# monniert/differentiable-blocksworld

Hardware: AMD Instinct MI355X
Metric: rendered views/sec (fwd+bwd) per node, DTU 400x300 K=10 blocks (higher is better)
Workload: dtype f32; 1 GPU; DTU-scan24-like synthetic: 49 views/GPU/step, 400x300, 10 superquadric blocks + ground + sky dome, faces_per_pixel=10, 256^2 textures, coarse phase (sigma=1e-4, opacity noise, decimated textures), MSE+parsimony+TV+overlap, Adam; LPIPS excluded; views_per_gpu=49, n_blocks=10, faces_per_pixel=10, txt_size=256, parallelism=one GPU: all views on it, no collective, nranks=1

## Files before the change

differentiable-blocksworld_amd/build.py:

```python
import os
import subprocess
import sys

HERE = os.path.dirname(os.path.abspath(__file__))
CSRC = os.path.join(HERE, 'csrc')
SOURCES = ['util.hip', 'raster.hip', 'project_clip.hip', 'shade_blend.hip', 'render_fused.hip', 'texture.hip', 'model_ops.hip', 'train_step.hip', 'lpips_head.hip',
           'nn_search.hip', 'render_lit.hip', 'frame_export.hip', 'image_ingest.hip', 'lens_undistort.hip', 'run_monitor.hip']
OUT = os.path.join(HERE, 'dbw_amd', 'libdbw_hip.so')
FLAGS = ['--offload-arch=gfx950', '-O3', '-std=c++17', '-fPIC', '-ffp-contract=off', '-munsafe-fp-atomics',
         '-fno-gpu-flush-denormals-to-zero', '-Wall', '-Wno-unused-function']


def needs_build():
    if not os.path.exists(OUT):
        return True
    t = os.path.getmtime(OUT)
    deps = [os.path.join(CSRC, f) for f in os.listdir(CSRC)] + [os.path.join(HERE, '..', 'include', h) for h in ('dbw_hip.h', 'dbw_eval.h', 'dbw_viz.h', 'dbw_export.h', 'dbw_ingest.h', 'dbw_lens.h', 'dbw_monitor.h')] + [__file__]
    return any(os.path.getmtime(d) > t for d in deps)


def build(force=False, verbose=False, extra_flags=()):
    if not force and not needs_build():
        return OUT
    hipcc = os.environ.get('HIPCC', '/opt/rocm/bin/hipcc')
    objs = []
    os.makedirs(os.path.join(HERE, 'build'), exist_ok=True)
    procs = []
    for s in SOURCES:
        o = os.path.join(HERE, 'build', s.replace('.hip', '.o'))
        objs.append(o)
        cmd = [hipcc] + FLAGS + list(extra_flags) + ['-c', os.path.join(CSRC, s), '-o', o]
        if verbose:
            print(' '.join(cmd))
        procs.append((s, subprocess.Popen(cmd, stdout=subprocess.PIPE, stderr=subprocess.STDOUT)))
    for s, p in procs:
        out, _ = p.communicate()
        if p.returncode != 0:
            sys.stderr.write(out.decode())
            raise RuntimeError(f'hipcc failed on {s}')
        if verbose and out:
            print(out.decode())
    subprocess.check_call([hipcc, '--offload-arch=gfx950', '-shared', '-fPIC'] + objs + ['-o', OUT])
    return OUT


def build_device_checks(force=False):
    src = os.path.join(HERE, '..', 'tests', 'device_checks.hip')
    out_dir = os.path.join(HERE, '..', 'tests', '_build')
    out = os.path.join(out_dir, 'libdbw_device_checks.so')
    deps = [src] + [os.path.join(CSRC, f) for f in ('dbw_common.h', 'raster_math.h', 'model_math.h', 'rng_math.h')]
# ... 11 lines not shown
```

differentiable-blocksworld_amd/csrc/env_bwd.h:

```cpp
#pragma once
#include "shade_common.h"

namespace dbw {

#ifndef DBW_HARD_TEX_LOG2
#define DBW_HARD_TEX_LOG2 6
#endif
#ifndef DBW_HARD_FACE_LOG2
#define DBW_HARD_FACE_LOG2 5
#endif
typedef LdsAgg<3, DBW_HARD_TEX_LOG2> HardTexAgg;
typedef LdsAgg<9, DBW_HARD_FACE_LOG2> HardFaceAgg;

#ifndef DBW_HARD_P
#define DBW_HARD_P 2
#endif
template <int P>
struct HardRegion {
    static_assert(P == 1 || P == 2 || P == 4, "tiles per wave: 1, 2 or 4");
    static constexpr int PX = P == 1 ? 1 : 2, PY = P / PX;
    static constexpr int RX = 2 * PX, RY = 2 * PY;
    static long long blocks(int N, int H, int W) {
        const int tx = (W + 7) >> 3, ty = (H + 7) >> 3;
        return (long long)N * ((tx + RX - 1) / RX) * ((ty + RY - 1) / RY);
    }
};

__device__ __forceinline__ void env_bwd_pixel(const ShadeArgs &A, const float *__restrict__ fv, float *__restrict__ gmaps, float *__restrict__ gfv,
                                              int want_bary, int persp, const MapDescCache &mdc, const int *s_md, HardTexAgg &tex_agg,
                                              HardFaceAgg &face_agg, bool valid, int fc, float u, float v, int jm, const float (&gc)[3], int xi, int yi) {
    const int j = jm & 0xfffff, map = jm >> 20;
    const bool tex = valid && (gc[0] != 0.f || gc[1] != 0.f || gc[2] != 0.f);
    Sample s;
    s.a00 = s.a01 = s.a10 = s.a11 = 0;
    s.w00 = s.w01 = s.w10 = s.w11 = 0.f;
    if (__ballot(tex) != 0ull) {
        int md[6];
        mdc.get(A, s_md, valid ? map : 0, md);
        footprint_desc(u, v, md[0], md[1], md[2], md[3], md[4], md[5], s);
        float w00 = s.w00, w01 = s.w01, w10 = s.w10, w11 = s.w11;
        if (s.a01 == s.a00) { w00 += w01; w01 = 0.f; }
        if (s.a10 == s.a00) { w00 += w10; w10 = 0.f; }
        if (s.a11 == s.a00) { w00 += w11; w11 = 0.f; }
        else if (s.a11 == s.a01) { w01 += w11; w11 = 0.f; }
        else if (s.a11 == s.a10) { w10 += w11; w11 = 0.f; }
        const int ad[4] = {s.a00, s.a01, s.a10, s.a11};
        const float wt[4] = {w00, w01, w10, w11};
        const int f = wt[1] != 0.f ? 1 : (wt[2] != 0.f ? 2 : 3);
        const int a2[2] = {ad[0], f == 1 ? ad[1] : (f == 2 ? ad[2] : ad[3])};
        const float w2[2] = {wt[0], f == 1 ? wt[1] : (f == 2 ? wt[2] : wt[3])};
#pragma unroll
        for (int q = 0; q < 2; ++q) {
            float val[3] = {gc[0] * w2[q], gc[1] * w2[q], gc[2] * w2[q]};
            const bool on = tex && w2[q] != 0.f;
            tex_agg.template add_wave_merged<4>(gmaps, (int)((unsigned)a2[q] / 3u), val, on);
        }
        const bool rest = tex && ((f == 1 && (wt[2] != 0.f || wt[3] != 0.f)) || (f == 2 && wt[3] != 0.f));
        const unsigned long long rm = __ballot(rest);
        if (rm != 0ull) {
            const bool wide = __popcll(rm) > 16;
#pragma unroll
            for (int q = 2; q < 4; ++q) {
                float val[3] = {gc[0] * wt[q], gc[1] * wt[q], gc[2] * wt[q]};
                const bool on = rest && q > f && wt[q] != 0.f;
                const int key = (int)((unsigned)ad[q] / 3u);
                if (wide) tex_agg.template add_wave_merged<4>(gmaps, key, val, on);
                else if (on) tex_agg.add(gmaps, key, val);
            }
        }
    }
    const bool geom = tex && want_bary != 0 && j >= A.geom_begin;
    float g9[9] = {0.f, 0.f, 0.f, 0.f, 0.f, 0.f, 0.f, 0.f, 0.f};
    bool has_g9 = false;
    if (__ballot(geom) != 0ull) {
        if (geom) {
            float gu, gv;
            sample_grad_uv(A.maps, s, gc, gu, gv);
            const float *uv = A.face_uvs + (long long)j * 6;
            const float go[3] = {gu * uv[0] + gv * uv[1], gu * uv[2] + gv * uv[3], gu * uv[4] + gv * uv[5]};
            int cd = -1;
            float w2 = 0.f, w3 = 0.f;
            if (A.c2o) {
                cd = A.code[fc]; w2 = A.cw[(long long)fc * 2]; w3 = A.cw[(long long)fc * 2 + 1];
            }
            float gb[3] = {0.f, 0.f, 0.f};
            convert_bary_bwd(cd, w2, w3, go, gb);
            if (gb[0] != 0.f || gb[1] != 0.f || gb[2] != 0.f) {
                has_g9 = true;
                f2 pndc;
                pndc.x = pix_to_ndc_fast(A.W - 1 - xi, ndc_axis_given(A.W, A.ndc[0], A.ndc[1]));
                pndc.y = pix_to_ndc_fast(A.H - 1 - yi, ndc_axis_given(A.H, A.ndc[2], A.ndc[3]));
                const float *q = fv + (long long)fc * 9;
                const f2 a{q[0], q[1]}, b{q[3], q[4]}, c{q[6], q[7]};
                const float z0 = q[2], z1 = q[5], z2 = q[8];
                const f3 bary0 = bary_fwd<true>(pndc, a, b, c);
                const f3 bp = persp ? persp_fwd<true>(bary0, z0, z1, z2) : bary0;
                f3 gg3{gb[0], gb[1], gb[2]};
                gg3 = clip_bwd<true>(bp, gg3);
                float pz0 = 0.f, pz1 = 0.f, pz2 = 0.f;
                if (persp) gg3 = persp_bwd<true>(bary0, z0, z1, z2, gg3, pz0, pz1, pz2);
                f2 e0, e1, e2;
                bary_bwd<true>(pndc, a, b, c, gg3, e0, e1, e2);
                g9[0] = e0.x; g9[1] = e0.y; g9[2] = pz0;
                g9[3] = e1.x; g9[4] = e1.y; g9[5] = pz1;
                g9[6] = e2.x; g9[7] = e2.y; g9[8] = pz2;
            }
        }
        face_agg.add_wave(gfv, valid ? fc : 0, g9, has_g9);
    }
}


template <int P>
__device__ __forceinline__ void env_bwd_region(const ShadeArgs &A, long long total_blocks, const float *__restrict__ gimg,
                                               float *__restrict__ gmaps, const float *__restrict__ fv, float *__restrict__ gfv,
                                               int want_bary, int persp, void *lds, int *s_md) {
    typedef HardRegion<P> R;
    constexpr int NTH = 256;
    const long long logical = xcd_remap(blockIdx.x, total_blocks);
    if (logical < 0) return;
    HardTexAgg tex_agg;
    HardFaceAgg face_agg;
    tex_agg.bind(lds);
    face_agg.bind((char *)lds + HardTexAgg::BYTES);
    const int lane = threadIdx.x & 63;
    const int wv = __builtin_amdgcn_readfirstlane(threadIdx.x >> 6);
    const int tiles_x = (A.W + 7) >> 3, tiles_y = (A.H + 7) >> 3;
    const int rx = (tiles_x + R::RX - 1) / R::RX, ry = (tiles_y + R::RY - 1) / R::RY;
    const int n = (int)(logical / (rx * ry)), t = (int)(logical % (rx * ry));
    const int tx0 = (t % rx) * R::RX + (wv & 1) * R::PX, ty0 = (t / rx) * R::RY + (wv >> 1) * R::PY;
    const long long view0 = (long long)n * tiles_y * tiles_x;
    const long long plane = (long long)A.H * A.W;
    const float gs = A.gscale ? *A.gscale : 1.f;
    int rfc[P], xs[P], ys[P];
    float ru[P], rv[P], rjm[P], rg[P][3];
    bool inpx[P];
#pragma unroll
    for (int p = 0; p < P; ++p) {
        const int tx = tx0 + p % R::PX, ty = ty0 + p / R::PX;
        const bool real = tx < tiles_x && ty < tiles_y;
        const long long tile = real ? view0 + (long long)ty * tiles_x + tx : view0;
        xs[p] = tx * 8 + (lane & 7);
        ys[p] = ty * 8 + (lane >> 3);
        inpx[p] = real && xs[p] < A.W && ys[p] < A.H;
        rfc[p] = ld_stream(A.p2f + (tile << 6) + lane);
        const float *b = A.bary + ((tile * 3) << 6) + lane;
        ru[p] = ld_stream(b); rv[p] = ld_stream(b + 64); rjm[p] = ld_stream(b + 128);
        const int xc = xs[p] < A.W ? xs[p] : A.W - 1, yc = ys[p] < A.H ? ys[p] : A.H - 1;
        const long long gb = A.img_tiled ? ((tile * 4) << 6) + lane : (long long)n * 4 * plane + (long long)yc * A.W + xc;
        const long long cs = A.img_tiled ? 64 : plane;
        rg[p][0] = ld_stream(gimg + gb); rg[p][1] = ld_stream(gimg + gb + cs); rg[p][2] = ld_stream(gimg + gb + 2 * cs);
    }
    tex_agg.clear(threadIdx.x, NTH);
    face_agg.clear(threadIdx.x, NTH);
    MapDescCache mdc;
    mdc.load(A, s_md, nullptr, threadIdx.x, NTH, true);
    __syncthreads();
    bool valid[P];
    int fc[P], jm[P];
    float gc[P][3];
#pragma unroll
    for (int p = 0; p < P; ++p) {
        valid[p] = inpx[p] && rfc[p] >= 0;
        fc[p] = valid[p] ? rfc[p] : 0;
        jm[p] = valid[p] ? __float_as_int(rjm[p]) : 0;
        ru[p] = valid[p] ? ru[p] : 0.f;
        rv[p] = valid[p] ? rv[p] : 0.f;
#pragma unroll
        for (int c = 0; c < 3; ++c) gc[p][c] = valid[p] ? rg[p][c] * gs : 0.f;
    }
#pragma unroll 1
    for (int p = 0; p < P; ++p)
        env_bwd_pixel(A, fv, gmaps, gfv, want_bary, persp, mdc, s_md, tex_agg, face_agg, valid[p], fc[p], ru[p], rv[p], jm[p], gc[p], xs[p], ys[p]);
    __syncthreads();
    tex_agg.flush(gmaps, threadIdx.x, NTH);
    face_agg.flush(gfv, threadIdx.x, NTH);
}

}
```

differentiable-blocksworld_amd/csrc/render_fused.hip:

```cpp
#include "raster_common.h"
#include "shade_common.h"
#include "loss_math.h"
#include "raster_bin.h"
#include "step_kernels.h"
#include "../../include/dbw_hip.h"

#include <math.h>
#include <stdlib.h>
#include <string.h>

using namespace dbw;

int dbw_prepare_raster(const float *face_verts, const int *first_idx, const int *num_faces, const int *neighbor, int N, long long F_total,
                       long long max_faces_per_view, int H, int W, float margin, int cull, void *workspace, size_t workspace_bytes,
                       dbw::CoarseBins &cb, hipStream_t s, bool launch, bool want_cells);
const dbw::FaceRec *dbw_workspace_recs(const void *workspace, long long F_total);
void *dbw_workspace_shade_recs(void *workspace, long long F_total);
int dbw_fill_shade_args(ShadeArgs &A, const int32_t *pix_to_face, const float *bary, const float *dists, const int32_t *c2o,
                        const int32_t *clip_code, const float *clip_w, int Fc_stride, const float *face_uvs,
                        const int32_t *face_map, const int32_t *map_desc, const float *maps, const float *faces_alpha,
                        int alpha_len, int N, int H, int W, int K, int F, float sigma, const float *background3);

#ifdef DBW_TILE_CLOCK
namespace dbw { __device__ unsigned g_tile_clock[1 << 18][4]; }
extern "C" void dbw_debug_read_tile_clock(unsigned *out, int nblocks) {
    (void)hipDeviceSynchronize();
    (void)hipMemcpyFromSymbol(out, HIP_SYMBOL(dbw::g_tile_clock), (size_t)(nblocks < (1 << 18) ? nblocks : (1 << 18)) * 16);
}
#endif
#ifdef DBW_PROFILE_FWD
extern "C" void dbw_debug_read_fwd_profile(unsigned long long *out16, int reset) {
    static unsigned long long *host = nullptr;
    const size_t bytes = (size_t)dbw::FPROF_BLOCKS * 16 * sizeof(unsigned long long);
    if (!host) host = (unsigned long long *)malloc(bytes);
    (void)hipDeviceSynchronize();
    (void)hipMemcpyFromSymbol(host, HIP_SYMBOL(dbw::g_fprof), bytes);
    for (int i = 0; i < 16; ++i) out16[i] = 0;
    for (size_t b = 0; b < (size_t)dbw::FPROF_BLOCKS; ++b)
// ... 115 lines not shown
                    bary[o.b + 3 * o.bstride] = a;
                    bary[o.b + 4 * o.bstride] = c[0]; bary[o.b + 5 * o.bstride] = c[1]; bary[o.b + 6 * o.bstride] = c[2];
                }
            }
        }
    }
    const ImgAddr ia = img_addr(A, n, yi, xi, 4);
    float *out = image + ia.base;
    float px[4];
    blend_front_finish(bl, A.bg, px);
    out[0] = px[0]; out[ia.cstride] = px[1]; out[2 * ia.cstride] = px[2]; out[3 * ia.cstride] = px[3];
}

struct UvSlot { bool valid; int fik; pay4 v; ShadeRec sr; };

template <int KMAX>
__device__ __forceinline__ UvSlot uv_slot(const TopK<KMAX, true> &q, const pay4 *home, const ShadeRec *__restrict__ srec, int k, bool in_img) {
    UvSlot s;
    float pz = 0.f;
    s.fik = 0;
    s.v = pay4{0.f, 0.f, 0.f, 0.f};
    s.valid = q.get(k, home, 64, threadIdx.x, pz, s.fik, s.v) && in_img;
    if (!s.valid) s.fik = 0;
    s.sr = srec[s.fik];
    return s;
}

__device__ __forceinline__ ShadeRec load_srec_uniform(const ShadeRec *__restrict__ sp) {
    union { v16f v; ShadeRec r; } u;
    u.v = *(const v16f *)sp;
    return u.r;
}

struct EnvFold {
    const FaceRec *recs;
    const int *first_idx;
    const int2 *cell; const int *pool;
    const int *dom;
    const int *clist, *ccount; int nx, ny;
    const int *num_faces;
    const ShadeRec *srec;
    const float *maps;
    float bg[3];
    int *p2f; float *uvj;
    int persp, dbg;
    float ndc[4];
};

__device__ __forceinline__ void env_fold_pixel(const EnvFold &E, int H, int W, int n_, int xi, int yi, bool in_img, float (&rgb)[3]) {
    const int lane = threadIdx.x;
    const int n = __builtin_amdgcn_readfirstlane(n_);
    const int tiles_x = (W + 7) >> 3, tiles_y = (H + 7) >> 3;
    const int L = __builtin_amdgcn_readfirstlane((n * tiles_y + (yi >> 3)) * tiles_x + (xi >> 3));
    const NdcAxis ax = ndc_axis_given(W, E.ndc[0], E.ndc[1]), ay = ndc_axis_given(H, E.ndc[2], E.ndc[3]);
    f2 p;
    p.x = pix_to_ndc_fast(W - 1 - xi, ax);
    p.y = pix_to_ndc_fast(H - 1 - yi, ay);
    const bool fastdiv = DBW_RASTER_FASTDIV && !(E.dbg & 1);
    const int fb = __builtin_amdgcn_readfirstlane(E.first_idx[n]);
    const int jb = __builtin_amdgcn_readfirstlane(E.dom[L]);
    if (jb >= 0 && fastdiv && !(E.dbg & 4096)) {
        const FaceRec r = load_rec_nowait(E.recs + fb + jb);
        float pz1 = 0.f, sd1 = 0.f;
        f3 bc1{0.f, 0.f, 0.f};
        bool unsafe = false;
        const bool inbox = in_img && !(p.x < r.xlo || p.x > r.xhi || p.y < r.ylo || p.y > r.yhi);
        const bool keep = inbox && eval_pair<true>(r, p, 0.f, E.persp, 1, pz1, sd1, bc1, unsafe, true);
        if (__ballot(in_img && (!keep || unsafe)) == 0ull) {
            const ShadeRec sr = load_srec_uniform(E.srec + fb + jb);
            const float bc[3] = {bc1.x, bc1.y, bc1.z};
            float bo[3], u, vv;
            convert_bary(sr.cd, sr.w2, sr.w3, bc, bo);
            interp_uv(bo, sr.uv, u, vv);
            SampleFwd s;
            footprint_fwd(u, vv, sr.off, sr.hw >> 16, sr.hw & 0xffff, sr.pads >> 16, sr.pads & 0xffff, sr.sh, s);
            fetch_fwd(E.maps, s, rgb);
            if (in_img) {
                const long long o = ((long long)L << 6) + lane;
                float *bp = E.uvj + ((long long)L * 3 << 6) + lane;
#if DBW_NT_STORES
                __builtin_nontemporal_store(fb + jb, E.p2f + o);
                __builtin_nontemporal_store(u, bp); __builtin_nontemporal_store(vv, bp + 64);
                __builtin_nontemporal_store(__int_as_float(sr.j | (sr.map << 20)), bp + 128);
#else
                E.p2f[o] = fb + jb;
                bp[0] = u; bp[64] = vv; bp[128] = __int_as_float(sr.j | (sr.map << 20));
#endif
            }
            return;
        }
    }
    TopK<1, false> q;
    q.init();
    const int2 c_ = E.cell[L];
    const int2 c = make_int2(__builtin_amdgcn_readfirstlane(c_.x), __builtin_amdgcn_readfirstlane(c_.y));
    const bool walk = c.y < 0;
    int total = c.y > 0 ? c.y : 0, cx = 0, cy = 0;
    const int *__restrict__ lst = E.pool + c.x;
    if (walk) {
        const int x0 = __builtin_amdgcn_readfirstlane(xi & ~7), y0 = __builtin_amdgcn_readfirstlane(yi & ~7);
        const int nb = E.nx * E.ny, bin = (y0 / COARSE) * E.nx + (x0 / COARSE);
        total = __builtin_amdgcn_readfirstlane(E.ccount[n * nb + bin]);
        lst = E.clist + (long long)fb * nb + (long long)bin * __builtin_amdgcn_readfirstlane(E.num_faces[n]);
        cx = (x0 & (COARSE - 1)) >> 3; cy = (y0 & (COARSE - 1)) >> 3;
    }
#pragma unroll 1
    for (int cb0 = 0; cb0 < total; cb0 += DBW_WAVE) {
        const bool have = cb0 + lane < total;
        const int e = have ? lst[cb0 + lane] : 0;
        const bool hit = have && (!walk || !(cx < ((e >> 20) & 7) || cx > ((e >> 23) & 7) || cy < ((e >> 26) & 7) || cy > ((e >> 29) & 7)));
        const unsigned long long m = __ballot(hit);
        eval_staged_chunk<1, false>(E.recs, fb, e & 0xfffff, min(DBW_WAVE, total - cb0), in_img, p, 1, 0.f, E.persp, 1, fastdiv, true, q, nullptr, DBW_WAVE,
                                    lane, false, false, m);
    }
    float pz = 0.f;
    int fi = 0;
    pay4 v{0.f, 0.f, 0.f, 0.f};
    const bool valid = q.get(0, nullptr, DBW_WAVE, lane, pz, fi, v) && in_img;
    if (!valid) fi = 0;
    const ShadeRec sr = E.srec[fi];
    const float bc[3] = {v.y, v.z, v.w};
    float bo[3], u, vv;
    convert_bary(sr.cd, sr.w2, sr.w3, bc, bo);
    interp_uv(bo, sr.uv, u, vv);
    SampleFwd s;
    footprint_fwd(u, vv, sr.off, sr.hw >> 16, sr.hw & 0xffff, sr.pads >> 16, sr.pads & 0xffff, sr.sh, s);
    float col[3];
    fetch_fwd(E.maps, s, col);
#pragma unroll
    for (int k = 0; k < 3; ++k) rgb[k] = valid ? col[k] : E.bg[k];
    if (in_img) {
        const long long o = ((long long)L << 6) + lane;
#if DBW_NT_STORES
        __builtin_nontemporal_store(valid ? fi : -1, E.p2f + o);
#else
        E.p2f[o] = valid ? fi : -1;
#endif
        if (valid) {
            float *bp = E.uvj + ((long long)L * 3 << 6) + lane;
#if DBW_NT_STORES
            __builtin_nontemporal_store(u, bp); __builtin_nontemporal_store(vv, bp + 64);
            __builtin_nontemporal_store(__int_as_float(sr.j | (sr.map << 20)), bp + 128);
#else
            bp[0] = u; bp[64] = vv; bp[128] = __int_as_float(sr.j | (sr.map << 20));
#endif
        }
    }
}

template <bool TILED>
__device__ __forceinline__ void uv8_epilogue_t(const ShadeArgs &A, int n, int xi, int yi, bool in_img, int tile, int lane, const float (&px)[4],
                                               float *__restrict__ image, const float (&env_rgb)[3], bool fold, bool no_fragments) {
    const long long plane = (long long)A.H * A.W, pix = (long long)yi * A.W + xi;
    const long long cs = TILED ? 64 : plane;
    const long long o4 = TILED ? (long long)tile * 256 : (long long)n * 4 * plane, o3 = TILED ? (long long)tile * 192 : (long long)n * 3 * plane;
    const unsigned ul = (unsigned)lane;
    const long long ol = TILED ? (long long)ul : pix;
    const float f0 = px[0], f1 = px[1], f2 = px[2], m = px[3];
    if (A.target) {
// ... 23 lines not shown
#endif
        }
        const float tot = wave_sum_dpp(sq);
        if (lane == 0) A.loss_part[tile] = tot;
    } else if (in_img) {
        float *out = image + o4 + ol;
        out[0] = f0;
        out[cs] = f1;
        out[2 * cs] = f2;
        out[3 * cs] = m;
    }
}
__device__ __forceinline__ void uv8_epilogue(const ShadeArgs &A, int n, int xi, int yi, bool in_img, int tile, int lane, const float (&px)[4],
                                             float *__restrict__ image, const float (&env_rgb)[3], bool fold, bool no_fragments = false) {
    if (A.img_tiled) uv8_epilogue_t<true>(A, n, xi, yi, in_img, tile, lane, px, image, env_rgb, fold, no_fragments);
    else uv8_epilogue_t<false>(A, n, xi, yi, in_img, tile, lane, px, image, env_rgb, fold, no_fragments);
}

template <int KMAX>
__device__ __forceinline__ void shade_uv8_empty(const ShadeArgs &A, int K, int n, int xi, int yi, int *__restrict__ p2f, float *__restrict__ image,
                                                const float (&env_rgb)[3], bool fold) {
    const int lane = threadIdx.x;
    const bool in_img = xi < A.W && yi < A.H;
    const int tiles_x = (A.W + 7) >> 3, tiles_y = (A.H + 7) >> 3;
    const int tile = __builtin_amdgcn_readfirstlane((n * tiles_y + (yi >> 3)) * tiles_x + (xi >> 3));
    if (in_img) p2f[(((long long)tile * K) << 6) + lane] = -1;
    BlendFront bl;
    blend_front_init(bl);
    float px[4];
    blend_front_finish(bl, A.bg, px);
    uv8_epilogue(A, n, xi, yi, in_img, tile, lane, px, image, env_rgb, fold, true);
}

template <int KMAX>
__device__ __forceinline__ void shade_uv8(const ShadeArgs &A, int K, const ShadeRec *__restrict__ srec, const TopK<KMAX, true> &q, const pay4 *home, int n,
                                          int xi, int yi, int *__restrict__ p2f, float *__restrict__ bary, float *__restrict__ dists,
                                          float *__restrict__ image, int dbg, const float (&env_rgb)[3], bool fold) {
    const int lane = threadIdx.x;
    const bool in_img = xi < A.W && yi < A.H;
    const int tiles_x = (A.W + 7) >> 3, tiles_y = (A.H + 7) >> 3;
    const int tile = __builtin_amdgcn_readfirstlane((n * tiles_y + (yi >> 3)) * tiles_x + (xi >> 3));
    const long long tb = ((long long)tile * K) << 6;
    int *__restrict__ p2f_t = p2f + tb;
    float *__restrict__ dists_t = dists + tb;
    float *__restrict__ bary_t = bary + tb * 8;
#if DBW_TOPK_ORDERED
    const int cnt = in_img ? q.cnt : 0;
#else
    int cnt = 0;
#pragma unroll
    for (int k = 0; k < KMAX; ++k) cnt += (in_img && k < K && q.valid(k)) ? 1 : 0;
#endif
    if (in_img && cnt == 0) p2f_t[lane] = -1;
    BlendFront bl;
    blend_front_init(bl);
    bool more = __ballot(cnt > 0) != 0ull && !(dbg & 64);
    UvSlot cur;
    cur.valid = false; cur.fik = 0; cur.v = pay4{0.f, 0.f, 0.f, 0.f};
    if (more) cur = uv_slot(q, home, srec, 0, in_img);
    UvSlot nxt = cur;
#pragma unroll
    for (int k = 0; k < KMAX; ++k) {
        more = more && k < K && __ballot(cnt > k) != 0ull;
        if (!more) break;
        if (k + 1 < KMAX) nxt = uv_slot(q, home, srec, k + 1, in_img);
        const ShadeRec &sr = cur.sr;
        const float bc[3] = {cur.v.y, cur.v.z, cur.v.w};
        float bo[3];
        convert_bary(sr.cd, sr.w2, sr.w3, bc, bo);
        float u, v;
        interp_uv(bo, sr.uv, u, v);
        const float d = cur.v.x;
        float e;
        if (A.sigma == 0.f) e = d <= 0.f ? 1.f : 0.f;
#if DBW_FWD_FAST_EXP
        else e = __expf(-(d > 0.f ? d : 0.f) * A.inv_sigma);
#else
        else e = expf(-(d > 0.f ? d : 0.f) / A.sigma);
#endif
        const float a = cur.valid ? e * sr.fa : 0.f;
        SampleFwd s;
        footprint_fwd(u, v, sr.off, sr.hw >> 16, sr.hw & 0xffff, sr.pads >> 16, sr.pads & 0xffff, sr.sh, s);
        float c[3];
        fetch_fwd(A.maps, s, c);
        if (!(a != 0.f)) c[0] = c[1] = c[2] = 0.f;
        const float T = bl.T;
        blend_front_step(bl, a, c);
        if (cur.valid && !(dbg & 32)) {
            const int o = (k << 6) + lane;
#if DBW_NT_STORES
            __builtin_nontemporal_store(k == 0 ? (cur.fik | (cnt << FRAG_COUNT_SHIFT)) : cur.fik, p2f_t + o);
            __builtin_nontemporal_store(d, dists_t + o);
            float *bp = bary_t + (k << 9) + lane;
            __builtin_nontemporal_store(u, bp);
            __builtin_nontemporal_store(v, bp + 64);
            __builtin_nontemporal_store(__int_as_float(sr.j | (sr.map << 20)), bp + 128);
            __builtin_nontemporal_store(a, bp + 192);
            __builtin_nontemporal_store(c[0], bp + 256); __builtin_nontemporal_store(c[1], bp + 320); __builtin_nontemporal_store(c[2], bp + 384);
            __builtin_nontemporal_store(T, bp + 448);
#else
            p2f_t[o] = k == 0 ? (cur.fik | (cnt << FRAG_COUNT_SHIFT)) : cur.fik;
            dists_t[o] = d;
            float *bp = bary_t + (k << 9) + lane;
            bp[0] = u;
            bp[64] = v;
            bp[128] = __int_as_float(sr.j | (sr.map << 20));
            bp[192] = a;
            bp[256] = c[0]; bp[320] = c[1]; bp[384] = c[2];
            bp[448] = T;
#endif
        }
        cur = nxt;
    }
    float px[4];
    blend_front_finish(bl, A.bg, px);
    uv8_epilogue(A, n, xi, yi, in_img, tile, lane, px, image, env_rgb, fold);
}

#define DBW_RENDER_WAVES(KMAX, UV) ((UV) ? ((KMAX) <= 4 ? 6 : (KMAX) <= 10 ? 5 : (KMAX) <= 16 ? 3 : 2) : DBW_RASTER_WAVES(KMAX))
template <int KMAX, int TW, int TH, int GROUP, bool UV, bool KEX = false>
__global__ __launch_bounds__(TW * TH, DBW_RENDER_WAVES(KMAX, UV)) void render_fwd_kernel(const FaceRec *__restrict__ recs, const float4 *__restrict__ bbox,
                                                             const int *__restrict__ first_idx, const int *__restrict__ num_faces,
                                                             float blur, int persp, int dbg,
                                                             long long total_blocks, ShadeArgs A, CoarseBins cb, const ShadeRec *__restrict__ srec,
                                                             int *__restrict__ p2f, float *__restrict__ bary, float *__restrict__ dists,
                                                             float *__restrict__ image, const EnvFold E) {
    static_assert(!UV || (TW == 8 && TH == 8), "shade_uv8 needs one wave per 8x8 tile");
    int n, xi, yi;
    TopK<KMAX, UV> q;
    pay4 *home;
    FPROF_T(t_k0);
    FPROF_ADD(13, wall_clock64());
#ifdef DBW_TILE_CLOCK
    if (KMAX > 1 && blockIdx.x < (1u << 18)) g_tile_clock[blockIdx.x][3] = (unsigned)wall_clock64();
#endif
    bool empty = false;
    float env_rgb[3] = {0.f, 0.f, 0.f};
#if defined(DBW_PROFILE_FWD) || defined(DBW_TILE_CLOCK)
    constexpr bool fold = false;
    (void)E;
#else
    const bool fold = UV && E.recs != nullptr;
#endif
    auto env_layer = [&](int n_, int xi_, int yi_, bool in_img_) {
        if constexpr (UV) { if (fold) env_fold_pixel(E, A.H, A.W, n_, xi_, yi_, in_img_, env_rgb); }
    };
    const int K = KEX ? KMAX : A.K;
    if (!raster_tile<KMAX, TW, TH, GROUP, UV>(recs, bbox, first_idx, num_faces, A.H, A.W, K, blur, persp, 1, total_blocks, cb,
                                              (dbg & (3 | 128)) | ((KMAX == 1 && A.tiled != 0 && !(dbg & 8)) ? 8 : 0), n, xi, yi, q, home,
                                              UV ? &empty : nullptr, env_layer)) return;
    FPROF_T(t_k1);
    if constexpr (UV) {
        if (empty) shade_uv8_empty<KMAX>(A, K, n, xi, yi, p2f, image, env_rgb, fold);
        else shade_uv8<KMAX>(A, K, srec, q, home, n, xi, yi, p2f, bary, dists, image, dbg, env_rgb, fold);
    }
    else {
        if (xi >= A.W || yi >= A.H) return;
        shade_generic<KMAX, TW * TH>(A, q, home, n, xi, yi, p2f, bary, dists, image);
    }
    FPROF_T(t_k2);
    FPROF_ADD(2, t_k2 - t_k1);
    FPROF_ADD(3, t_k2 - t_k0);
    FPROF_ADD(14, wall_clock64());
#ifdef DBW_TILE_CLOCK
    if (KMAX > 1 && threadIdx.x == 0 && blockIdx.x < (1u << 18)) {
        unsigned *o = g_tile_clock[blockIdx.x];
        o[0] = (unsigned)n | ((__builtin_amdgcn_s_getreg((16 - 1) << 11 | 4) & 0xffffu) << 16); o[1] = ((unsigned)(yi >> 3) << 16) | (unsigned)(xi >> 3); o[2] = (unsigned)wall_clock64();
    }
#endif
}

template <int KMAX, int TW, int TH, int GROUP, bool UV, bool KEX = false>
int launch_v(const FaceRec *recs, const float4 *bbox, const int *first_idx, const int *num_faces, float blur,
             int persp, ShadeArgs &A, const CoarseBins &cb, const ShadeRec *srec, int *p2f, float *bary, float *dists, float *image, const EnvFold &E,
             hipStream_t s) {
    const long long total = (long long)A.N * ((A.W + TW - 1) / TW) * ((A.H + TH - 1) / TH);
    DBW_REQUIRE(total < (1LL << 31) - 8, "more than 2^31 tiles in one pass");
    hipLaunchKernelGGL((render_fwd_kernel<KMAX, TW, TH, GROUP, UV, KEX>), dim3(dbw_xcd_grid(total)), dim3(TW * TH), 0, s, recs, bbox, first_idx,
                       num_faces, blur, persp, g_render_dbg, total, A, cb, srec, p2f, bary, dists, image, E);
    return dbw_check_launch("render_fwd_kernel");
}

template <int KMAX>
int launch(const FaceRec *recs, const float4 *bbox, const int *first_idx, const int *num_faces, float blur,
           int persp, ShadeArgs &A, const CoarseBins &cb, const ShadeRec *srec, int *p2f, float *bary, float *dists, float *image, const EnvFold &E,
           hipStream_t s) {
#define DBW_V(TW, TH, G, UV) launch_v<KMAX, TW, TH, G, UV>(recs, bbox, first_idx, num_faces, blur, persp, A, cb, srec, p2f, bary, dists, image, E, s)
    if constexpr (KMAX == 1) {
        if (g_render_variant == 1) return DBW_V(8, 8, 2, false);
        if (g_render_variant == 2) return DBW_V(16, 8, 2, false);
        return DBW_V(16, 16, 1, false);
    }
    else {
#ifndef DBW_FWD_GROUP
#define DBW_FWD_GROUP 2
#endif
        if (A.tiled == 2 && (A.target || !(g_render_dbg & 4)) && A.sigma >= 0.f) {
#if DBW_FWD_KEXACT
            if (A.K == KMAX) return launch_v<KMAX, 8, 8, DBW_FWD_GROUP, true, true>(recs, bbox, first_idx, num_faces, blur, persp, A, cb, srec, p2f, bary, dists, image, E, s);
#endif
            return DBW_V(8, 8, DBW_FWD_GROUP, true);
        }
        return DBW_V(8, 8, DBW_FWD_GROUP, false);
    }
#undef DBW_V
}

}

struct MseArgs { const float *env_img, *target; float scale; float *loss_part, *g_fg, *g_env; float *rec_out = nullptr; const float *grad_rec = nullptr; };

static int render_fwd_impl(const float *face_verts_c, const int32_t *first_idx, const int32_t *num_faces,
                                    const int32_t *neighbor, const int32_t *c2o, const int32_t *clip_code,
                                    const float *clip_w, int Fc_stride, const float *face_uvs, const int32_t *face_map,
                                    const int32_t *map_desc, const float *maps, const float *faces_alpha, int alpha_len,
                                    int N, int64_t F_total, int H, int W, int K, int F, float sigma, float blur_radius,
                                    int perspective_correct, const float *background3, int32_t *pix_to_face, float *bary,
                                    float *dists, float *image, void *workspace, size_t workspace_bytes,
                                    int frag_layout, const MseArgs *mse, int stage, int image_layout, dbw_stream_t stream,
                                    const dbw::EnvFoldHost *fold = nullptr) {
    DBW_REQUIRE(stage >= 0 && stage <= 2, "stage must be 0 (whole pass), 1 (workspace only) or 2 (workspace already prepared)");
    DBW_REQUIRE(face_verts_c && first_idx && num_faces && pix_to_face && bary && dists && (image || mse) && workspace, "null pointer");
    DBW_REQUIRE(workspace_bytes >= dbw_rasterize_workspace_bytes(F_total), "workspace too small");
    DBW_REQUIRE(blur_radius >= 0.f && F_total >= 0, "bad blur_radius / F_total");
    ShadeArgs A;
    int rc = dbw_fill_shade_args(A, pix_to_face, bary, dists, c2o, clip_code, clip_w, Fc_stride, face_uvs, face_map, map_desc, maps,
                                 faces_alpha, alpha_len, N, H, W, K, F, sigma, background3);
    if (rc) return rc;
    DBW_REQUIRE(frag_layout >= 0 && frag_layout <= 3, "frag_layout must be 0 (N,H,W,K), 1 (8x8-tile planar), 2 (planar, uv) or 3 (planar, hard uv)");
    DBW_REQUIRE(frag_layout < 2 || F < (1 << 20), "frag_layouts 2 and 3 pack the face id in 20 bits");
    DBW_REQUIRE(frag_layout != 3 || (K == 1 && sigma == 0.f && blur_radius == 0.f && !faces_alpha),
                "frag_layout 3 is the hard single-layer pass: K == 1, sigma == 0, no faces_alpha");
    DBW_REQUIRE(frag_layout != 2 || F_total < (1LL << FRAG_COUNT_SHIFT), "frag_layout 2 packs the clipped face id in 26 bits");
    DBW_REQUIRE(image_layout == 0 || image_layout == 1, "image_layout must be 0 (N,C,H,W) or 1 (8x8-tile planar)");
    A.tiled = frag_layout;
    A.img_tiled = image_layout;
    if (mse) {
        DBW_REQUIRE(frag_layout == 2 && K > 1 && sigma >= 0.f, "the composite + MSE epilogue belongs to the uv-fragment soft pass (frag_layout 2, K > 1, sigma >= 0)");
        DBW_REQUIRE(stage == 1 || ((mse->env_img || fold) && mse->target && mse->loss_part && mse->g_fg && mse->g_env), "null pointer");
        A.env_img = mse->env_img; A.target = mse->target; A.mse_scale = mse->scale; A.loss_part = mse->loss_part; A.g_fg = mse->g_fg; A.g_env = mse->g_env;
        A.rec_out = mse->rec_out; A.grad_rec = mse->grad_rec;
    }
    if (K > DBW_MAX_FACES_PER_PIXEL) {
        dbw_set_error("dbw_render_fwd_fused: faces_per_pixel=%d > %d", K, DBW_MAX_FACES_PER_PIXEL);
        return DBW_ERR_UNSUPPORTED;
    }
    if (N == 0) return DBW_OK;
    hipStream_t s = (hipStream_t)stream;
    const float margin = (float)sqrt((double)blur_radius);
    CoarseBins cb;
    rc = dbw_prepare_raster(face_verts_c, first_idx, num_faces, neighbor, N, F_total, c2o ? (long long)Fc_stride : F_total, H, W, margin, 0, workspace, workspace_bytes, cb, s,
                            stage != 2,  K > 1 || g_render_variant == 1);
    if (rc) return rc;
    const float4 *bbox = (const float4 *)workspace;
    const FaceRec *recs = dbw_workspace_recs(workspace, F_total);
    ShadeRec *srec = nullptr;
    if (frag_layout == 2 && K > 1 && F_total > 0) {
        srec = (ShadeRec *)dbw_workspace_shade_recs(workspace, F_total);
        if (stage != 2) {
            hipLaunchKernelGGL(shade_setup_kernel, dim3((unsigned)((F_total + 255) / 256)), dim3(256), 0, s, A, first_idx, num_faces, (long long)F_total, srec);
            rc = dbw_check_launch("shade_setup_kernel");
            if (rc) return rc;
        }
    }
    if (stage == 1) return DBW_OK;
    EnvFold E;
    memset(&E, 0, sizeof(E));
    if (fold) {
        DBW_REQUIRE(mse && frag_layout == 2 && K > 1, "the env layer folds into the soft pass with the loss epilogue");
        DBW_REQUIRE(fold->ws && fold->ws->cells && fold->ws->dom && fold->ws->shade_recs && fold->first_idx && fold->num_faces && fold->maps && fold->p2f && fold->uvj, "null pointer (env fold)");
        const dbw::RasterWorkspace &w = *fold->ws;
        E.recs = w.recs; E.first_idx = fold->first_idx; E.cell = w.cell; E.pool = w.pool; E.dom = w.dom; E.clist = w.list; E.ccount = w.count; E.nx = w.nx; E.ny = w.ny;
        E.num_faces = fold->num_faces; E.srec = (const ShadeRec *)w.shade_recs; E.maps = fold->maps;
        for (int i = 0; i < 3; ++i) E.bg[i] = fold->bg[i];
        E.p2f = fold->p2f; E.uvj = fold->uvj; E.persp = perspective_correct; E.dbg = g_render_dbg;
        for (int i = 0; i < 4; ++i) E.ndc[i] = cb.ndc[i];
        A.lean_grads = 1;
    }
#define DBW_RF(KM) launch<KM>(recs, bbox, first_idx, num_faces, blur_radius, perspective_correct, A, cb, srec, pix_to_face, bary, dists, image, E, s)
    if (K == 1) return DBW_RF(1);
    if (K <= 4) return DBW_RF(4);
    if (K <= 10) return DBW_RF(10);
    if (K <= 16) return DBW_RF(16);
    return DBW_RF(25);
#undef DBW_RF
}

extern "C" int dbw_render_fwd_fused(const float *face_verts_c, const int32_t *first_idx, const int32_t *num_faces,
                                    const int32_t *neighbor, const int32_t *c2o, const int32_t *clip_code,
                                    const float *clip_w, int Fc_stride, const float *face_uvs, const int32_t *face_map,
                                    const int32_t *map_desc, const float *maps, const float *faces_alpha, int alpha_len,
                                    int N, int64_t F_total, int H, int W, int K, int F, float sigma, float blur_radius,
                                    int perspective_correct, const float *background3, int32_t *pix_to_face, float *bary,
                                    float *dists, float *image, void *workspace, size_t workspace_bytes,
                                    int frag_layout, int stage, int image_layout, dbw_stream_t stream) {
    return render_fwd_impl(face_verts_c, first_idx, num_faces, neighbor, c2o, clip_code, clip_w, Fc_stride, face_uvs, face_map, map_desc, maps,
                           faces_alpha, alpha_len, N, F_total, H, W, K, F, sigma, blur_radius, perspective_correct, background3, pix_to_face,
                           bary, dists, image, workspace, workspace_bytes, frag_layout, nullptr, stage, image_layout, stream);
}

extern "C" int dbw_render_fwd_fused_mse(const float *face_verts_c, const int32_t *first_idx, const int32_t *num_faces,
                                        const int32_t *neighbor, const int32_t *c2o, const int32_t *clip_code,
                                        const float *clip_w, int Fc_stride, const float *face_uvs, const int32_t *face_map,
                                        const int32_t *map_desc, const float *maps, const float *faces_alpha, int alpha_len,
                                        int N, int64_t F_total, int H, int W, int K, int F, float sigma, float blur_radius,
                                        int perspective_correct, const float *background3, int32_t *pix_to_face, float *bary,
                                        float *dists, void *workspace, size_t workspace_bytes, const float *env_image,
                                        const float *target, float mse_scale, float *loss_partial, float *grad_fg,
                                        float *grad_env, int stage, int image_layout, dbw_stream_t stream) {
    const MseArgs mse{env_image, target, mse_scale, loss_partial, grad_fg, grad_env, nullptr, nullptr};
    return render_fwd_impl(face_verts_c, first_idx, num_faces, neighbor, c2o, clip_code, clip_w, Fc_stride, face_uvs, face_map, map_desc, maps,
                           faces_alpha, alpha_len, N, F_total, H, W, K, F, sigma, blur_radius, perspective_correct, background3, pix_to_face,
                           bary, dists, nullptr, workspace, workspace_bytes, 2, &mse, stage, image_layout, stream);
}

int dbw::render_fwd_fused_mse_fold(const float *face_verts_c, const int32_t *first_idx, const int32_t *num_faces, const int32_t *neighbor,
                                   const int32_t *c2o, const int32_t *clip_code, const float *clip_w, int Fc_stride, const float *face_uvs,
                                   const int32_t *face_map, const int32_t *map_desc, const float *maps, const float *faces_alpha, int alpha_len, int N,
                                   int64_t F_total, int H, int W, int K, int F, float sigma, float blur_radius, int perspective_correct,
                                   const float *background3, int32_t *pix_to_face, float *bary, float *dists, void *workspace, size_t workspace_bytes,
                                   const float *target, float mse_scale, float *loss_partial, float *grad_fg, float *grad_env, const EnvFoldHost &fold,
                                   float *rec_out, const float *grad_rec, hipStream_t stream) {
    const MseArgs mse{nullptr, target, mse_scale, loss_partial, grad_fg, grad_env, rec_out, grad_rec};
    return render_fwd_impl(face_verts_c, first_idx, num_faces, neighbor, c2o, clip_code, clip_w, Fc_stride, face_uvs, face_map, map_desc, maps,
                           faces_alpha, alpha_len, N, F_total, H, W, K, F, sigma, blur_radius, perspective_correct, background3, pix_to_face,
                           bary, dists, nullptr, workspace, workspace_bytes, 2, &mse, 2, 1, (dbw_stream_t)stream, &fold);
}
```

differentiable-blocksworld_amd/csrc/shade_blend.hip:

```cpp
#include "shade_common.h"
#include "env_bwd.h"
#include "../../include/dbw_hip.h"
#include "step_kernels.h"

#include <stdlib.h>
#include <string.h>

using namespace dbw;

__device__ __forceinline__ void st_stream4(int4 *p, int4 v) {
#if DBW_NT_LOADS
    int *q = (int *)p;
    typedef int v4i __attribute__((ext_vector_type(4)));
    v4i w; w.x = v.x; w.y = v.y; w.z = v.z; w.w = v.w;
    __builtin_nontemporal_store(w, (v4i *)q);
#else
    *p = v;
#endif
}

__device__ __forceinline__ void st_record(int4 *records, unsigned long long idx, int packed, float wx1, float wy1, float g0, float g1, float g2) {
    typedef int v2i __attribute__((ext_vector_type(2)));
    v2i *q = (v2i *)records + idx * 3ull;
    v2i a, b, c;
    a.x = packed; a.y = __float_as_int(wx1); b.x = __float_as_int(wy1); b.y = __float_as_int(g0); c.x = __float_as_int(g1); c.y = __float_as_int(g2);
#if DBW_NT_LOADS
    __builtin_nontemporal_store(a, q); __builtin_nontemporal_store(b, q + 1); __builtin_nontemporal_store(c, q + 2);
#else
    q[0] = a; q[1] = b; q[2] = c;
#endif
}

namespace {

#ifndef DBW_BWD_UNROLL
// ... 487 lines not shown
    const float t = (dx * (p.x - a.x) + dy * (p.y - a.y)) * __builtin_amdgcn_rcpf(l2);
    tt = t < 0.f ? 0.f : (t > 1.f ? 1.f : t);
    const float qx = a.x + tt * dx, qy = a.y + tt * dy;
    return (p.x - qx) * (p.x - qx) + (p.y - qy) * (p.y - qy);
}

struct BinRes {
    int bin, rank, leader, base, packed;
    float wx1, wy1;
    uint2 lay;
};

constexpr int ALPHA_DIRECT_MAPS = 64, ALPHA_DIRECT_SPREAD = 8;
constexpr size_t ALPHA_DIRECT_BYTES = (size_t)ALPHA_DIRECT_MAPS * ALPHA_DIRECT_SPREAD * sizeof(double);
#ifndef DBW_TEX_MERGE
#define DBW_TEX_MERGE 1
#endif
#ifndef DBW_FACE_MERGE
#define DBW_FACE_MERGE 1
#endif
#ifndef DBW_FACE_MERGE_BINNED
#define DBW_FACE_MERGE_BINNED 1
#endif
constexpr int TEX_MERGE = DBW_TEX_MERGE, FACE_MERGE = DBW_FACE_MERGE;
#ifndef DBW_UVB_WAVES
#define DBW_UVB_WAVES 4
#endif
#ifdef DBW_TILE_CLOCK
__device__ unsigned g_bwd_clock[1 << 16][4];
#define BWD_CLOCK_END(n_, layers_) { if (threadIdx.x == 0 && blockIdx.x < (1u << 16)) { unsigned *o_ = g_bwd_clock[blockIdx.x]; o_[0] = (unsigned)(n_); o_[1] = (unsigned)(layers_); o_[2] = (unsigned)wall_clock64(); } }
#else
#define BWD_CLOCK_END(n_, layers_)
#endif
template <bool BINNED>
__global__ __launch_bounds__(NT, (BINNED ? DBW_UVB_WAVES : 5)) void render_bwd_uv_kernel(ShadeArgs A, long long total_blocks, const float *__restrict__ gimg,
                                                              float *__restrict__ gmaps, float *__restrict__ galpha,
                                                              const float *__restrict__ fv, float *__restrict__ gfv) {
    extern __shared__ __attribute__((aligned(16))) float s_uvbwd[];
    constexpr bool SINGLE = false;
    (void)SINGLE;
    TexAgg tex_agg;
    FaceAlphaAgg fa_agg;
    if (A.sync_flag && blockIdx.x == 0 && threadIdx.x == 0) __hip_atomic_store(A.sync_flag, A.sync_val, __ATOMIC_RELEASE, __HIP_MEMORY_SCOPE_AGENT);
#ifdef DBW_TILE_CLOCK
    if (blockIdx.x < (1u << 16)) { g_bwd_clock[blockIdx.x][3] = (unsigned)wall_clock64(); g_bwd_clock[blockIdx.x][2] = 0u; }
#endif
    int n, xi, yi;
    if (!pixel_of_block<true>(A, total_blocks, n, xi, yi)) return;
    const bool in_img = xi < A.W && yi < A.H;
    const int lane = threadIdx.x & 63;
    const int tiles_x = (A.W + 7) >> 3, tiles_y = (A.H + 7) >> 3;
    const bool phantom = (yi >> 3) >= tiles_y || (xi >> 3) >= tiles_x;
    const int tile = __builtin_amdgcn_readfirstlane(phantom ? n * tiles_y * tiles_x : (n * tiles_y + (yi >> 3)) * tiles_x + (xi >> 3));
    const long long tb = ((long long)tile * A.K) << 6;
    const int *__restrict__ p2f_t = A.p2f + tb + lane;
    const float *__restrict__ dists_t = A.dists + tb + lane;
    const float *__restrict__ bary_t = A.bary + tb * 8 + lane;
    int cnt = 0;
    if (in_img && (yi >> 3) < tiles_y && (xi >> 3) < tiles_x) {
        const int raw0 = ld_stream(p2f_t);
        cnt = raw0 < 0 ? 0 : (raw0 >> FRAG_COUNT_SHIFT);
    }
    if (!BINNED) {
        tex_agg.bind(s_uvbwd);
        tex_agg.clear(threadIdx.x, NT);
    }
    fa_agg.bind((char *)s_uvbwd + (BINNED ? 0 : TexAgg::BYTES));
    fa_agg.clear(threadIdx.x, NT);
#ifndef DBW_MD_LDS_UNBINNED
#define DBW_MD_LDS_UNBINNED 0
#endif
    constexpr bool MD_LDS = BINNED || DBW_MD_LDS_UNBINNED;
    __shared__ __attribute__((aligned(16))) int s_md[MD_LDS ? MD_CACHE_MAPS * 8 : 8];
#ifndef DBW_LAST_WAVE_FLUSH
#define DBW_LAST_WAVE_FLUSH 1
#endif
    constexpr bool LAST_WAVE_FLUSH = BINNED && DBW_LAST_WAVE_FLUSH;
    __shared__ int s_done;
    if (threadIdx.x == 0) s_done = 0;
    MapDescCache mdc;
    mdc.load(A, s_md, BINNED ? A.bin_base : nullptr, threadIdx.x, NT, MD_LDS);
    double *alpha_dir = (double *)((char *)s_uvbwd + (BINNED ? 0 : TexAgg::BYTES) + FaceAlphaAgg::BYTES);
    const int n_maps = -A.alpha_len;
    const bool alpha_direct = galpha && A.faces_alpha && A.alpha_len < 0 && n_maps <= ALPHA_DIRECT_MAPS;
    if (alpha_direct)
        for (int i = threadIdx.x; i < n_maps * ALPHA_DIRECT_SPREAD; i += NT) alpha_dir[i] = 0.0;
    if (!__syncthreads_or(cnt > 0)) { BWD_CLOCK_END(n, -1); return; }
    f2 pndc;
    pndc.x = pix_to_ndc(A.W - 1 - xi, A.W, A.H);
    pndc.y = pix_to_ndc(A.H - 1 - yi, A.H, A.W);
    const long long plane = (long long)A.H * A.W;
    float gr = 0.f, gg = 0.f, gbl = 0.f, gA = 0.f;
    if (in_img && cnt > 0) {
        const ImgAddr ia = img_addr(A, n, yi, xi, 4);
        const float *gi = gimg + ia.base;
        const float gs = A.gscale ? *A.gscale : 1.f;
        gr = ld_stream(gi) * gs; gg = ld_stream(gi + ia.cstride) * gs; gbl = ld_stream(gi + 2 * ia.cstride) * gs; gA = ld_stream(gi + 3 * ia.cstride) * gs;
    }
    PROF_T(t_begin);
    int kmax = 0;
    for (int k = 0; k < A.K; ++k) {
        if (__ballot(cnt > k) == 0ull) break;
        kmax = k + 1;
    }
    PROF_T(t_p0);
    PROF_ADD(0, t_begin, t_p0);
    BlendBack bk;
    blend_back_init(bk, A.bg);
    struct Raw { int fc; float u, v, jm, a, c0, c1, c2, T, d; };
    auto load = [&](int k, bool ok) {
        Raw r;
        r.fc = 0; r.u = r.v = r.jm = r.a = r.c0 = r.c1 = r.c2 = r.d = 0.f; r.T = 1.f;
        if (ok) {
            r.fc = ld_stream(p2f_t + (k << 6)) & FRAG_FACE_MASK;
            const float *b = bary_t + (k << 9);
            r.u = ld_stream(b); r.v = ld_stream(b + 64); r.jm = ld_stream(b + 128); r.a = ld_stream(b + 192);
            r.c0 = ld_stream(b + 256); r.c1 = ld_stream(b + 320); r.c2 = ld_stream(b + 384); r.T = ld_stream(b + 448);
            r.d = ld_stream(dists_t + (k << 6));
        }
        return r;
    };
    auto load_u = [&](int k) {
        Raw r;
        r.fc = ld_stream(p2f_t + (k << 6));
        const float *b = bary_t + (k << 9);
        r.u = ld_stream(b); r.v = ld_stream(b + 64); r.jm = ld_stream(b + 128); r.a = ld_stream(b + 192);
        r.c0 = ld_stream(b + 256); r.c1 = ld_stream(b + 320); r.c2 = ld_stream(b + 384); r.T = ld_stream(b + 448);
        r.d = ld_stream(dists_t + (k << 6));
        return r;
    };
    auto masked = [&](const Raw &x, bool ok) {
        Raw r;
        r.fc = ok ? (x.fc & FRAG_FACE_MASK) : 0;
        r.u = ok ? x.u : 0.f; r.v = ok ? x.v : 0.f; r.jm = ok ? x.jm : 0.f; r.a = ok ? x.a : 0.f;
        r.c0 = ok ? x.c0 : 0.f; r.c1 = ok ? x.c1 : 0.f; r.c2 = ok ? x.c2 : 0.f; r.T = ok ? x.T : 1.f; r.d = ok ? x.d : 0.f;
        return r;
    };
    struct FaceXY { float2 v0, v1, v2; };
    auto load_xy = [&](int fc) {
        FaceXY q;
        const float *p = fv + (long long)fc * 9;
        q.v0 = make_float2(p[0], p[1]); q.v1 = make_float2(p[3], p[4]); q.v2 = make_float2(p[6], p[7]);
        return q;
    };
    const int sub = tile & (BIN_SUB - 1);
    auto reserve = [&](const Raw &r, bool ok) {
        BinRes R;
        R.bin = -1; R.rank = 0; R.leader = 0; R.base = 0; R.packed = 0; R.wx1 = R.wy1 = 0.f; R.lay = make_uint2(0u, 0u);
        const float wgt = r.T * r.a;
        const bool tex = ok && (wgt * gr != 0.f || wgt * gg != 0.f || wgt * gbl != 0.f) && !(A.dbg & (1 << 19));
        if (__ballot(tex) == 0ull) return R;
        const int map = __float_as_int(r.jm) >> 20;
        int md[6];
        mdc.get(A, s_md, tex ? map : 0, md);
        Sample s;
        footprint_desc(r.u, r.v, md[0], md[1], md[2], md[3], md[4], md[5], s);
        const bool on = tex && bin_regular(s);
        if (on) {
            R.bin = mdc.get_extra(s_md, A.bin_base, map) + (s.r0 >> 5) * ((s.ws + 31) >> 5) + (s.c0 >> 5);
            R.packed = (int)((unsigned)(s.r0 & 31) | ((unsigned)(s.c0 & 31) << 5) | ((unsigned)(s.r0 - s.r1) << 10) | ((unsigned)(s.c1 - s.c0) << 11));
            R.wx1 = s.wx1; R.wy1 = s.wy1;
        }
        unsigned long long rem = __ballot(on);
        const unsigned long long below = (1ull << lane) - 1ull;
        while (rem) {
// ... 48 lines not shown
            if (g7[6] != 0.f) atomicAdd(&alpha_dir[map * ALPHA_DIRECT_SPREAD + (lane & (ALPHA_DIRECT_SPREAD - 1))], (double)g7[6]);
            g7[6] = 0.f;
        }
        const bool f_pre = valid && (gd != 0.f || g7[6] != 0.f) && !(A.dbg & 2);
        PROF_T(t_a);
        PROF_ADD(2, t_it, t_a);
        if (BINNED) {
            if (__ballot(tex) != 0ull) {
                const unsigned start = (unsigned)__shfl((int)(cres.lay.x + (unsigned)cres.base), cres.leader, 64);
                const int room = __shfl((int)cres.lay.y - cres.base, cres.leader, 64);
                bool pending = tex;
                if (tex && cres.bin >= 0) {
                    if (cres.rank < room) {
                        if (!(A.dbg & (1 << 17)))
                            st_record(A.bin_records, (unsigned long long)(start + (unsigned)cres.rank), cres.packed, cres.wx1, cres.wy1, gc[0], gc[1], gc[2]);
                        pending = false;
                    }
                }
                if (pending) {
                    int md[6];
                    mdc.get(A, s_md, map, md);
                    Sample s;
                    footprint_desc(cur.u, cur.v, md[0], md[1], md[2], md[3], md[4], md[5], s);
#pragma unroll
                    for (int ch = 0; ch < 3; ++ch) {
                        unsafeAtomicAdd(gmaps + s.a00 + ch, gc[ch] * s.w00);
                        unsafeAtomicAdd(gmaps + s.a01 + ch, gc[ch] * s.w01);
                        unsafeAtomicAdd(gmaps + s.a10 + ch, gc[ch] * s.w10);
                        unsafeAtomicAdd(gmaps + s.a11 + ch, gc[ch] * s.w11);
                    }
                }
            }
        } else if (__ballot(tex) != 0ull) {
            int md[6];
            mdc.get(A, s_md, valid ? map : 0, md);
            Sample s;
            footprint_desc(cur.u, cur.v, md[0], md[1], md[2], md[3], md[4], md[5], s);
            float w00 = s.w00, w01 = s.w01, w10 = s.w10, w11 = s.w11;
            if (s.a01 == s.a00) { w00 += w01; w01 = 0.f; }
            if (s.a10 == s.a00) { w00 += w10; w10 = 0.f; }
            if (s.a11 == s.a00) { w00 += w11; w11 = 0.f; }
            else if (s.a11 == s.a01) { w01 += w11; w11 = 0.f; }
            else if (s.a11 == s.a10) { w10 += w11; w11 = 0.f; }
            const int ad[4] = {s.a00, s.a01, s.a10, s.a11};
            const float wt[4] = {w00, w01, w10, w11};
#ifdef DBW_STATS_BWD
            {
                int dk, rp, taps = 0, tap_lanes = 0, tap_replays = 0;
                for (int q = 0; q < 4; ++q) {
                    const bool onq = tex && wt[q] != 0.f;
                    key_stats((int)((unsigned)ad[q] / 3u), onq, dk, rp);
                    taps += __ballot(onq) != 0ull ? 1 : 0;
                    tap_lanes += __popcll(__ballot(onq));
                    tap_replays += rp;
                    if (q == 0) STAT_ADD(2, dk);
                }
                STAT_ADD(1, tap_lanes); STAT_ADD(3, taps); STAT_ADD(7, tap_replays);
            }
#endif
            const int f = wt[1] != 0.f ? 1 : (wt[2] != 0.f ? 2 : 3);
            const int a2[2] = {ad[0], f == 1 ? ad[1] : (f == 2 ? ad[2] : ad[3])};
            const float w2[2] = {wt[0], f == 1 ? wt[1] : (f == 2 ? wt[2] : wt[3])};
#pragma unroll
            for (int q = 0; q < 2; ++q) {
                float v3[3] = {gc[0] * w2[q], gc[1] * w2[q], gc[2] * w2[q]};
                bool on = tex && w2[q] != 0.f && !(A.dbg & 1);
                if (TEX_MERGE > 0 && __ballot(on) != 0ull) lane_merge<3, TEX_MERGE>((int)((unsigned)a2[q] / 3u), on, v3);
                if (on) tex_agg.add(gmaps, (int)((unsigned)a2[q] / 3u), v3);
            }
            const bool rest = tex && !(A.dbg & 1) && ((f == 1 && (wt[2] != 0.f || wt[3] != 0.f)) || (f == 2 && wt[3] != 0.f));
            if (__ballot(rest) != 0ull) {
#pragma unroll
                for (int q = 2; q < 4; ++q)
                    if (rest && q > f && wt[q] != 0.f) {
                        const float v3[3] = {gc[0] * wt[q], gc[1] * wt[q], gc[2] * wt[q]};
                        tex_agg.add(gmaps, (int)((unsigned)ad[q] / 3u), v3);
                    }
            }
        }
        PROF_T(t_b);
        PROF_ADD(4, t_a, t_b);
        if (__ballot(gd != 0.f) != 0ull && !(A.dbg & 16)) {
            f2 v0, v1, v2;
            if (PIPE) { v0 = f2{curq.v0.x, curq.v0.y}; v1 = f2{curq.v1.x, curq.v1.y}; v2 = f2{curq.v2.x, curq.v2.y}; }
            else {
                const float *q = fv + (long long)(valid ? cur.fc : 0) * 9;
                v0 = f2{q[0], q[1]}; v1 = f2{q[3], q[4]}; v2 = f2{q[6], q[7]};
            }
            float t01, t02, t12;
            const float e01 = seg_dist_t(pndc, v0, v1, t01), e02 = seg_dist_t(pndc, v0, v2, t02), e12 = seg_dist_t(pndc, v1, v2, t12);
            const int sel = (e01 <= e02 && e01 <= e12) ? 0 : ((e02 <= e01 && e02 <= e12) ? 1 : ((e12 <= e01 && e12 <= e02) ? 2 : 3));
            const f2 ea = sel == 2 ? v1 : v0, eb = sel == 0 ? v1 : v2;
            const float tt = sel == 0 ? t01 : (sel == 1 ? t02 : t12);
            const float qx = (1.f - tt) * ea.x + tt * eb.x, qy = (1.f - tt) * ea.y + tt * eb.y;
            const float g = sel == 3 ? 0.f : gd;
            const float gax = g * (1.f - tt) * 2.f * (qx - pndc.x), gay = g * (1.f - tt) * 2.f * (qy - pndc.y);
            const float gbx = g * tt * 2.f * (qx - pndc.x), gby = g * tt * 2.f * (qy - pndc.y);
            g7[0] = sel <= 1 ? gax : 0.f; g7[1] = sel <= 1 ? gay : 0.f;
            g7[2] = sel == 0 ? gbx : (sel == 2 ? gax : 0.f); g7[3] = sel == 0 ? gby : (sel == 2 ? gay : 0.f);
            g7[4] = sel >= 1 ? gbx : 0.f; g7[5] = sel >= 1 ? gby : 0.f;
        }
        PROF_T(t_c);
        PROF_ADD(5, t_b, t_c);
#ifdef DBW_STATS_BWD
        {
            int dk, rp;
            const bool f_on = valid && (gd != 0.f || g7[6] != 0.f);
            key_stats(cur.fc, f_on, dk, rp);
            STAT_ADD(0, 1); STAT_ADD(4, __popcll(__ballot(f_on))); STAT_ADD(5, dk); STAT_ADD(6, rp);
        }
#endif
        bool f_on = f_pre;
        constexpr int FM = BINNED ? DBW_FACE_MERGE_BINNED : FACE_MERGE;
        if (FM > 0 && __ballot(f_on) != 0ull) lane_merge<7, FM>(cur.fc, f_on, g7);
        if (f_on) {
            const int aidx = A.faces_alpha ? (int)alpha_grad_index(A, n, j, map) : 0;
            fa_agg.add(gfv, galpha, cur.fc, aidx, g7);
        }
        PROF_T(t_d);
        PROF_ADD(6, t_c, t_d);
    }
    PROF_T(t_end);
    int last = 0;
    if (LAST_WAVE_FLUSH) {
        if (lane == 0) last = atomicAdd(&s_done, 1) == NT / 64 - 1 ? 1 : 0;
        last = __builtin_amdgcn_readfirstlane(last);
    } else __syncthreads();
    PROF_T(t_sync);
    PROF_ADD(3, t_end, t_sync);
    if ((LAST_WAVE_FLUSH && !last) || (A.dbg & 128)) return;
    const int f_tid = LAST_WAVE_FLUSH ? lane : (int)threadIdx.x, f_n = LAST_WAVE_FLUSH ? 64 : NT;
    if (!BINNED) tex_agg.flush(gmaps, f_tid, f_n);
    fa_agg.flush(gfv, galpha, f_tid, f_n);
    if (alpha_direct)
        for (int i = f_tid; i < n_maps * ALPHA_DIRECT_SPREAD; i += f_n) {
            const float x = (float)alpha_dir[i];
            if (x != 0.f) unsafeAtomicAdd(galpha + (long long)(i / ALPHA_DIRECT_SPREAD) * DBW_ALPHA_SPREAD + ((blockIdx.x * ALPHA_DIRECT_SPREAD + i) & (DBW_ALPHA_SPREAD - 1)), x);
        }
    PROF_T(t_fl);
    PROF_ADD(1, t_sync, t_fl);
    PROF_ADD(7, t_begin, t_fl);
    BWD_CLOCK_END(n, kmax);
}

#ifndef DBW_BIN_STAGE
#define DBW_BIN_STAGE 512
#endif
constexpr int BIN_STAGE = DBW_BIN_STAGE, BIN_PER_THREAD = BIN_STAGE / 256, BIN_LANE_STRIDE = BIN_STAGE / 64;
typedef int bin_fix_t;
constexpr int BIN_FIX_SH = 20, BIN_FIX_EMIN = -100;
__global__ __launch_bounds__(256) void texbin_reduce_kernel(const int *__restrict__ bin_info, const int *__restrict__ cursor,
                                                            const int4 *__restrict__ records, int cap, const unsigned *__restrict__ layout,
                                                            float *__restrict__ gmaps) {
    __shared__ bin_fix_t tile[33 * 33 * 3];
    __shared__ int2 stage[BIN_STAGE * 3 + BIN_STAGE / BIN_LANE_STRIDE];
    __shared__ float s_wmax[4];
#ifdef DBW_REDUCE_SCRAMBLE
    const unsigned bx = blockIdx.x, nb_ = gridDim.x;
    const int bin = bx < (nb_ & ~63u) ? (int)((bx & ~63u) | ((__brev(bx & 63u) >> 26) ^ (((bx >> 6) * 2654435761u) >> 26))) : (int)bx;
    const int sub0 = blockIdx.y * BIN_SUB_PER_WG;
#else
    const int bin = (int)window_scramble(blockIdx.x, gridDim.x), sub0 = blockIdx.y * BIN_SUB_PER_WG;
#endif
    int n_sub[BIN_SUB_PER_WG], total = 0;
    unsigned first[BIN_SUB_PER_WG];
#pragma unroll
    for (int g = 0; g < BIN_SUB_PER_WG; ++g) {
        const int ci = bin * BIN_SUB + sub0 + g;
        first[g] = layout[ci * 2];
        n_sub[g] = min(cursor[ci], (int)layout[ci * 2 + 1]);
        total += n_sub[g];
    }
    if (total == 0) return;
    for (int i = threadIdx.x; i < 33 * 33 * 3; i += 256) tile[i] = 0;
    const int lane = threadIdx.x & 63, wv = threadIdx.x >> 6;
// ... 124 lines not shown
        for (int i = 0; i < 8; ++i) out8[i] += host[b * 8 + i];
    if (reset) { memset(host, 0, bytes); (void)hipMemcpyToSymbol(HIP_SYMBOL(g_prof), host, bytes); }
}
#endif

int fill_args(ShadeArgs &A, const int32_t *pix_to_face, const float *bary, const float *dists, const int32_t *c2o,
              const int32_t *clip_code, const float *clip_w, int Fc_stride, const float *face_uvs,
              const int32_t *face_map, const int32_t *map_desc, const float *maps, const float *faces_alpha,
              int alpha_len, int N, int H, int W, int K, int F, float sigma, const float *background3) {
    DBW_REQUIRE(pix_to_face && bary && dists && face_uvs && face_map && map_desc && maps, "null pointer");
    DBW_REQUIRE((c2o && clip_code && clip_w) || (!c2o && !clip_code && !clip_w), "c2o/clip_code/clip_w: all or none");
    DBW_REQUIRE(N >= 0 && H > 0 && W > 0 && K > 0 && F > 0, "bad size");
    DBW_REQUIRE(!faces_alpha || alpha_len == F || (long long)alpha_len == (long long)N * F || alpha_len < 0,
                "faces_alpha length must be F, N*F, or -(number of maps) for one opacity per texture map");
    A.p2f = pix_to_face; A.bary = bary; A.dists = dists; A.c2o = c2o; A.code = clip_code; A.cw = clip_w;
    A.Fc_stride = Fc_stride; A.face_uvs = face_uvs; A.face_map = face_map; A.map_desc = map_desc; A.maps = maps;
    A.faces_alpha = faces_alpha; A.alpha_len = alpha_len; A.N = N; A.H = H; A.W = W; A.K = K; A.F = F; A.sigma = sigma; A.inv_sigma = sigma != 0.f ? 1.f / fabsf(sigma) : 0.f;
    for (int i = 0; i < 3; ++i) A.bg[i] = background3 ? background3[i] : 0.f;
    {
        float rx = 2.0f, ry = 2.0f;
        if (W > H) rx = ((float)W * rx) / (float)H;
        if (H > W) ry = ((float)H * ry) / (float)W;
        A.ndc[0] = rx; A.ndc[1] = rx / 2.0f; A.ndc[2] = ry; A.ndc[3] = ry / 2.0f;
    }
    A.dbg = g_dbg_flags;
    A.agg = 0;
    A.tiled = 0;
    A.bin_base = nullptr; A.bin_cursor = nullptr; A.bin_records = nullptr; A.bin_cap = 0; A.bin_layout = nullptr;
    A.gscale = nullptr; A.geom_begin = 0; A.env_img = nullptr; A.target = nullptr; A.mse_scale = 0.f; A.loss_part = nullptr; A.g_fg = nullptr; A.g_env = nullptr;
    A.img_tiled = 0;
    A.lean_grads = 0;
    A.rec_out = nullptr; A.grad_rec = nullptr;
    A.sync_flag = nullptr; A.sync_val = 0;
    return DBW_OK;
}

}

extern "C" int dbw_shade_blend_fwd(const int32_t *pix_to_face, const float *bary, const float *dists,
                                   const int32_t *c2o, const int32_t *clip_code, const float *clip_w, int Fc_stride,
                                   const float *face_uvs, const int32_t *face_map, const int32_t *map_desc,
                                   const float *maps, const float *faces_alpha, int alpha_len, int N, int H, int W,
                                   int K, int F, float sigma, const float *background3, float *image,
                                   dbw_stream_t stream) {
    ShadeArgs A;
    int rc = fill_args(A, pix_to_face, bary, dists, c2o, clip_code, clip_w, Fc_stride, face_uvs, face_map, map_desc,
                       maps, faces_alpha, alpha_len, N, H, W, K, F, sigma, background3);
    if (rc) return rc;
    DBW_REQUIRE(image, "null pointer");
    if (N == 0) return DBW_OK;
    const long long total = (long long)N * ((W + TILE - 1) / TILE) * ((H + TILE - 1) / TILE);
    hipLaunchKernelGGL(shade_blend_fwd_kernel, dim3(dbw_xcd_grid(total)), dim3(NT), 0, (hipStream_t)stream, A, total, image);
    return dbw_check_launch("shade_blend_fwd_kernel");
}

int dbw_fill_shade_args(ShadeArgs &A, const int32_t *pix_to_face, const float *bary, const float *dists, const int32_t *c2o,
                        const int32_t *clip_code, const float *clip_w, int Fc_stride, const float *face_uvs,
                        const int32_t *face_map, const int32_t *map_desc, const float *maps, const float *faces_alpha,
                        int alpha_len, int N, int H, int W, int K, int F, float sigma, const float *background3) {
    return fill_args(A, pix_to_face, bary, dists, c2o, clip_code, clip_w, Fc_stride, face_uvs, face_map, map_desc, maps, faces_alpha,
                     alpha_len, N, H, W, K, F, sigma, background3);
}


constexpr int HARD_P = DBW_HARD_P;
__global__ __launch_bounds__(NT) void render_bwd_hard_kernel(ShadeArgs A, long long total_blocks, const float *__restrict__ gimg,
                                                            float *__restrict__ gmaps, const float *__restrict__ fv,
                                                            float *__restrict__ gfv, int want_bary, int persp) {
    extern __shared__ __attribute__((aligned(16))) float s_hard[];
    __shared__ __attribute__((aligned(16))) int s_md[MD_CACHE_MAPS * 8];
    env_bwd_region<HARD_P>(A, total_blocks, gimg, gmaps, fv, gfv, want_bary, persp, s_hard, s_md);
}

__global__ void flag_store_kernel(unsigned *flag, unsigned v) { __hip_atomic_store(flag, v, __ATOMIC_RELEASE, __HIP_MEMORY_SCOPE_AGENT); }

static int launch_bwd(ShadeArgs &A, int N, int H, int W, int K, const float *grad_image, float *grad_maps,
                      float *grad_faces_alpha, float *grad_dists, float *grad_bary, int lds_aggregate, const float *fv,
                      float *gfv, int want_bary, int persp, hipStream_t s) {
    if (K > DBW_MAX_FACES_PER_PIXEL) {
        dbw_set_error("shade/blend backward: faces_per_pixel=%d > %d", K, DBW_MAX_FACES_PER_PIXEL);
        return DBW_ERR_UNSUPPORTED;
    }
    if (N == 0) return DBW_OK;
    const long long total = (long long)N * ((W + TILE - 1) / TILE) * ((H + TILE - 1) / TILE);
    size_t lds = (size_t)K * NT * sizeof(float);
    const bool fused = gfv != nullptr;
    A.agg = (lds_aggregate && !(g_dbg_flags & 8)) ? 3 : ((fused && grad_faces_alpha && !(g_dbg_flags & 8)) ? 2 : 0);
    if (A.agg & 1) lds += TexAgg::BYTES;
    if (A.agg & 2) lds += AlphaAgg::BYTES;
    if (fused) lds += FaceAgg::BYTES;
    if (fused && A.bin_records) lds += (size_t)(4 * BIN_SLOTS + K * NT) * sizeof(int);
    static bool raised = false;
    if (!raised) {
        if (hipFuncSetAttribute((const void *)shade_blend_bwd_kernel<false, false, false>, hipFuncAttributeMaxDynamicSharedMemorySize, 160 * 1024) != hipSuccess ||
            hipFuncSetAttribute((const void *)shade_blend_bwd_kernel<true, false, false>, hipFuncAttributeMaxDynamicSharedMemorySize, 160 * 1024) != hipSuccess ||
            hipFuncSetAttribute((const void *)shade_blend_bwd_kernel<true, false, true>, hipFuncAttributeMaxDynamicSharedMemorySize, 160 * 1024) != hipSuccess ||
            hipFuncSetAttribute((const void *)shade_blend_bwd_kernel<true, true, false>, hipFuncAttributeMaxDynamicSharedMemorySize, 160 * 1024) != hipSuccess) {
            dbw_set_error("shade/blend backward: cannot raise the dynamic LDS limit");
            return DBW_ERR_LAUNCH;
        }
        raised = true;
    }
    const bool uv_kernel = fused && K > 1 && A.tiled == 2 && !want_bary && ((A.agg & 1) || A.bin_records) && !(g_dbg_flags & (1 << 16)) && A.sigma >= 0.f;
    if (A.sync_flag && !uv_kernel) {
        hipLaunchKernelGGL(flag_store_kernel, dim3(1), dim3(1), 0, s, A.sync_flag, A.sync_val);
        A.sync_flag = nullptr;
    }
    if (uv_kernel) {
        static bool raised_uv = false;
        if (!raised_uv) {
            if (hipFuncSetAttribute((const void *)render_bwd_uv_kernel<false>, hipFuncAttributeMaxDynamicSharedMemorySize, 64 * 1024) != hipSuccess ||
                hipFuncSetAttribute((const void *)render_bwd_uv_kernel<true>, hipFuncAttributeMaxDynamicSharedMemorySize, 64 * 1024) != hipSuccess) {
                dbw_set_error("shade/blend backward: cannot raise the dynamic LDS limit");
                return DBW_ERR_LAUNCH;
            }
            raised_uv = true;
        }
        if (A.bin_records)
            hipLaunchKernelGGL(render_bwd_uv_kernel<true>, dim3(bwd_interleave_grid(total)), dim3(NT), FaceAlphaAgg::BYTES + ALPHA_DIRECT_BYTES, s, A, total, grad_image, grad_maps,
                               grad_faces_alpha, fv, gfv);
        else
            hipLaunchKernelGGL(render_bwd_uv_kernel<false>, dim3(bwd_interleave_grid(total)), dim3(NT), TexAgg::BYTES + FaceAlphaAgg::BYTES + ALPHA_DIRECT_BYTES, s, A, total,
                               grad_image, grad_maps, grad_faces_alpha, fv, gfv);
        return dbw_check_launch("render_bwd_uv_kernel");
    }
    if (A.tiled == 3) {
        const long long regions = HardRegion<HARD_P>::blocks(N, H, W);
        hipLaunchKernelGGL(render_bwd_hard_kernel, dim3(dbw_xcd_grid(regions)), dim3(NT), HardTexAgg::BYTES + HardFaceAgg::BYTES, s, A, regions, grad_image,
                           grad_maps, fv, gfv, want_bary, persp);
        return dbw_check_launch("render_bwd_hard_kernel");
    }
    if (fused && A.bin_records)
        hipLaunchKernelGGL((shade_blend_bwd_kernel<true, true, false>), dim3(dbw_xcd_grid(total)), dim3(NT), lds, s, A, total, grad_image, grad_maps,
                           grad_faces_alpha, nullptr, nullptr, fv, gfv, want_bary, persp);
    else if (fused && K == 1)
        hipLaunchKernelGGL((shade_blend_bwd_kernel<true, false, true>), dim3(dbw_xcd_grid(total)), dim3(NT), lds, s, A, total, grad_image, grad_maps,
                           grad_faces_alpha, nullptr, nullptr, fv, gfv, want_bary, persp);
    else if (fused)
        hipLaunchKernelGGL((shade_blend_bwd_kernel<true, false, false>), dim3(dbw_xcd_grid(total)), dim3(NT), lds, s, A, total, grad_image, grad_maps,
                           grad_faces_alpha, nullptr, nullptr, fv, gfv, want_bary, persp);
    else
        hipLaunchKernelGGL((shade_blend_bwd_kernel<false, false, false>), dim3(dbw_xcd_grid(total)), dim3(NT), lds, s, A, total, grad_image, grad_maps,
                           grad_faces_alpha, grad_dists, grad_bary, nullptr, nullptr, 0, 1);
    return dbw_check_launch("shade_blend_bwd_kernel");
}

extern "C" int dbw_shade_blend_bwd(const int32_t *pix_to_face, const float *bary, const float *dists,
                                   const int32_t *c2o, const int32_t *clip_code, const float *clip_w, int Fc_stride,
                                   const float *face_uvs, const int32_t *face_map, const int32_t *map_desc,
                                   const float *maps, const float *faces_alpha, int alpha_len, int N, int H, int W,
                                   int K, int F, float sigma, const float *background3, const float *grad_image,
                                   float *grad_maps, float *grad_faces_alpha, float *grad_dists, float *grad_bary,
                                   int lds_aggregate, dbw_stream_t stream) {
    ShadeArgs A;
    int rc = fill_args(A, pix_to_face, bary, dists, c2o, clip_code, clip_w, Fc_stride, face_uvs, face_map, map_desc,
                       maps, faces_alpha, alpha_len, N, H, W, K, F, sigma, background3);
    if (rc) return rc;
    DBW_REQUIRE(grad_image && grad_maps, "null pointer");
    DBW_REQUIRE(!grad_faces_alpha || faces_alpha, "grad_faces_alpha without faces_alpha");
    return launch_bwd(A, N, H, W, K, grad_image, grad_maps, grad_faces_alpha, grad_dists, grad_bary, lds_aggregate, nullptr,
                      nullptr, 0, 1, (hipStream_t)stream);
}

int dbw::render_bwd_fused_signal(const int32_t *pix_to_face, const float *bary, const float *dists,
                                    const int32_t *c2o, const int32_t *clip_code, const float *clip_w, int Fc_stride,
                                    const float *face_uvs, const int32_t *face_map, const int32_t *map_desc,
                                    const float *maps, const float *faces_alpha, int alpha_len, int N, int H, int W,
                                    int K, int F, float sigma, const float *background3, const float *grad_image,
                                    const float *face_verts_c, int perspective_correct, int detach_bary,
                                    float *grad_maps, float *grad_faces_alpha, float *grad_face_verts_c,
                                    int lds_aggregate, int frag_layout, const int32_t *bin_base, int32_t *bin_cursor,
                                    void *bin_records, int bin_cap, const uint32_t *bin_layout, int const_geometry_faces,
                                    const float *grad_scale, int image_layout, dbw_stream_t stream, unsigned *sync_flag, unsigned sync_val) {
    ShadeArgs A;
    int rc = fill_args(A, pix_to_face, bary, dists, c2o, clip_code, clip_w, Fc_stride, face_uvs, face_map, map_desc,
                       maps, faces_alpha, alpha_len, N, H, W, K, F, sigma, background3);
    if (rc) return rc;
    DBW_REQUIRE(grad_image && grad_maps && face_verts_c && grad_face_verts_c, "null pointer");
    DBW_REQUIRE(!grad_faces_alpha || faces_alpha, "grad_faces_alpha without faces_alpha");
    DBW_REQUIRE(frag_layout >= 0 && frag_layout <= 3, "frag_layout must be 0 (N,H,W,K), 1 (8x8-tile planar), 2 (planar, uv) or 3 (planar, hard uv)");
    DBW_REQUIRE(frag_layout != 2 || detach_bary, "frag_layout 2 carries no barycentrics: only valid with detach_bary");
    DBW_REQUIRE(frag_layout != 3 || (K == 1 && sigma == 0.f && !faces_alpha && lds_aggregate && F < (1 << 20)),
                "frag_layout 3 is the hard single-layer pass: K == 1, sigma == 0, no faces_alpha, lds_aggregate, F < 2^20");
    DBW_REQUIRE(const_geometry_faces >= 0 && const_geometry_faces <= F, "const_geometry_faces must lie in [0, F]");
    DBW_REQUIRE(image_layout == 0 || image_layout == 1, "image_layout must be 0 (N,4,H,W) or 1 (8x8-tile planar)");
    A.tiled = frag_layout;
    A.img_tiled = image_layout;
    A.gscale = grad_scale;
    A.geom_begin = const_geometry_faces;
    A.sync_flag = sync_flag; A.sync_val = sync_val;
    DBW_REQUIRE((bin_base && bin_cursor && bin_records && bin_cap >= DBW_BIN_SUBCURSORS) || (!bin_base && !bin_cursor && !bin_records), "texture bins: all or none (bin_cap >= DBW_BIN_SUBCURSORS)");
    if (bin_records && !lds_aggregate) {
        A.bin_base = bin_base; A.bin_cursor = bin_cursor; A.bin_records = (int4 *)bin_records; A.bin_cap = bin_cap; A.bin_layout = bin_layout;
    }
    DBW_REQUIRE(!bin_records || bin_layout, "texture bins need their layout table (bin_layout: dbw_bin_layout; equal shares: all counts 0)");
    return launch_bwd(A, N, H, W, K, grad_image, grad_maps, grad_faces_alpha, nullptr, nullptr, lds_aggregate, face_verts_c,
                      grad_face_verts_c, detach_bary ? 0 : 1, perspective_correct, (hipStream_t)stream);
}

extern "C" int dbw_render_bwd_fused(const int32_t *pix_to_face, const float *bary, const float *dists,
                                    const int32_t *c2o, const int32_t *clip_code, const float *clip_w, int Fc_stride,
                                    const float *face_uvs, const int32_t *face_map, const int32_t *map_desc,
                                    const float *maps, const float *faces_alpha, int alpha_len, int N, int H, int W,
                                    int K, int F, float sigma, const float *background3, const float *grad_image,
                                    const float *face_verts_c, int perspective_correct, int detach_bary,
                                    float *grad_maps, float *grad_faces_alpha, float *grad_face_verts_c,
                                    int lds_aggregate, int frag_layout, const int32_t *bin_base, int32_t *bin_cursor,
                                    void *bin_records, int bin_cap, const uint32_t *bin_layout, int const_geometry_faces,
                                    const float *grad_scale, int image_layout, dbw_stream_t stream) {
    return dbw::render_bwd_fused_signal(pix_to_face, bary, dists, c2o, clip_code, clip_w, Fc_stride, face_uvs, face_map, map_desc, maps, faces_alpha, alpha_len,
                                        N, H, W, K, F, sigma, background3, grad_image, face_verts_c, perspective_correct, detach_bary, grad_maps, grad_faces_alpha,
                                        grad_face_verts_c, lds_aggregate, frag_layout, bin_base, bin_cursor, bin_records, bin_cap, bin_layout, const_geometry_faces,
                                        grad_scale, image_layout, stream, nullptr, 0);
}

#ifdef DBW_TILE_CLOCK
extern "C" void dbw_debug_read_bwd_clock(unsigned *out, int nblocks) {
    (void)hipDeviceSynchronize();
    (void)hipMemcpyFromSymbol(out, HIP_SYMBOL(g_bwd_clock), (size_t)(nblocks < (1 << 16) ? nblocks : (1 << 16)) * 16);
}
#endif

extern "C" int dbw_texbin_reduce(const int32_t *bin_info, const int32_t *bin_cursor, const void *bin_records, int bin_cap,
                                 const uint32_t *bin_layout, int nbins, float *grad_maps, dbw_stream_t stream) {
    DBW_REQUIRE(bin_info && bin_cursor && bin_records && bin_layout && grad_maps, "null pointer");
    DBW_REQUIRE(bin_cap >= DBW_BIN_SUBCURSORS && nbins >= 0, "bad size");
    DBW_REQUIRE((long long)nbins * bin_cap < (1LL << 32), "the record array is indexed with 32 bits: nbins * bin_cap must stay below 2^32 (128 GB of records)");
    if (nbins == 0) return DBW_OK;
    hipLaunchKernelGGL(texbin_reduce_kernel, dim3(nbins, BIN_SUB / BIN_SUB_PER_WG), dim3(256), 0, (hipStream_t)stream, bin_info, bin_cursor,
                       (const int4 *)bin_records, bin_cap, bin_layout, grad_maps);
    return dbw_check_launch("texbin_reduce_kernel");
}

__global__ __launch_bounds__(1024) void bin_layout_kernel(const int *__restrict__ asked, long long n, double total, int min_records,
                                                          unsigned *__restrict__ layout) {
    __shared__ double s_sum[1024];
    const int t = threadIdx.x;
    const long long per = (n + 1023) / 1024, i0 = min(n, t * per), i1 = min(n, i0 + per);
    double mine = 0.0;
    for (long long i = i0; i < i1; ++i) mine += (double)max(asked[i], min_records) * 1.25;
    s_sum[t] = mine;
    __syncthreads();
    for (int o = 512; o > 0; o >>= 1) { if (t < o) s_sum[t] += s_sum[t + o]; __syncthreads(); }
    const double scale = (total - (double)n) / s_sum[0];
    __syncthreads();
    double caps = 0.0;
// ... 31 lines not shown
```

differentiable-blocksworld_amd/csrc/shade_common.h:

```cpp
#pragma once
#include "dbw_common.h"
#include "shade_math.h"

namespace dbw {

#ifndef DBW_NT_LOADS
#define DBW_NT_LOADS 1
#endif
template <class T>
__device__ __forceinline__ T ld_stream(const T *p) {
#if DBW_NT_LOADS
    return __builtin_nontemporal_load(p);
#else
    return *p;
#endif
}

#ifndef DBW_TEX_LOG2
#define DBW_TEX_LOG2 8
#endif
typedef LdsAgg<3, DBW_TEX_LOG2> TexAgg;
typedef LdsAgg<1, 8> AlphaAgg;
typedef LdsAgg<9, 7> FaceAgg;

struct ShadeArgs {
    const int *p2f; const float *bary; const float *dists;
    const int *c2o; const int *code; const float *cw; int Fc_stride;
    const float *face_uvs; const int *face_map; const int *map_desc; const float *maps;
    const float *faces_alpha; int alpha_len;
    int N, H, W, K, F; float sigma, inv_sigma; float bg[3];
    int tiled;
    int agg;
    const int *bin_base;
    float ndc[4];
    int *bin_cursor;
    int4 *bin_records;
    int bin_cap;
    const unsigned *bin_layout;
    int dbg;
    const float *gscale;
    int geom_begin;
    const float *env_img, *target;
    float mse_scale;
    float *loss_part, *g_fg, *g_env;
    int img_tiled;
    int lean_grads;
    float *rec_out;
    const float *grad_rec;
    unsigned *sync_flag; unsigned sync_val;
};

#ifndef DBW_MD_LDS
#define DBW_MD_LDS 1
#endif
constexpr int MD_CACHE_MAPS = 64;
struct MapDescCache {
    bool in_lds;
    __device__ __forceinline__ void load(const ShadeArgs &A, int *s_md, const int *extra, int tid, int nthreads, bool enable) {
        const int rows = (DBW_MD_LDS && enable) ? __builtin_amdgcn_readfirstlane(A.map_desc[6]) : 0;
        in_lds = rows > 0 && rows <= MD_CACHE_MAPS;
        if (in_lds)
            for (int i = tid; i < rows * 8; i += nthreads) s_md[i] = ((i & 7) == 7 && extra) ? extra[i >> 3] : A.map_desc[i];
    }
    __device__ __forceinline__ void get(const ShadeArgs &A, const int *s_md, int map, int (&d)[6]) const {
        if (in_lds) {
            const int4 a = *(const int4 *)(s_md + map * 8);
            const int2 b = *(const int2 *)(s_md + map * 8 + 4);
            d[0] = a.x; d[1] = a.y; d[2] = a.z; d[3] = a.w; d[4] = b.x; d[5] = b.y;
        } else {
            const int *md = A.map_desc + map * 8;
#pragma unroll
            for (int i = 0; i < 6; ++i) d[i] = md[i];
            asm volatile("" : "+v"(d[0]), "+v"(d[1]), "+v"(d[2]), "+v"(d[3]), "+v"(d[4]), "+v"(d[5]));
        }
    }
    __device__ __forceinline__ int get_extra(const int *s_md, const int *extra, int map) const {
        int v;
        if (in_lds) v = s_md[map * 8 + 7];
        else {
            v = extra[map];
            asm volatile("" : "+v"(v));
        }
// ... 188 lines not shown
```

differentiable-blocksworld_amd/csrc/shade_math.h:

```cpp
#pragma once
#include "raster_math.h"

namespace dbw {

struct Sample {
    int a00, a01, a10, a11;
    float w00, w01, w10, w11;
    float dudx, dvdy;
    float wx0, wx1, wy0, wy1;
    int r0, c0, r1, c1, ws;
};

DBW_HD float sel3(int i, float a, float b, float c) { return i == 0 ? a : (i == 1 ? b : c); }

#ifndef DBW_SHADE_FMA
#define DBW_SHADE_FMA 0
#endif
#if DBW_SHADE_FMA && defined(__clang__)
#define DBW_FMA_SCOPE _Pragma("clang fp contract(fast)")
#else
#define DBW_FMA_SCOPE
#endif

DBW_HD void convert_bary(int cd, float w2, float w3, const float b[3], float bo[3]) {
// ... 28 lines not shown
    if ((unsigned)c >= (unsigned)w) { c %= w; if (c < 0) c += w; }
    return c;
}

DBW_HD void footprint_desc(float u, float v, int off, int h, int w, int pl, int pr, int sh, Sample &s) {
    const int wp = w + pl + pr;
    float ix = ((u * 2.f - 1.f) + 1.f) / 2.f * (float)(wp - 1);
    float iy = ((v * 2.f - 1.f) + 1.f) / 2.f * (float)(h - 1);
    s.dudx = (float)(wp - 1); s.dvdy = (float)(h - 1);
    if (!(ix > 0.f)) { ix = 0.f; s.dudx = 0.f; } else if (ix >= (float)(wp - 1)) { ix = (float)(wp - 1); s.dudx = 0.f; }
    if (!(iy > 0.f)) { iy = 0.f; s.dvdy = 0.f; } else if (iy >= (float)(h - 1)) { iy = (float)(h - 1); s.dvdy = 0.f; }
    const float fx = floorf(ix), fy = floorf(iy);
    const int x0 = (int)fx, y0 = (int)fy;
    const int x1 = x0 + 1 < wp - 1 ? x0 + 1 : wp - 1, y1 = y0 + 1 < h - 1 ? y0 + 1 : h - 1;
    s.wx1 = ix - fx; s.wx0 = 1.f - s.wx1;
    s.wy1 = iy - fy; s.wy0 = 1.f - s.wy1;
    int c0 = wrap_col(x0 - pl, w), c1 = wrap_col(x1 - pl, w);
    const int r0 = (h - 1 - y0) >> sh, r1 = (h - 1 - y1) >> sh, ws = w >> sh;
    c0 >>= sh; c1 >>= sh;
    s.a00 = off + (r0 * ws + c0) * 3; s.a01 = off + (r0 * ws + c1) * 3;
    s.a10 = off + (r1 * ws + c0) * 3; s.a11 = off + (r1 * ws + c1) * 3;
    s.w00 = s.wx0 * s.wy0; s.w01 = s.wx1 * s.wy0; s.w10 = s.wx0 * s.wy1; s.w11 = s.wx1 * s.wy1;
    s.r0 = r0; s.c0 = c0; s.r1 = r1; s.c1 = c1; s.ws = ws;
}

DBW_HD void fetch(const float *maps, const Sample &s, float c[3]) {
    DBW_FMA_SCOPE
#pragma unroll
    for (int ch = 0; ch < 3; ++ch)
        c[ch] = maps[s.a00 + ch] * s.w00 + maps[s.a01 + ch] * s.w01 + maps[s.a10 + ch] * s.w10 + maps[s.a11 + ch] * s.w11;
}

struct SampleFwd { unsigned b00, b01, b10, b11; float w00, w01, w10, w11; };
DBW_HD void footprint_fwd(float u, float v, int off, int h, int w, int pl, int pr, int sh, SampleFwd &s) {
    const int wp = w + pl + pr;
    float ix = ((u * 2.f - 1.f) + 1.f) / 2.f * (float)(wp - 1);
    float iy = ((v * 2.f - 1.f) + 1.f) / 2.f * (float)(h - 1);
    ix = __builtin_fminf(__builtin_fmaxf(ix, 0.f), (float)(wp - 1));
    iy = __builtin_fminf(__builtin_fmaxf(iy, 0.f), (float)(h - 1));
    const float fx = floorf(ix), fy = floorf(iy);
    const int x0 = (int)fx, y0 = (int)fy;
    const int x1 = x0 + 1 < wp - 1 ? x0 + 1 : wp - 1, y1 = y0 + 1 < h - 1 ? y0 + 1 : h - 1;
    const float wx1 = ix - fx, wx0 = 1.f - wx1, wy1 = iy - fy, wy0 = 1.f - wy1;
    int c0 = wrap_col(x0 - pl, w), c1 = wrap_col(x1 - pl, w);
    const int r0 = (h - 1 - y0) >> sh, r1 = (h - 1 - y1) >> sh, ws = w >> sh;
    c0 >>= sh; c1 >>= sh;
    s.b00 = ((unsigned)off + (unsigned)(r0 * ws + c0) * 3u) * 4u; s.b01 = ((unsigned)off + (unsigned)(r0 * ws + c1) * 3u) * 4u;
    s.b10 = ((unsigned)off + (unsigned)(r1 * ws + c0) * 3u) * 4u; s.b11 = ((unsigned)off + (unsigned)(r1 * ws + c1) * 3u) * 4u;
    s.w00 = wx0 * wy0; s.w01 = wx1 * wy0; s.w10 = wx0 * wy1; s.w11 = wx1 * wy1;
}
DBW_HD void fetch_fwd(const float *maps, const SampleFwd &s, float c[3]) {
    DBW_FMA_SCOPE
    const char *m = (const char *)maps;
    const float *t00 = (const float *)(m + s.b00), *t01 = (const float *)(m + s.b01), *t10 = (const float *)(m + s.b10), *t11 = (const float *)(m + s.b11);
#pragma unroll
    for (int ch = 0; ch < 3; ++ch) c[ch] = t00[ch] * s.w00 + t01[ch] * s.w01 + t10[ch] * s.w10 + t11[ch] * s.w11;
}


DBW_HD void sample_grad_uv(const float *maps, const Sample &s, const float gc[3], float &gu, float &gv) {
    float gix = 0.f, giy = 0.f;
#pragma unroll
    for (int ch = 0; ch < 3; ++ch) {
        const float t00 = maps[s.a00 + ch], t01 = maps[s.a01 + ch], t10 = maps[s.a10 + ch], t11 = maps[s.a11 + ch];
        gix += gc[ch] * ((t01 - t00) * s.wy0 + (t11 - t10) * s.wy1);
        giy += gc[ch] * ((t10 - t00) * s.wx0 + (t11 - t01) * s.wx1);
    }
    gu = gix * s.dudx;
    gv = giy * s.dvdy;
}

DBW_HD float geometric_alpha(float d, float sigma) {
    if (sigma == 0.f) return d <= 0.f ? 1.f : 0.f;
    if (sigma < 0.f) return 1.f / (1.f + expf(d / -sigma));
    return expf(-(d > 0.f ? d : 0.f) / sigma);
}

struct BlendFront { float T, r, g, b; };
DBW_HD void blend_front_init(BlendFront &s) { s.T = 1.f; s.r = s.g = s.b = 0.f; }
DBW_HD void blend_front_step(BlendFront &s, float a, const float c[3]) {
    DBW_FMA_SCOPE
    const float wgt = s.T * a;
// ... 21 lines not shown
```

differentiable-blocksworld_amd/csrc/step_kernels.h:

```cpp
#pragma once
#include <hip/hip_runtime.h>
#include <stdint.h>

#include "../../include/dbw_hip.h"

namespace dbw {
struct RasterWorkspace;

constexpr int STEP_MAX_SETS = 4;
struct StepTextureSets { dbw_texture_set s[STEP_MAX_SETS]; };

struct PrologueArgs {
    StepTextureSets tex; int nsets;
    const float *alpha_logit, *noise;
    float noise_scale, thresh;
    int nb;
    float *alpha, *alpha_full;
    int *keep;
    unsigned long long seed, rng_step;
    const float *sq_eps, *S, *R6, *T, *trig;
    int nv;
    float ratio, scale_min, S_world;
    const float *Rw, *Tw;
    float *blk_verts;
// ... 44 lines not shown
    float *ws;
    unsigned *ticket;
};
int launch_regularisers(const RegulariserArgs &A, hipStream_t s);

struct BlocksTailArgs {
    const float *sq_eps, *S, *R6, *T, *sq_local; const int *keep; int nb, nv; float scale_min, S_world; const float *Rw;
    const float *g_verts;
    float *g_sq_eps, *g_S, *g_R6, *g_T;
    const float *alpha, *g_alpha_parts, *g_alpha_full; int alpha_parts; float *g_logit;
    const float *void_raised; float *void_flag;
};
int launch_blocks_tail(const BlocksTailArgs &A, hipStream_t s);

struct ClipBwdArgs {
    const float *verts; const int *faces; const float *R, *T, *Kmat; int B, V, F; float eps, zc; int persp;
    const int *num_faces, *c2o, *code; const float *cw, *gfvc; float *gverts;
};
int launch_clip_bwd_tex(const ClipBwdArgs &C, const dbw_texture_set &tex, hipStream_t s);

struct AdamTailArgs {
    float *param, *grad, *exp_avg, *exp_avg_sq; const int64_t *group_end; const float *lr; int ngroups;
    float beta1, beta2, eps; int step;
    void *zero_buf; int64_t zero_bytes, hole_begin, hole_end;
    dbw_texture_set tex[2]; int ntex;
    const float *void_raised; float *void_flag;
};
bool adam_tail_fits(const AdamTailArgs &A);
int launch_adam_tail(const AdamTailArgs &A, hipStream_t s);

struct EnvFoldHost {
    const RasterWorkspace *ws; const int *first_idx, *num_faces; const float *maps; float bg[3];
    int *p2f; float *uvj;
};
int render_fwd_fused_mse_fold(const float *face_verts_c, const int32_t *first_idx, const int32_t *num_faces, const int32_t *neighbor,
                              const int32_t *c2o, const int32_t *clip_code, const float *clip_w, int Fc_stride, const float *face_uvs,
                              const int32_t *face_map, const int32_t *map_desc, const float *maps, const float *faces_alpha, int alpha_len, int N,
                              int64_t F_total, int H, int W, int K, int F, float sigma, float blur_radius, int perspective_correct,
                              const float *background3, int32_t *pix_to_face, float *bary, float *dists, void *workspace, size_t workspace_bytes,
                              const float *target, float mse_scale, float *loss_partial, float *grad_fg, float *grad_env, const EnvFoldHost &fold,
                              float *rec_out, const float *grad_rec, hipStream_t stream);

int render_bwd_fused_signal(const int32_t *pix_to_face, const float *bary, const float *dists, const int32_t *c2o, const int32_t *clip_code,
                            const float *clip_w, int Fc_stride, const float *face_uvs, const int32_t *face_map, const int32_t *map_desc, const float *maps,
                            const float *faces_alpha, int alpha_len, int N, int H, int W, int K, int F, float sigma, const float *background3,
                            const float *grad_image, const float *face_verts_c, int perspective_correct, int detach_bary, float *grad_maps,
                            float *grad_faces_alpha, float *grad_face_verts_c, int lds_aggregate, int frag_layout, const int32_t *bin_base,
                            int32_t *bin_cursor, void *bin_records, int bin_cap, const uint32_t *bin_layout, int const_geometry_faces,
                            const float *grad_scale, int image_layout, dbw_stream_t stream, unsigned *sync_flag, unsigned sync_val);

}
```

differentiable-blocksworld_amd/csrc/train_step.hip:

```cpp
#include "dbw_common.h"
#include "raster_bin.h"
#include "step_kernels.h"
#include "../../include/dbw_hip.h"

#include <math.h>
#include <mutex>
#include <new>
#include <stdlib.h>
#include <string.h>

using namespace dbw;

namespace {

__global__ __launch_bounds__(256) void tile_target_kernel(const float *__restrict__ img, int B, int C, int H, int W, float *__restrict__ out) {
    const int tx = (W + 7) >> 3, ty = (H + 7) >> 3;
    const long long total = (long long)B * ty * tx * C * 64;
    for (long long i = (long long)blockIdx.x * blockDim.x + threadIdx.x; i < total; i += (long long)gridDim.x * blockDim.x) {
        const int lane = (int)(i & 63);
        long long r = i >> 6;
        const int c = (int)(r % C); r /= C;
        const int tix = (int)(r % tx); r /= tx;
        const int tiy = (int)(r % ty);
        const int n = (int)(r / ty);
        const int y = tiy * 8 + (lane >> 3), x = tix * 8 + (lane & 7);
        out[i] = (y < H && x < W) ? img[(((long long)n * C + c) * H + y) * W + x] : 0.f;
    }
}

constexpr int LOSS_BLOCKS = 32;
__global__ __launch_bounds__(256) void loss_finish_kernel(const float *__restrict__ part, long long nparts, float scale, float tv_value_scale, float *vals,
                                                          float *__restrict__ out5) {
    __shared__ float s_red[4];
    __shared__ int s_last;
    float acc = 0.f;
    for (long long i = (long long)blockIdx.x * 256 + threadIdx.x; i < nparts; i += (long long)gridDim.x * 256) acc += part[i];
    acc = wave_sum(acc);
    if ((threadIdx.x & 63) == 0) s_red[threadIdx.x >> 6] = acc;
    __syncthreads();
    if (threadIdx.x == 0) {
        const float t = (s_red[0] + s_red[1]) + (s_red[2] + s_red[3]);
        if (t != 0.f) unsafeAtomicAdd(vals, t);
        __threadfence();
        s_last = atomicAdd((unsigned *)(vals + 5), 1u) == gridDim.x - 1 ? 1 : 0;
    }
    __syncthreads();
    if (s_last && threadIdx.x == 0) {
        __threadfence();
        const float rgb = atomicAdd(vals, 0.f) * scale;
        const float tvv = vals[2] * tv_value_scale;
        out5[0] = rgb; out5[1] = vals[1]; out5[2] = tvv; out5[3] = vals[3];
        out5[4] = ((rgb + vals[1]) + tvv) + vals[3];
    }
}

size_t al(size_t x) { return (x + 255) & ~(size_t)255; }

struct SceneBuf { size_t fvc, first, num, c2o, nbr, code, cw, rws, rws_bytes; };

struct Layout {
    SceneBuf e, f;
    size_t p2f_e, bary_e, dists_e, img_e, p2f, bary, dists, part, g_fg, g_env;
    size_t env_maps, blk_maps, sig[3], g_sig[3];
    size_t alpha, alpha_full, keep, blk_verts, sq_local, losses, target;
    size_t records, cursor[2], layout[2], layout_uniform;
    size_t arena_begin, g_alpha_full, ovl_ws, vals, tickets, g_blk_maps, g_env_maps, g_maps_end, g_fa, g_fvc_f, g_blk_verts, g_fvc_e, g_env_verts, arena_end;
    size_t total;
    int Fe, Ff, Ve, Vf, tiles, bin_cap;
    size_t ce, cb_, n_env_maps, n_blk_maps;
};

bool tv_on(const dbw_step_desc &d) { return d.w_tv_bkg != 0.f || d.w_tv_blocks != 0.f || d.w_tv_ground != 0.f; }
bool bins_on(const dbw_step_desc &d) { return d.decim_blocks == 1 && d.n_bins > 0 && d.block_bin_base && d.block_bin_info; }

int texbin_capacity(int B, int H, int W, int K, int nbins) {
    long long cap = (long long)B * H * W * (K > 4 ? K : 4) / (2LL * nbins);
    if (cap < 256) cap = 256;
    const long long hi = (16LL << 30) / (32LL * nbins);
    if (cap > hi) cap = hi;
    return (int)((cap + DBW_BIN_SUBCURSORS - 1) / DBW_BIN_SUBCURSORS * DBW_BIN_SUBCURSORS);
}

void scene_layout(SceneBuf &s, size_t &o, int B, int F, int H, int W) {
    const size_t n = (size_t)B * 2 * F;
    s.fvc = o; o += al(n * 9 * 4);
    s.first = o; o += al((size_t)B * 4);
    s.num = o; o += al((size_t)B * 4);
    s.c2o = o; o += al(n * 4);
    s.nbr = o; o += al(n * 4);
    s.code = o; o += al(n * 4);
    s.cw = o; o += al(n * 8);
    s.rws_bytes = dbw_rasterize_workspace_bytes_binned((int64_t)n, B, H, W);
    s.rws = o; o += al(s.rws_bytes);
}

void make_layout(const dbw_step_desc &d, Layout &L) {
    memset(&L, 0, sizeof(L));
    const int B = d.max_views, K = d.faces_per_pixel;
    L.Fe = d.n_sky_faces + d.n_ground_faces; L.Ff = d.n_blocks * d.block_nf;
    L.Ve = d.n_sky_verts + d.n_ground_verts; L.Vf = d.n_blocks * d.block_nv;
    L.tiles = ((d.H + 7) / 8) * ((d.W + 7) / 8);
    const size_t bt = (size_t)B * L.tiles;
    L.ce = (size_t)(d.env_txt_size / d.decim_env) * (d.env_txt_size / d.decim_env) * 3;
    L.cb_ = (size_t)(d.txt_size / d.decim_blocks) * (d.txt_size / d.decim_blocks) * 3;
    L.n_env_maps = 2 * L.ce; L.n_blk_maps = (size_t)d.n_blocks * L.cb_;
    size_t o = 0;
// ... 3 lines not shown
    L.bary_e = o; o += al(bt * 64 * 3 * 4);
    L.dists_e = o; o += al(bt * 64 * 4);
    L.img_e = o; o += al(bt * 256 * 4);
    L.p2f = o; o += al(bt * K * 64 * 4);
    L.bary = o; o += al(bt * K * 64 * 8 * 4);
    L.dists = o; o += al(bt * K * 64 * 4);
    L.part = o; o += al(bt * 4);
    L.g_fg = o; o += al(bt * 256 * 4);
    L.g_env = o; o += al(bt * 256 * 4);
    L.env_maps = o; o += al(L.n_env_maps * 4);
    L.blk_maps = o; o += al(L.n_blk_maps * 4);
    const size_t full[3] = {(size_t)d.env_txt_size * d.env_txt_size * 3, (size_t)d.n_blocks * d.txt_size * d.txt_size * 3, (size_t)d.env_txt_size * d.env_txt_size * 3};
    const int dec[3] = {d.decim_env, d.decim_blocks, d.decim_env};
    for (int i = 0; i < 3; ++i) {
        if (dec[i] > 1) { L.sig[i] = o; o += al(full[i] * 4); }
        else L.sig[i] = i == 0 ? L.env_maps : (i == 1 ? L.blk_maps : L.env_maps + L.ce * 4);
        if (tv_on(d)) { L.g_sig[i] = o; o += al(full[i] * 4); }
    }
    L.alpha = o; o += al((size_t)d.n_blocks * 4);
    L.alpha_full = o; o += al((size_t)d.n_blocks * 4);
    L.keep = o; o += al((size_t)d.n_blocks * 4);
    L.blk_verts = o; o += al((size_t)L.Vf * 12);
    L.sq_local = o; o += al((size_t)L.Vf * 36);
    L.losses = o; o += al(8 * 4);
    L.target = o; o += al(bt * 192 * 4);
    if (bins_on(d)) {
        L.bin_cap = texbin_capacity(B, d.H, d.W, K, d.n_bins);
        const size_t nsub = (size_t)d.n_bins * DBW_BIN_SUBCURSORS;
        L.records = o; o += al((size_t)d.n_bins * L.bin_cap * 32);
        for (int i = 0; i < 2; ++i) { L.cursor[i] = o; o += al(nsub * 4); }
        for (int i = 0; i < 2; ++i) { L.layout[i] = o; o += al(nsub * 8); }
        L.layout_uniform = o; o += al(nsub * 8);
    }
    L.arena_begin = o;
    L.g_alpha_full = o; o += al((size_t)d.n_blocks * 4);
    L.ovl_ws = o; o += al((size_t)d.n_blocks * 18 * 4);
    L.vals = o; o += al(8 * 4);
    L.tickets = o; o += al(4 * 4);
    L.g_blk_maps = o; o += al(L.n_blk_maps * 4);
    L.g_env_maps = o; o += al(L.n_env_maps * 4);
    L.g_maps_end = o;
    L.g_fa = o; o += al((size_t)d.n_blocks * 64 * 4);
    L.g_fvc_f = o; o += al((size_t)B * 2 * L.Ff * 9 * 4);
    L.g_blk_verts = o; o += al((size_t)L.Vf * 12);
    L.g_fvc_e = o; o += al((size_t)B * 2 * L.Fe * 9 * 4);
    L.g_env_verts = o; o += al((size_t)L.Ve * 12);
    L.arena_end = o;
    L.total = o;
}


void fill_texture_sets(const dbw_step_desc &d, const Layout &L, char *ws, dbw_texture_set (&sets)[3]) {
#define FPW(off) ((float *)(ws + (off)))
    memset(sets, 0, sizeof(sets));
    const float *tex[3] = {d.texture_bkg, d.textures, d.texture_ground};
    float *gtex[3] = {d.g_texture_bkg, d.g_textures, d.g_texture_ground};
    const int tn[3] = {1, d.n_blocks, 1}, th[3] = {d.env_txt_size, d.txt_size, d.env_txt_size}, td[3] = {d.decim_env, d.decim_blocks, d.decim_env};
    float *maps_out[3] = {FPW(L.env_maps), FPW(L.blk_maps), FPW(L.env_maps) + L.ce};
    float *gmaps[3] = {FPW(L.g_env_maps), FPW(L.g_blk_maps), FPW(L.g_env_maps) + L.ce};
    const float tvw[3] = {d.w_tv_bkg, d.w_tv_blocks, d.w_tv_ground};
    for (int i = 0; i < 3; ++i) {
        dbw_texture_set &t = sets[i];
        t.texture = tex[i]; t.n = tn[i]; t.h = th[i]; t.w = th[i]; t.decim = td[i];
        t.maps = maps_out[i];
        t.sig = td[i] > 1 ? FPW(L.sig[i]) : nullptr;
        t.wrap_x = i == 1 ? 1 : 0;
// ... 78 lines not shown
            __hip_atomic_store(host_timeouts, 1u, __ATOMIC_RELEASE, __HIP_MEMORY_SCOPE_SYSTEM);
            break;
        }
    }
}
constexpr unsigned long long SYNC_LIMIT_TICKS = 100000000ull;

}

struct dbw_step_plan {
    dbw_step_desc d;
    Layout L;
    char *ws;
    RasterWorkspace rw_e, rw_f;
    hipEvent_t ev_prologue, ev_scatter, ev_fg_fwd, ev_reg, ev_layout, ev_kernel_done, ev_blocks_ready, ev_env_done, ev_losses;
    hipStream_t stream_r, stream_env;
    unsigned long long runs;
    int bin_turn, bin_ready, uniform_ready;
    bool arena_clean;
    float *host_losses;
    bool losses_pending;
    bool phase1_done;
    bool cur_flags;
    bool profile, profiled;
    hipEvent_t ev_t[8];
    unsigned *sync_words;
    unsigned *host_timeouts, *host_timeouts_dev;
    unsigned sync_val[SYNC_FLAGS];
    int voided_runs;
    int force_timeout;
    bool last_tail;
};

extern "C" size_t dbw_train_step_workspace_bytes(const dbw_step_desc *desc) {
    if (check_desc(desc)) return 0;
    Layout L;
    make_layout(*desc, L);
    return L.total;
}

extern "C" dbw_step_plan *dbw_train_step_create(const dbw_step_desc *desc, void *workspace, size_t workspace_bytes) {
    if (check_desc(desc)) return nullptr;
    if (!workspace || ((uintptr_t)workspace & 255)) { dbw_set_error("dbw_train_step_create: the workspace must be 256-byte aligned"); return nullptr; }
    dbw_step_plan *p = new (std::nothrow) dbw_step_plan();
    if (!p) { dbw_set_error("dbw_train_step_create: out of host memory"); return nullptr; }
    p->d = *desc;
    make_layout(p->d, p->L);
    if (workspace_bytes < p->L.total) {
        dbw_set_error("dbw_train_step_create: workspace of %zu bytes, %zu needed", workspace_bytes, p->L.total);
        dbw_train_step_destroy(p);
        return nullptr;
    }
    p->ws = (char *)workspace;
    hipEvent_t *evs[] = {&p->ev_prologue, &p->ev_scatter, &p->ev_fg_fwd, &p->ev_reg, &p->ev_layout, &p->ev_kernel_done, &p->ev_blocks_ready, &p->ev_env_done, &p->ev_losses};
    for (hipEvent_t *e : evs)
        if (hipEventCreateWithFlags(e, hipEventDisableTiming) != hipSuccess) { dbw_set_error("dbw_train_step_create: hipEventCreate failed"); dbw_train_step_destroy(p); return nullptr; }
    if (step_streams(p->stream_r, p->stream_env)) { dbw_train_step_destroy(p); return nullptr; }
    if (hipHostMalloc((void **)&p->host_losses, 8 * sizeof(float), hipHostMallocDefault) != hipSuccess) {
        dbw_set_error("dbw_train_step_create: hipHostMalloc failed");
        dbw_train_step_destroy(p);
        return nullptr;
    }
    for (int i = 0; i < 8; ++i) p->host_losses[i] = 0.f;
    p->sync_words = nullptr;
    if (hipMalloc((void **)&p->sync_words, SYNC_WORDS * sizeof(unsigned)) != hipSuccess || hipMemset(p->sync_words, 0, SYNC_WORDS * sizeof(unsigned)) != hipSuccess) {
        dbw_set_error("dbw_train_step_create: hipMalloc failed");
// ... 18 lines not shown
    return p;
}

extern "C" void dbw_train_step_destroy(dbw_step_plan *p) {
    if (!p) return;
    hipEvent_t evs[] = {p->ev_prologue, p->ev_scatter, p->ev_fg_fwd, p->ev_reg, p->ev_layout, p->ev_kernel_done, p->ev_blocks_ready, p->ev_env_done, p->ev_losses};
    for (hipEvent_t e : evs) if (e) (void)hipEventDestroy(e);
    for (hipEvent_t e : p->ev_t) if (e) (void)hipEventDestroy(e);
    if (p->host_losses) (void)hipHostFree(p->host_losses);
    if (p->sync_words) (void)hipFree(p->sync_words);
    if (p->host_timeouts) (void)hipHostFree(p->host_timeouts);
    delete p;
}

extern "C" int64_t dbw_train_step_offset(const dbw_step_plan *p, int which) {
    if (!p) return -1;
    const Layout &L = p->L;
    switch (which) {
        case 0: return (int64_t)L.alpha;
        case 1: return (int64_t)L.alpha_full;
        case 2: return (int64_t)L.keep;
        case 3: return (int64_t)L.losses;
        case 4: return (int64_t)L.arena_begin;
        case 5: return (int64_t)L.arena_end;
        case 6: return (int64_t)L.g_fg;
        case 7: return (int64_t)L.g_env;
        case 8: return (int64_t)L.img_e;
        case 9: return (int64_t)L.blk_verts;
        case 10: return (int64_t)L.part;
        case 11: return (int64_t)L.p2f_e;
        case 12: return (int64_t)L.bary_e;
        case 13: return (int64_t)L.g_blk_maps;
        case 14: return (int64_t)L.g_maps_end;
        default: return -1;
    }
}


extern "C" int dbw_train_step_losses(dbw_step_plan *p, float *out5) {
    DBW_REQUIRE(p && out5, "null pointer");
    DBW_REQUIRE(p->losses_pending, "no run with read_losses != 0 to read from");
    if (hipEventSynchronize(p->ev_losses) != hipSuccess) { dbw_set_error("dbw_train_step_losses: hipEventSynchronize failed"); return DBW_ERR_LAUNCH; }
    for (int i = 0; i < 5; ++i) out5[i] = p->host_losses[i];
    return DBW_OK;
}

#define HIP_OK(call)                                                              \
    do {                                                                          \
        const hipError_t e_ = (call);                                             \
        if (e_ != hipSuccess) {                                                   \
            dbw_set_error("dbw_train_step_run: %s: %s", #call, hipGetErrorString(e_)); \
            return DBW_ERR_LAUNCH;                                                \
        }                                                                         \
    } while (0)
#define RC(call)                  \
    do {                          \
        const int rc_ = (call);   \
        if (rc_) return rc_;      \
    } while (0)

extern "C" int dbw_train_step_run(dbw_step_plan *p, const dbw_step_inputs *in, dbw_stream_t stream_main, dbw_stream_t stream_side) {
    DBW_REQUIRE(p && in, "null pointer");
    const dbw_step_desc &d = p->d;
    const Layout &L = p->L;
    DBW_REQUIRE(in->imgs && in->R && in->T, "null input");
    if (*(volatile unsigned *)p->host_timeouts != 0u) {
// ... 233 lines not shown
            RC(launch_scene_bins(Bn, M));
            RC(dbw_launch_work_scatter(wf, B, H, W, M, tex_flag, tex_val));
        }
    } else {
        RC(dbw_project_clip_fwd(d.env_verts, d.env_faces, in->R, in->T, d.Kmat, B, Ve, Fe, d.cam_eps, zc_on, d.z_clip, d.perspective_correct, FP(L.e.fvc),
                                IP(L.e.first), IP(L.e.num), IP(L.e.c2o), IP(L.e.nbr), IP(L.e.code), FP(L.e.cw), M));
        RC(dbw_project_clip_fwd(FP(L.blk_verts), d.block_faces, in->R, in->T, d.Kmat, B, Vf, Ff, d.cam_eps, zc_on, d.z_clip, d.perspective_correct,
                                FP(L.f.fvc), IP(L.f.first), IP(L.f.num), IP(L.f.c2o), IP(L.f.nbr), IP(L.f.code), FP(L.f.cw), M));
        RC(dbw_render_fwd_fused(FP(L.e.fvc), IP(L.e.first), IP(L.e.num), IP(L.e.nbr), IP(L.e.c2o), IP(L.e.code), FP(L.e.cw), 2 * Fe, d.env_face_uvs,
                                d.env_face_map, d.env_map_desc, FP(L.env_maps), nullptr, 0, B, Fte, H, W, 1, Fe, 0.f, 0.f, d.perspective_correct, d.bg_env,
                                IP(L.p2f_e), FP(L.bary_e), FP(L.dists_e), FP(L.img_e), ws + L.e.rws, L.e.rws_bytes, 3, 1, 1, M));
        RC(dbw_render_fwd_fused_mse(FP(L.f.fvc), IP(L.f.first), IP(L.f.num), IP(L.f.nbr), IP(L.f.c2o), IP(L.f.code), FP(L.f.cw), 2 * Ff, d.block_face_uvs,
                                    d.block_face_map, d.block_map_desc, FP(L.blk_maps), fa, alpha_len, B, Ftf, H, W, K, Ff, d.sigma, d.blur_radius,
                                    d.perspective_correct, d.bg_fg, IP(L.p2f), FP(L.bary), FP(L.dists), ws + L.f.rws, L.f.rws_bytes, nullptr, nullptr, 0.f,
                                    nullptr, nullptr, nullptr, 1, 1, M));
    }

    if (prologue_signal_folded) RC(side_head());

#define PROF(i, st) do { if (p->profile) HIP_OK(hipEventRecord(p->ev_t[i], st)); } while (0)
    PROF(0, M);
    if (!fold)
        RC(dbw_render_fwd_fused(FP(L.e.fvc), IP(L.e.first), IP(L.e.num), IP(L.e.nbr), IP(L.e.c2o), IP(L.e.code), FP(L.e.cw), 2 * Fe, d.env_face_uvs,
                                d.env_face_map, d.env_map_desc, FP(L.env_maps), nullptr, 0, B, Fte, H, W, 1, Fe, 0.f, 0.f, d.perspective_correct, d.bg_env,
                                IP(L.p2f_e), FP(L.bary_e), FP(L.dists_e), FP(L.img_e), ws + L.e.rws, L.e.rws_bytes, 3, 2, 1, M));
    PROF(1, M);
    if (setup_aside) RC(await(M, F_SCATTER, p->ev_scatter));
    PROF(2, M);
    if (fold) {
        EnvFoldHost fh;
        fh.ws = &we; fh.first_idx = IP(L.e.first); fh.num_faces = IP(L.e.num); fh.maps = FP(L.env_maps);
        for (int i = 0; i < 3; ++i) fh.bg[i] = d.bg_env[i];
        fh.p2f = IP(L.p2f_e); fh.uvj = FP(L.bary_e);
        RC(render_fwd_fused_mse_fold(FP(L.f.fvc), IP(L.f.first), IP(L.f.num), IP(L.f.nbr), IP(L.f.c2o), IP(L.f.code), FP(L.f.cw), 2 * Ff, d.block_face_uvs,
                                     d.block_face_map, d.block_map_desc, FP(L.blk_maps), fa, alpha_len, B, Ftf, H, W, K, Ff, d.sigma, d.blur_radius,
                                     d.perspective_correct, d.bg_fg, IP(L.p2f), FP(L.bary), FP(L.dists), ws + L.f.rws, L.f.rws_bytes, target, mse_scale,
                                     FP(L.part), FP(L.g_fg), FP(L.g_env), fh, phase == 1 ? in->rec_out : nullptr, phase == 2 ? in->grad_rec : nullptr, M));
        if (phase == 1) { p->phase1_done = true; return DBW_OK; }
        p->phase1_done = false;
    } else
    RC(dbw_render_fwd_fused_mse(FP(L.f.fvc), IP(L.f.first), IP(L.f.num), IP(L.f.nbr), IP(L.f.c2o), IP(L.f.code), FP(L.f.cw), 2 * Ff, d.block_face_uvs,
                                d.block_face_map, d.block_map_desc, FP(L.blk_maps), fa, alpha_len, B, Ftf, H, W, K, Ff, d.sigma, d.blur_radius,
                                d.perspective_correct, d.bg_fg, IP(L.p2f), FP(L.bary), FP(L.dists), ws + L.f.rws, L.f.rws_bytes, FP(L.img_e), target, mse_scale,
                                FP(L.part), FP(L.g_fg), FP(L.g_env), 2, 1, M));
    PROF(3, M);
    const bool seq = d.backward_order != 0 || (bins && !d.binned_concurrent);
    const bool fwd_signal_folded = flags && two;
    if (two && !fwd_signal_folded) RC(signal(M, F_FG_FWD, p->ev_fg_fwd));

    auto loss_values = [&](hipStream_t st) -> int {
        hipLaunchKernelGGL(loss_finish_kernel, dim3(LOSS_BLOCKS), dim3(256), 0, st, FP(L.part), (long long)B * L.tiles, mse_scale,
                           d.tv_value_scale != 0.f ? d.tv_value_scale : 1.f, vals, FP(L.losses));
        RC(dbw_check_launch("loss_finish_kernel"));
        if (two) RC(signal(st, F_REG, p->ev_reg));
        if (in->read_losses) {
            HIP_OK(hipMemcpyAsync(p->host_losses, FP(L.losses), 5 * sizeof(float), hipMemcpyDeviceToHost, st));
            HIP_OK(hipEventRecord(p->ev_losses, st));
            p->losses_pending = true;
        }
        return DBW_OK;
    };

    auto env_backward = [&](hipStream_t st) -> int {
        PROF(6, st);
        RC(dbw_render_bwd_fused(IP(L.p2f_e), FP(L.bary_e), FP(L.dists_e), IP(L.e.c2o), IP(L.e.code), FP(L.e.cw), 2 * Fe, d.env_face_uvs, d.env_face_map,
                                d.env_map_desc, FP(L.env_maps), nullptr, 0, B, H, W, 1, Fe, 0.f, d.bg_env, FP(L.g_env), FP(L.e.fvc), d.perspective_correct, 0,
                                FP(L.g_env_maps), nullptr, FP(L.g_fvc_e), 1, 3, nullptr, nullptr, nullptr, 0, nullptr, d.n_sky_faces, nullptr, 1, st));
        PROF(7, st);
        RC(dbw_project_clip_bwd(d.env_verts, d.env_faces, in->R, in->T, d.Kmat, B, Ve, Fe, d.cam_eps, d.z_clip, d.perspective_correct, IP(L.e.num),
                                IP(L.e.c2o), IP(L.e.code), FP(L.e.cw), FP(L.g_fvc_e), FP(L.g_env_verts), st));
        RC(dbw_posed_mesh_bwd(d.ground_base, d.n_ground_verts, d.R6_ground, d.T_ground, d.S_world, d.R_world, FP(L.g_env_verts) + (size_t)d.n_sky_verts * 3,
                              d.g_R6_ground, d.g_T_ground, st));
        if (defer || adam_tail) return DBW_OK;
        if (two) RC(await(st, F_REG, p->ev_reg));
        dbw_texture_set env_sets[2] = {sets[0], sets[2]};
        if (!tv) { env_sets[0].grad_sig = nullptr; env_sets[1].grad_sig = nullptr; }
        RC(dbw_texture_prep_bwd_sets(env_sets, 2, st));
        return DBW_OK;
    };
    auto side_after_fwd = [&]() -> int {
        if (two) {
            RC(await(Rg, F_FG_FWD, p->ev_fg_fwd));
            RC(loss_values(Rg));
        }
        if (two && !seq) {
            RC(await(E, F_FG_FWD, p->ev_fg_fwd));
            RC(env_backward(E));
            RC(signal(E, F_ENV_DONE, p->ev_env_done));
        }
        return DBW_OK;
    };
    if (!fwd_signal_folded) RC(side_after_fwd());

    if (bins && two) RC(await(M, F_LAYOUT, p->ev_layout));
    PROF(4, M);
    unsigned *bwd_flag = nullptr, bwd_val = 0;
    if (fwd_signal_folded) { bwd_flag = p->sync_words + F_FG_FWD; bwd_val = ++p->sync_val[F_FG_FWD]; }
    RC(render_bwd_fused_signal(IP(L.p2f), FP(L.bary), FP(L.dists), IP(L.f.c2o), IP(L.f.code), FP(L.f.cw), 2 * Ff, d.block_face_uvs, d.block_face_map,
                               d.block_map_desc, FP(L.blk_maps), fa, alpha_len, B, H, W, K, Ff, d.sigma, d.bg_fg, FP(L.g_fg), FP(L.f.fvc), d.perspective_correct, 1,
                               FP(L.g_blk_maps), coarse ? FP(L.g_fa) : nullptr, FP(L.g_fvc_f), d.decim_blocks > 1 ? 1 : 0, 2, bins ? d.block_bin_base : nullptr, cursor,
                               bins ? (void *)(ws + L.records) : nullptr, bins ? L.bin_cap : 0, blayout, 0, nullptr, 1, M, bwd_flag, bwd_val));
    PROF(5, M);
    if (fwd_signal_folded) RC(side_after_fwd());
    if (two && seq) {
        RC(signal(M, F_KERNEL_DONE, p->ev_kernel_done));
        RC(await(E, F_KERNEL_DONE, p->ev_kernel_done));
        RC(env_backward(E));
        RC(signal(E, F_ENV_DONE, p->ev_env_done));
    }
    if (bins) RC(dbw_texbin_reduce(d.block_bin_info, cursor, ws + L.records, L.bin_cap, blayout, d.n_bins, FP(L.g_blk_maps), M));
    if (adam_tail) RC(await(M, F_REG, p->ev_reg));
    const bool early_textures = two && !in->with_adam && !defer;
    auto blocks_textures = [&]() -> int {
        if (defer) return DBW_OK;
        dbw_texture_set blk = sets[1];
        if (!tv) blk.grad_sig = nullptr;
        RC(dbw_texture_prep_bwd_sets(&blk, 1, M));
        if (early_textures) RC(signal(M, F_BLOCKS_READY, p->ev_blocks_ready));
        return DBW_OK;
    };
    if (early_textures) {
        RC(await(M, F_REG, p->ev_reg));
        RC(blocks_textures());
    }
    const bool tail_merged = (d.fuse & 32) && !early_textures && !defer;
    if (!tail_merged)
        RC(dbw_project_clip_bwd(FP(L.blk_verts), d.block_faces, in->R, in->T, d.Kmat, B, Vf, Ff, d.cam_eps, d.z_clip, d.perspective_correct, IP(L.f.num),
                                IP(L.f.c2o), IP(L.f.code), FP(L.f.cw), FP(L.g_fvc_f), FP(L.g_blk_verts), M));
    if (!two) { RC(env_backward(M)); RC(loss_values(M)); }
    auto blocks_chain = [&]() -> int {
        if (tail_merged) {
            ClipBwdArgs C;
            C.verts = FP(L.blk_verts); C.faces = d.block_faces; C.R = in->R; C.T = in->T; C.Kmat = d.Kmat; C.B = B; C.V = Vf; C.F = Ff;
            C.eps = d.cam_eps; C.zc = d.z_clip; C.persp = d.perspective_correct;
// ... 137 lines not shown
```

differentiable-blocksworld_amd/dbw_amd/_lib.py:

```python
import ctypes
import os

_HERE = os.path.dirname(os.path.abspath(__file__))
LIB_PATH = os.path.join(_HERE, 'libdbw_hip.so')
_lib = None


def _header_abi_version():
    import re
    with open(os.path.join(_HERE, '..', '..', 'include', 'dbw_hip.h')) as f:
        return int(re.search(r'#define DBW_ABI_VERSION (\d+)', f.read()).group(1))


ABI_VERSION = _header_abi_version()

c_p = ctypes.c_void_p
c_i = ctypes.c_int
c_f = ctypes.c_float
c_i64 = ctypes.c_int64
c_d = ctypes.c_double
c_sz = ctypes.c_size_t



# ... 165 lines not shown
    'dbw_images_undistort_u8': [c_p, c_i, c_i, c_i, c_p, c_p, c_p],
}
LENS_N_PARAMS = 12


def _header_lens_abi_version():
    import re
    with open(os.path.join(_HERE, '..', '..', 'include', 'dbw_lens.h')) as f:
        return int(re.search(r'#define DBW_LENS_ABI_VERSION (\d+)', f.read()).group(1))


LENS_ABI_VERSION = _header_lens_abi_version()

MONITOR_SIGNATURES = {
    'dbw_image_scores': [c_p, c_p, c_i, c_i, c_i, c_i, c_p, c_p, c_p, c_p],
    'dbw_meter_add': [c_p, c_p, c_i, c_d, c_i64, c_p],
    'dbw_meter_reset': [c_p, c_i, c_p],
}
MONITOR_OTHER_SIGNATURES = {
    'dbw_image_scores_workspace_bytes': (c_sz, [c_i, c_i, c_i, c_i]),
}
METER_MAX_VALUES = 16


def _header_monitor_abi_version():
    import re
    with open(os.path.join(_HERE, '..', '..', 'include', 'dbw_monitor.h')) as f:
        return int(re.search(r'#define DBW_MONITOR_ABI_VERSION (\d+)', f.read()).group(1))


MONITOR_ABI_VERSION = _header_monitor_abi_version()


def load():
    global _lib
    if _lib is not None:
        return _lib
    try:
        import importlib.util
        spec = importlib.util.spec_from_file_location('_dbw_build', os.path.join(_HERE, '..', 'build.py'))
        b = importlib.util.module_from_spec(spec)
        spec.loader.exec_module(b)
        if b.needs_build() and os.path.exists(os.environ.get('HIPCC', '/opt/rocm/bin/hipcc')):
            b.build()
    except Exception as e:
        if not os.path.exists(LIB_PATH):
            raise RuntimeError(f'libdbw_hip.so is missing and could not be built: {e}') from e
    if not os.path.exists(LIB_PATH):
        raise RuntimeError(f'{LIB_PATH} not found: run `python differentiable-blocksworld_amd/build.py` '
                           '(there is no CPU fallback for the render path)')
    lib = ctypes.CDLL(os.environ.get('DBW_HIP_LIB') or LIB_PATH)
    lib.dbw_last_error.restype = ctypes.c_char_p
    lib.dbw_abi_version.restype = c_i
    if not os.environ.get('DBW_HIP_LIB') and lib.dbw_abi_version() != ABI_VERSION:
        raise RuntimeError(f'{LIB_PATH} was built for ABI {lib.dbw_abi_version()}, include/dbw_hip.h declares {ABI_VERSION}: rebuild '
                           '(python differentiable-blocksworld_amd/build.py --force)')
    if hasattr(lib, 'dbw_bin_subcursors'):
        lib.dbw_bin_subcursors.restype = c_i
    lib.dbw_rasterize_workspace_bytes.restype = c_sz
    lib.dbw_rasterize_workspace_bytes.argtypes = [c_i64]
    lib.dbw_rasterize_workspace_bytes_binned.restype = c_sz
    lib.dbw_rasterize_workspace_bytes_binned.argtypes = [c_i64, c_i, c_i, c_i]
    for name, argtypes in SIGNATURES.items():
        if name.startswith('dbw_train_step') and not hasattr(lib, name):
            continue
        fn = getattr(lib, name)
# ... 18 lines not shown
        for name, (restype, argtypes) in VIZ_OTHER_SIGNATURES.items():
            fn = getattr(lib, name)
            fn.argtypes, fn.restype = argtypes, restype
    if hasattr(lib, 'dbw_export_abi_version'):
        lib.dbw_export_abi_version.restype = c_i
        for name, argtypes in EXPORT_SIGNATURES.items():
            fn = getattr(lib, name)
            fn.argtypes = argtypes
            fn.restype = c_i
    if hasattr(lib, 'dbw_ingest_abi_version'):
        lib.dbw_ingest_abi_version.restype = c_i
        for name, argtypes in INGEST_SIGNATURES.items():
            fn = getattr(lib, name)
            fn.argtypes = argtypes
            fn.restype = c_i
        for name, (restype, argtypes) in INGEST_OTHER_SIGNATURES.items():
            fn = getattr(lib, name)
            fn.argtypes, fn.restype = argtypes, restype
    if hasattr(lib, 'dbw_lens_abi_version'):
        lib.dbw_lens_abi_version.restype = c_i
        for name, argtypes in LENS_SIGNATURES.items():
            fn = getattr(lib, name)
            fn.argtypes = argtypes
            fn.restype = c_i
    if hasattr(lib, 'dbw_monitor_abi_version'):
        lib.dbw_monitor_abi_version.restype = c_i
        for name, argtypes in MONITOR_SIGNATURES.items():
            fn = getattr(lib, name)
            fn.argtypes = argtypes
            fn.restype = c_i
        for name, (restype, argtypes) in MONITOR_OTHER_SIGNATURES.items():
            fn = getattr(lib, name)
            fn.argtypes, fn.restype = argtypes, restype
    _lib = lib
    return lib


def call(name, *args):
    lib = load()
    rc = getattr(lib, name)(*args)
    if rc != 0:
        raise RuntimeError(f'{name} failed (rc={rc}): {lib.dbw_last_error().decode()}')
```

differentiable-blocksworld_amd/dbw_amd/c_step.py:

```python
import ctypes
import os
import warnings
import weakref

import torch

from . import _lib, ops
from .dbw import OVERLAP_N_BLOCKS, OVERLAP_N_POINTS, OVERLAP_TEMPERATURE

_p = ops._ptr
FUSE_ALL = 127
_SIDE_STREAMS = {}
_OFF = {'alpha': 0, 'alpha_full': 1, 'keep': 2, 'losses': 3, 'arena_begin': 4, 'arena_end': 5, 'g_fg': 6, 'g_env': 7, 'env_img': 8, 'blk_verts': 9,
        'loss_part': 10, 'p2f_env': 11, 'uvj_env': 12}


def side_stream(dev, priority=True):
    key = (dev.index, bool(priority))
    if key not in _SIDE_STREAMS:
        _SIDE_STREAMS[key] = torch.cuda.Stream(device=dev, priority=-1 if priority else 0)
    return _SIDE_STREAMS[key]


class StepLosses(dict):
    NAMES = ('rgb', 'parsimony', 'tv', 'overlap', 'total')

    def __init__(self, step, dev_vals, names, pending_host, perceptual=None):
        super().__init__()
        self._step, self._pending, self._perceptual = step, pending_host, perceptual
        for k in names:
            if k == 'perceptual':
                dict.__setitem__(self, k, perceptual)
            elif k in self.NAMES:
                dict.__setitem__(self, k, dev_vals[self.NAMES.index(k)])
        dict.__setitem__(self, 'total', dev_vals[4] if perceptual is None else dev_vals[4] + perceptual)

    def host(self):
        if self._pending:
            out = (ctypes.c_float * 5)()
            _lib.call('dbw_train_step_losses', self._step._plan_handle(), ctypes.cast(out, ctypes.c_void_p))
            res = {k: float(out[self.NAMES.index(k)]) for k in self if k in self.NAMES}
            if self._perceptual is not None:
                res['perceptual'] = float(self._perceptual)
                res['total'] += res['perceptual']
            return {k: res[k] for k in self}
        v = torch.stack([dict.__getitem__(self, k) for k in self]).tolist()
        return dict(zip(self.keys(), v))


class CStep:
    def __init__(self, model, params, opt_state, fuse=FUSE_ALL, max_views=None):
        self.m, self.params, self.opt = model, params, opt_state
        self.fuse = int(fuse)
        self.max_views = max_views
        self.side_priority = True
        self.backward_order = None
        self.binned_concurrent = None
        self.use_side_stream = True
        self.own_side_stream = False
        self.serial_setup_max_views = 12
        self.sync_events = os.environ.get('DBW_STEP_EVENTS', '0') not in ('', '0')
        self.read_losses = False
        self._plans = {}
        self._pid = os.getpid()
        self._cur = None
        self._target, self._target_key = None, None
        self._env_key = None
        self._inp = _lib.StepInputs()
        self._clean_plan = None
        self._calls = 0
        self._voided_seen = {}

    def supported(self):
        m, w = self.m, self.m.loss_weights
        r = m.renderer
        perceptual_ok = 'perceptual' not in w or (m.perceptual_fn is not None and (self.fuse & 18) == 18)
        ok = (m.decouple_rendering and m.sync_free and 'rgb' in w and perceptual_ok and r.detach_bary and r.faces_per_pixel > 1
              and r.clip_inside and getattr(m.renderer_fine, 'clip_inside', True) and getattr(m, 'default_criteria', True)
              and r.cam_name == 'perspective' and m.blocks_n_faces < (1 << 20) and m.n_blocks + 2 < (1 << 11) and m.n_blocks <= 64
              and ops.FUSED_FORWARD and ops.FUSED_BACKWARD and ops.TILED_FRAGMENTS and ops.UV_FRAGMENTS and ops.HARD_UV_FRAGMENTS
              and ops.COARSE_BINS and ops.TEXTURE_BINS)
        lib = _lib.load()
        return bool(ok and hasattr(lib, 'dbw_train_step_run'))

    def _plan_handle(self):
        return self._cur[0]

    def close(self):
        if os.getpid() == self._pid:
            for handle, *_ in self._plans.values():
                _lib.load().dbw_train_step_destroy(handle)
        self._plans, self._cur = {}, None

    def __del__(self):
        try:
            self.close()
        except Exception:
            pass

    def _plan_for(self, inp, B, defer=False):
        m = self.m
        coarse = m.is_live('coarse_learning')
        decim = int(m.decim_factor) if m.is_live('decimate_txt') else 1
        decim_blocks = decim if coarse else 1
        renderer = m.renderer if coarse else m.renderer_fine
        dev = inp['imgs'].device
        Kt = renderer.cameras.K
        seq = self.backward_order
        if seq is None:
            seq = 1 if (m.world_size > 1 and not defer) else 0
        both = self.binned_concurrent
        if both is None:
            both = m.world_size == 1
        key = (coarse, decim, decim_blocks, m.world_size, self.fuse, int(seq), int(bool(both)), Kt.data_ptr(), m.R_world.data_ptr(),
               m.R_world._version, m.T_world._version, float(m.S_world),
               self.params.flat.data_ptr(), tuple(sorted(m.loss_weights.items())), float(m.opacity_noise or 0.0), bool(m.kill_blocks),
               int(self.serial_setup_max_views), bool(self.sync_events), bool(defer))
        have = self._plans.get(key)
        if have is not None and have[3] >= B:
            self._cur = have
            return self._cur
        max_views = max(int(self.max_views or 0), B)
        if have is not None:
            if os.getpid() == self._pid:
                with torch.cuda.device(dev):
                    torch.cuda.synchronize(dev)
                    _lib.load().dbw_train_step_destroy(have[0])
            if self._clean_plan == have[0]:
                self._clean_plan = None
            del self._plans[key]
        w = m.loss_weights
        rs = 1.0 / m.world_size
        fine = not coarse
        S_w, R_w, T_w = m._world_consts()
        TS, u_, nb = m.txt_size, m.txt_bkg_upscale, m.n_blocks
        keep = []
        d = _lib.StepDesc()
        H, W = m.img_size
        d.H, d.W, d.faces_per_pixel, d.max_views = H, W, int(renderer.faces_per_pixel), max_views
        d.n_blocks, d.block_nv, d.block_nf = nb, m._block_nv, m.BNF
        d.n_sky_verts, d.n_ground_verts = m._bkg_verts.shape[0], m._ground_base.shape[0]
        d.n_sky_faces, d.n_ground_faces = m._n_bkg_faces, m._n_ground_faces
        d.txt_size, d.env_txt_size, d.decim_env, d.decim_blocks, d.coarse = TS, TS * u_, decim, decim_blocks, int(coarse)
        cfg = renderer._cfg(nb * m.BNF)
        d.sigma, d.blur_radius = float(cfg.sigma), float(cfg.blur)
        d.z_clip, d.cam_eps, d.perspective_correct = float(cfg.z_clip or 0.0), float(cfg.eps), int(cfg.persp)
        for i in range(3):
            d.bg_fg[i], d.bg_env[i] = float(renderer.background_color[i]), float(m.renderer_env.background_color[i])
        d.S_world, d.ratio_block_scene, d.scale_min = float(S_w), float(m.ratio_block_scene), float(m.scale_min)
        d.opacity_noise = float(m.opacity_noise) if (m.opacity_noise and coarse) else 0.0
# ... 5 lines not shown
        d.w_rgb = float(w['rgb'])
        d.w_parsimony = float(w['parsimony']) * rs if ('parsimony' in w and coarse) else 0.0
        d.w_tv_bkg, d.w_tv_blocks, d.w_tv_ground = tv, tv, tv * tv_f
        d.w_overlap = float(w['overlap']) * rs if ('overlap' in w and coarse) else 0.0
        d.overlap_points, d.overlap_temperature, d.overlap_n_blocks = OVERLAP_N_POINTS, OVERLAP_TEMPERATURE, OVERLAP_N_BLOCKS
        Kmat = Kt[0].to(dev).contiguous()
        nbv = m._bkg_verts.shape[0]
        env_verts = torch.empty(nbv + m._ground_base.shape[0], 3, device=dev)
        env_verts[:nbv] = ((m._bkg_verts * S_w) @ R_w + T_w)
        desc_e = m._env_map_desc if decim == 1 else m._env_map_desc_dec
        desc_f = m._block_map_desc_all if decim_blocks == 1 else m._block_map_desc_dec
        keep += [R_w, T_w, Kmat, env_verts]
        d.R_world, d.T_world, d.Kmat = _p(R_w), _p(T_w), _p(Kmat)
        d.ground_base, d.env_verts = _p(m._ground_base), _p(env_verts)
        d.env_faces, d.env_face_uvs, d.env_face_map, d.env_map_desc = _p(m._env_faces), _p(m._env_face_uvs), _p(m._env_face_map), _p(desc_e)
        d.trig, d.block_faces, d.block_face_uvs = _p(m._trig), _p(m._block_faces_all), _p(m._block_face_uvs_all)
        d.block_face_map, d.block_map_desc = _p(m._block_face_map_all), _p(desc_f)
        if decim_blocks == 1:
            d.block_bin_base, d.block_bin_info, d.n_bins = _p(m._block_bin_base), _p(m._block_bin_info), nb * m._bins_per_block
        g = {n: m.get_parameter(n).grad for n, _, _ in self.params.names}
        for f, n in (('sq_eps', 'sq_eps'), ('S', 'S'), ('R6', 'R_6d'), ('T', 'T'), ('alpha_logit', 'alpha_logit'), ('R6_ground', 'R_6d_ground'),
                     ('T_ground', 'T_ground'), ('texture_bkg', 'texture_bkg'), ('texture_ground', 'texture_ground'), ('textures', 'textures')):
            setattr(d, f, _p(m.get_parameter(n)))
            setattr(d, 'g_' + f, _p(g[n]))
        P = self.params
        d.flat_param, d.flat_grad, d.exp_avg, d.exp_avg_sq = _p(P.flat), _p(P.grad), _p(self.opt[0]), _p(self.opt[1])
        d.group_end[0], d.group_end[1] = P.bounds[0][1], P.bounds[1][1]
        d.small_grads, d.n_small_grads = _p(P.grad), P.bounds[0][1]
        d.fuse, d.backward_order, d.binned_concurrent = self.fuse, int(seq), int(bool(both))
        d.serial_setup_max_views = int(self.serial_setup_max_views)
        d.seed = int(getattr(m, '_rng_seed', 227391)) & 0xffffffffffffffff
        d.sync_events = int(bool(self.sync_events))
        lib = _lib.load()
        nbytes = lib.dbw_train_step_workspace_bytes(ctypes.byref(d))
        if nbytes == 0:
            raise RuntimeError(f'dbw_train_step_workspace_bytes: {lib.dbw_last_error().decode()}')
        wsb = torch.empty(nbytes + 256, dtype=torch.uint8, device=dev)
        off = (-wsb.data_ptr()) % 256
        wsb = wsb[off:off + nbytes]
        with torch.cuda.device(dev):
            handle = lib.dbw_train_step_create(ctypes.byref(d), wsb.data_ptr(), nbytes)
        if not handle:
            raise RuntimeError(f'dbw_train_step_create: {lib.dbw_last_error().decode()}')
        self._plans[key] = self._cur = (handle, wsb, keep + [d], max_views)
        return self._cur

    def view(self, name, dtype=torch.float32, numel=None):
        handle, wsb = self._cur[:2]
        off = _lib.load().dbw_train_step_offset(handle, _OFF[name])
        t = wsb[off:].view(dtype)
        return t if numel is None else t[:numel]

    def arena(self):
        handle, wsb = self._cur[:2]
        lib = _lib.load()
        return wsb[lib.dbw_train_step_offset(handle, 4):lib.dbw_train_step_offset(handle, 5)]

    def arena_cleaned_by_caller(self):
        self._clean_plan = self._cur[0]

    def void_flag(self):
        handle, wsb = self._cur[:2]
        off = _lib.load().dbw_train_step_void_flag_offset(handle)
        return wsb[off:off + 4].view(torch.float32)

    def voided_runs(self):
        return int(_lib.load().dbw_train_step_voided_runs(self._cur[0]))

    _WAITS = ('prologue', 'tile order', 'fg forward', 'regularisers', 'bin layout', 'fg backward kernel', "blocks' textures", 'env chain', 'texture preparation')

    def last_timeout(self):
        out = (ctypes.c_int * 3)()
        _lib.call('dbw_debug_train_step_last_timeout', self._cur[0], out)
        if out[0] < 0:
            return None
        seen, asked = (ctypes.c_uint * 12)(), (ctypes.c_uint * 12)()
        _lib.call('dbw_debug_train_step_counters', self._cur[0], seen, asked)
        return (self._WAITS[out[0]] if out[0] < len(self._WAITS) else str(out[0]), out[1], out[2],
                {n: (int(seen[i]), int(asked[i])) for i, n in enumerate(self._WAITS)})

    def _report_voided(self):
        h = self._cur[0]
        n = self.voided_runs()
        if n > self._voided_seen.get(h, 0):
# ... 108 lines not shown
```

differentiable-blocksworld_amd/dbw_amd/ops.py:

```python
import ctypes
import math

import torch

from . import _lib

MAX_FACES_PER_PIXEL = 25
ALPHA_SPREAD = 64

def bin_subcursors():
    lib = _lib.load()
    return int(lib.dbw_bin_subcursors()) if hasattr(lib, 'dbw_bin_subcursors') else 16


def __getattr__(name):
    if name == 'BIN_SUBCURSORS':
        return bin_subcursors()
    raise AttributeError(name)

COARSE_BINS = True
TEXTURE_BINS = True
UV_FRAGMENTS = True
TILED_FRAGMENTS = True
FUSED_FORWARD = True
# ... 216 lines not shown
        self.texbins = texbins
        self.bin_demand = None
        self.H, self.W, self.K, self.sigma, self.z_clip, self.persp = H, W, K, float(sigma) if clip_inside else -float(sigma), z_clip, persp
        self.blur = math.log(1. / 1e-4 - 1.) * float(sigma)
        self.detach_bary, self.eps, self.F = detach_bary, eps, F_


HARD_UV_FRAGMENTS = True


def hard_layout(cfg, fa, map_desc):
    ok = (HARD_UV_FRAGMENTS and cfg.K == 1 and cfg.sigma == 0.0 and fa is None and cfg.lds_aggregate and cfg.F < (1 << 20)
          and map_desc.shape[0] < (1 << 11))
    return 3 if ok else 1


def tiled_image_empty(B, C, H, W, device):
    return torch.empty(B, (H + 7) // 8, (W + 7) // 8, C, 64, dtype=torch.float32, device=device)


def tile_image(img):
    B, C, H, W = img.shape
    ty, tx = (H + 7) // 8, (W + 7) // 8
    if (H, W) != (ty * 8, tx * 8):
        img = torch.nn.functional.pad(img, (0, tx * 8 - W, 0, ty * 8 - H))
    return img.reshape(B, C, ty, 8, tx, 8).permute(0, 2, 4, 1, 3, 5).reshape(B, ty, tx, C, 64).contiguous()


def untile_image(t, H, W):
    B, ty, tx, C, _ = t.shape
    return t.view(B, ty, tx, C, 8, 8).permute(0, 3, 1, 4, 2, 5).reshape(B, C, ty * 8, tx * 8)[:, :, :H, :W].contiguous()


def _render_fwd_fused(fvc, cl, B, cfg, face_uvs, face_map, map_desc, maps, fa, bg, tiled=None, stage=0, state=None, img_tiled=False):
    TILED_FRAGMENTS = globals()['TILED_FRAGMENTS'] if tiled is None else tiled
    dev = fvc.device
    Ft = fvc.shape[0]
    if stage == 2:
        ws, ws_bytes, out = state
    else:
        ws_bytes = _workspace_bytes(Ft, B, cfg.H, cfg.W)
        ws = torch.empty((ws_bytes + 3) // 4, dtype=torch.float32, device=dev)
        if TILED_FRAGMENTS:
            ty, tx = (cfg.H + 7) // 8, (cfg.W + 7) // 8
            p2f = torch.empty(B, ty, tx, cfg.K, 64, dtype=torch.int32, device=dev)
            bary = torch.empty(B, ty, tx, cfg.K, 8 if int(TILED_FRAGMENTS) == 2 else 3, 64, dtype=torch.float32, device=dev)
            dists = torch.empty(B, ty, tx, cfg.K, 64, dtype=torch.float32, device=dev)
        else:
            p2f = torch.empty(B, cfg.H, cfg.W, cfg.K, dtype=torch.int32, device=dev)
            bary = torch.empty(B, cfg.H, cfg.W, cfg.K, 3, dtype=torch.float32, device=dev)
            dists = torch.empty(B, cfg.H, cfg.W, cfg.K, dtype=torch.float32, device=dev)
        img = tiled_image_empty(B, 4, cfg.H, cfg.W, dev) if img_tiled else torch.empty(B, 4, cfg.H, cfg.W, dtype=torch.float32, device=dev)
        out = (p2f, bary, dists, img)
    p2f, bary, dists, img = out
    if int(TILED_FRAGMENTS) == 2 and maps.numel() >= (1 << 30):
        raise RuntimeError(f'uv-fragment passes address their texels with 32-bit byte offsets: the maps buffer ({maps.numel()} floats) must hold fewer than 2^30')
    _lib.call('dbw_render_fwd_fused', _ptr(fvc), _ptr(cl['first_idx']), _ptr(cl['num_faces']), _ptr(cl['neighbor']), _ptr(cl['c2o']),
              _ptr(cl['clip_code']), _ptr(cl['clip_w']), 2 * cfg.F, _ptr(face_uvs), _ptr(face_map), _ptr(map_desc), _ptr(maps), _ptr(fa),
              _alpha_len(fa, map_desc, cfg.F), B, Ft, cfg.H, cfg.W, cfg.K, cfg.F, float(cfg.sigma), float(cfg.blur), int(cfg.persp),
              _bg_ptr(bg), _ptr(p2f), _ptr(bary), _ptr(dists), _ptr(img), _ptr(ws), ws_bytes, int(TILED_FRAGMENTS), int(stage),
              int(img_tiled), _stream(fvc))
    return (ws, ws_bytes, out) if stage == 1 else out


class _RenderScene(torch.autograd.Function):
    @staticmethod
    def forward(ctx, verts, maps, faces_alpha, faces_i32, R, T, Kmat, face_uvs, face_map, map_desc, bg, cfg):
        verts_c = _chk(verts.detach(), torch.float32, 'verts')
        maps_c = _chk(maps.detach(), torch.float32, 'maps')
        fa = None if faces_alpha is None else _chk(faces_alpha.detach(), torch.float32, 'faces_alpha')
        B = R.shape[0]
        cl = project_clip(verts_c, faces_i32, R, T, Kmat, cfg.eps, cfg.z_clip, cfg.persp)
        fvc = cl['face_verts'].view(-1, 3, 3)
        ctx.tiled = int(FUSED_FORWARD and FUSED_BACKWARD and TILED_FRAGMENTS)
        if ctx.tiled and UV_FRAGMENTS and cfg.detach_bary and cfg.F < (1 << 20) and map_desc.shape[0] < (1 << 11):
            ctx.tiled = 2
        elif ctx.tiled:
            ctx.tiled = hard_layout(cfg, fa, map_desc)
        if FUSED_FORWARD:
            p2f, bary, dists, img = _render_fwd_fused(fvc, cl, B, cfg, face_uvs, face_map, map_desc, maps_c, fa, bg, ctx.tiled)
        else:
            p2f, _, bary, dists = _raster_fwd(fvc, cl['first_idx'], cl['num_faces'], cl['neighbor'].view(-1), B, cfg.H, cfg.W, cfg.K,
                                              cfg.blur, cfg.persp, True, False, need_zbuf=False)
            img = shade_blend_fwd(p2f, bary, dists, cl, face_uvs, face_map, map_desc, maps_c, fa, cfg.F, cfg.sigma, bg)
        ctx.cfg, ctx.cl = cfg, cl
        ctx.has_alpha = fa is not None
        ctx.bg = bg
        ctx.save_for_backward(verts_c, maps_c, fa if fa is not None else verts_c.new_empty(0), faces_i32, R, T, Kmat, face_uvs,
                              face_map, map_desc, p2f, bary, dists)
        return img

    @staticmethod
    def backward(ctx, g_img):
        verts, maps, fa, faces_i32, R, T, Kmat, face_uvs, face_map, map_desc, p2f, bary, dists = ctx.saved_tensors
# ... 50 lines not shown
    def _fit(self, nbins, device):
        n = nbins * bin_subcursors()
        if self.key != (n, device):
            self.key = (n, device)
            self.cursors = [torch.zeros(n, dtype=torch.int32, device=device) for _ in range(2)]
            self.layouts = [torch.zeros(n, 2, dtype=torch.int32, device=device) for _ in range(2)]
            self.turn, self.ready = 0, False
        return n

    def prepare(self, nbins, cap, device):
        n = self._fit(nbins, device)
        if not self.ready:
            return None
        lay = self.layouts[self.turn]
        _lib.call('dbw_bin_layout', _ptr(self.cursors[1 - self.turn]), n, float(nbins) * float(cap), self.MIN, _ptr(lay),
                  torch.cuda.current_stream(device).cuda_stream)
        self.prepared = (nbins, cap, lay)
        return lay

    def begin(self, nbins, cap, device):
        self._fit(nbins, device)
        lay = None
        if self.ready:
            pre = getattr(self, 'prepared', None)
            lay = pre[2] if (pre is not None and pre[:2] == (nbins, cap) and pre[2] is self.layouts[self.turn]) else self.prepare(nbins, cap, device)
        self.prepared = None
        cur = self.cursors[self.turn]
        cur.zero_()
        self.turn, self.ready = 1 - self.turn, True
        return cur, lay


def _fused_bwd(p2f, bary, dists, cl, face_uvs, face_map, map_desc, maps, fa, cfg, bg, tiled, g_img, B, gscale, after_kernel=None, img_tiled=False,
               bin_demand=None):
    fvc = cl['face_verts'].view(-1, 3, 3)
    per_map = fa is not None and _alpha_len(fa, map_desc, cfg.F) < 0
    g_maps = ARENA.zeros_like(maps)
    g_alpha = None if fa is None else (ARENA.zeros(fa.numel() * ALPHA_SPREAD, torch.float32, fa.device) if per_map else ARENA.zeros_like(fa))
    g_fvc = ARENA.zeros_like(fvc)
    bins = cfg.texbins if (TEXTURE_BINS and not cfg.lds_aggregate) else None
    bin_base = cursor = records = layout = None
    cap = 0
    if bins is not None and bins[2] > 0:
        bin_base, bin_info, nbins = bins
        cap = texbin_capacity(B, cfg.H, cfg.W, cfg.K, nbins)
        if bin_demand is None:
            bin_demand = cfg.bin_demand
        if bin_demand is not None:
            cursor, layout = bin_demand.begin(nbins, cap, fvc.device)
        else:
            cursor = ARENA.zeros(nbins * bin_subcursors(), torch.int32, fvc.device)
        if layout is None:
            layout = uniform_bin_layout(nbins, cap, fvc.device)
        records = torch.empty(nbins * cap * 8, dtype=torch.int32, device=fvc.device)
    _lib.call('dbw_render_bwd_fused', *_shade_args(p2f, bary, dists, cl, face_uvs, face_map, map_desc, maps, fa, cfg.F, cfg.sigma, bg,
                                                   (B, cfg.H, cfg.W, cfg.K)),
              _ptr(g_img), _ptr(fvc), int(cfg.persp), int(cfg.detach_bary), _ptr(g_maps), _ptr(g_alpha), _ptr(g_fvc),
              int(cfg.lds_aggregate), int(tiled), _ptr(bin_base), _ptr(cursor), _ptr(records), cap, _ptr(layout), int(cfg.const_faces),
              _ptr(gscale), int(img_tiled), _stream(fvc))
    if after_kernel is not None:
        after_kernel()
    if records is not None:
        _lib.call('dbw_texbin_reduce', _ptr(bin_info), _ptr(cursor), _ptr(records), cap, _ptr(layout), nbins, _ptr(g_maps), _stream(fvc))
    return g_maps, g_alpha, g_fvc


def render_fwd_fused_mse(cl, B, cfg, face_uvs, face_map, map_desc, maps, fa, bg, env_img, imgs, scale, stage=0, state=None, img_tiled=False):
    fvc = cl['face_verts'].view(-1, 3, 3)
    dev, Ft = fvc.device, fvc.shape[0]
    if stage == 2:
        ws, ws_bytes, out = state
    else:
        ws_bytes = _workspace_bytes(Ft, B, cfg.H, cfg.W)
        ws = torch.empty((ws_bytes + 3) // 4, dtype=torch.float32, device=dev)
        ty, tx = (cfg.H + 7) // 8, (cfg.W + 7) // 8
        p2f = torch.empty(B, ty, tx, cfg.K, 64, dtype=torch.int32, device=dev)
        bary = torch.empty(B, ty, tx, cfg.K, 8, 64, dtype=torch.float32, device=dev)
        dists = torch.empty(B, ty, tx, cfg.K, 64, dtype=torch.float32, device=dev)
        part = torch.empty(B * ty * tx, dtype=torch.float32, device=dev)
        g_fg = tiled_image_empty(B, 4, cfg.H, cfg.W, dev) if img_tiled else torch.empty(B, 4, cfg.H, cfg.W, dtype=torch.float32, device=dev)
        g_env = torch.empty_like(g_fg)
        out = (p2f, bary, dists, part, g_fg, g_env)
    p2f, bary, dists, part, g_fg, g_env = out
    if maps.numel() >= (1 << 30):
        raise RuntimeError(f'uv-fragment passes address their texels with 32-bit byte offsets: the maps buffer ({maps.numel()} floats) must hold fewer than 2^30')
    _lib.call('dbw_render_fwd_fused_mse', _ptr(fvc), _ptr(cl['first_idx']), _ptr(cl['num_faces']), _ptr(cl['neighbor']), _ptr(cl['c2o']),
              _ptr(cl['clip_code']), _ptr(cl['clip_w']), 2 * cfg.F, _ptr(face_uvs), _ptr(face_map), _ptr(map_desc), _ptr(maps), _ptr(fa),
              _alpha_len(fa, map_desc, cfg.F), B, Ft, cfg.H, cfg.W, cfg.K, cfg.F, float(cfg.sigma), float(cfg.blur), int(cfg.persp),
              _bg_ptr(bg), _ptr(p2f), _ptr(bary), _ptr(dists), _ptr(ws), ws_bytes, _ptr(env_img), _ptr(imgs), float(scale), _ptr(part),
              _ptr(g_fg), _ptr(g_env), int(stage), int(img_tiled), _stream(fvc))
    return (ws, ws_bytes, out) if stage == 1 else out

# ... 607 lines not shown
```

Before: 78220 views/s.

## Record texture footprints in forward pass and reuse them in backward

The forward shading passes (soft uv-fragment pass and env fold) now write a per-fragment footprint record: the base texel address, packed steps and bilinear weights. The backward pass reads these records instead of re-deriving the texture footprint from uv and the map descriptor, and re-derives it from the descriptor only on the geometry-gradient path. This trades extra forward stores and backward loads (four floats per fragment) for less recomputation and fewer descriptor lookups in backward. It is enabled by default through a records mask set to 3.

```diff
diff --git a/differentiable-blocksworld_amd/build.py b/differentiable-blocksworld_amd/build.py
--- a/differentiable-blocksworld_amd/build.py
+++ b/differentiable-blocksworld_amd/build.py
@@ -15,7 +15,7 @@
     if not os.path.exists(OUT):
         return True
     t = os.path.getmtime(OUT)
-    deps = [os.path.join(CSRC, f) for f in os.listdir(CSRC)] + [os.path.join(HERE, '..', 'include', h) for h in ('dbw_hip.h', 'dbw_eval.h', 'dbw_viz.h', 'dbw_export.h', 'dbw_ingest.h', 'dbw_lens.h', 'dbw_monitor.h')] + [__file__]
+    deps = [os.path.join(CSRC, f) for f in os.listdir(CSRC)] + [os.path.join(HERE, '..', 'include', h) for h in ('dbw_hip.h', 'dbw_eval.h', 'dbw_viz.h', 'dbw_export.h', 'dbw_ingest.h', 'dbw_lens.h', 'dbw_monitor.h', 'dbw_records.h')] + [__file__]
     return any(os.path.getmtime(d) > t for d in deps)
 
 
diff --git a/differentiable-blocksworld_amd/csrc/env_bwd.h b/differentiable-blocksworld_amd/csrc/env_bwd.h
--- a/differentiable-blocksworld_amd/csrc/env_bwd.h
+++ b/differentiable-blocksworld_amd/csrc/env_bwd.h
@@ -26,18 +26,26 @@
     }
 };
 
+template <bool REC>
 __device__ __forceinline__ void env_bwd_pixel(const ShadeArgs &A, const float *__restrict__ fv, float *__restrict__ gmaps, float *__restrict__ gfv,
                                               int want_bary, int persp, const MapDescCache &mdc, const int *s_md, HardTexAgg &tex_agg,
-                                              HardFaceAgg &face_agg, bool valid, int fc, float u, float v, int jm, const float (&gc)[3], int xi, int yi) {
+                                              HardFaceAgg &face_agg, bool valid, int fc, float u, float v, float wx1, float wy1, int jm,
+                                              const float (&gc)[3], int xi, int yi) {
     const int j = jm & 0xfffff, map = jm >> 20;
     const bool tex = valid && (gc[0] != 0.f || gc[1] != 0.f || gc[2] != 0.f);
     Sample s;
     s.a00 = s.a01 = s.a10 = s.a11 = 0;
     s.w00 = s.w01 = s.w10 = s.w11 = 0.f;
+    auto key_of = [](int a) { return REC ? a : (int)((unsigned)a / 3u); };
     if (__ballot(tex) != 0ull) {
-        int md[6];
-        mdc.get(A, s_md, valid ? map : 0, md);
-        footprint_desc(u, v, md[0], md[1], md[2], md[3], md[4], md[5], s);
+        if (REC) {
+            const FootRec fk{(int)((unsigned)__float_as_int(u) / 3u), __float_as_uint(v), wx1, wy1};
+            foot_rec_unpack<1>(fk, s);
+        } else {
+            int md[6];
+            mdc.get(A, s_md, valid ? map : 0, md);
+            footprint_desc(u, v, md[0], md[1], md[2], md[3], md[4], md[5], s);
+        }
         float w00 = s.w00, w01 = s.w01, w10 = s.w10, w11 = s.w11;
         if (s.a01 == s.a00) { w00 += w01; w01 = 0.f; }
         if (s.a10 == s.a00) { w00 += w10; w10 = 0.f; }
@@ -53,7 +61,7 @@
         for (int q = 0; q < 2; ++q) {
             float val[3] = {gc[0] * w2[q], gc[1] * w2[q], gc[2] * w2[q]};
             const bool on = tex && w2[q] != 0.f;
-            tex_agg.template add_wave_merged<4>(gmaps, (int)((unsigned)a2[q] / 3u), val, on);
+            tex_agg.template add_wave_merged<4>(gmaps, key_of(a2[q]), val, on);
         }
         const bool rest = tex && ((f == 1 && (wt[2] != 0.f || wt[3] != 0.f)) || (f == 2 && wt[3] != 0.f));
         const unsigned long long rm = __ballot(rest);
@@ -63,7 +71,7 @@
             for (int q = 2; q < 4; ++q) {
                 float val[3] = {gc[0] * wt[q], gc[1] * wt[q], gc[2] * wt[q]};
                 const bool on = rest && q > f && wt[q] != 0.f;
-                const int key = (int)((unsigned)ad[q] / 3u);
+                const int key = key_of(ad[q]);
                 if (wide) tex_agg.template add_wave_merged<4>(gmaps, key, val, on);
                 else if (on) tex_agg.add(gmaps, key, val);
             }
@@ -74,6 +82,12 @@
     bool has_g9 = false;
     if (__ballot(geom) != 0ull) {
         if (geom) {
+            if (REC) {
+                int md[6];
+                mdc.get(A, s_md, map, md);
+                const FootRec fr{__float_as_int(u), __float_as_uint(v), wx1, wy1};
+                foot_rec_unpack_grad(fr, md[1], md[2], md[3], md[4], s);
+            }
             float gu, gv;
             sample_grad_uv(A.maps, s, gc, gu, gv);
             const float *uv = A.face_uvs + (long long)j * 6;
@@ -111,7 +125,7 @@
 }
 
 
-template <int P>
+template <int P, bool REC>
 __device__ __forceinline__ void env_bwd_region(const ShadeArgs &A, long long total_blocks, const float *__restrict__ gimg,
                                                float *__restrict__ gmaps, const float *__restrict__ fv, float *__restrict__ gfv,
                                                int want_bary, int persp, void *lds, int *s_md) {
@@ -133,7 +147,7 @@
     const long long plane = (long long)A.H * A.W;
     const float gs = A.gscale ? *A.gscale : 1.f;
     int rfc[P], xs[P], ys[P];
-    float ru[P], rv[P], rjm[P], rg[P][3];
+    float ru[P], rv[P], rwx[P], rwy[P], rjm[P], rg[P][3];
     bool inpx[P];
 #pragma unroll
     for (int p = 0; p < P; ++p) {
@@ -145,7 +159,12 @@
         inpx[p] = real && xs[p] < A.W && ys[p] < A.H;
         rfc[p] = ld_stream(A.p2f + (tile << 6) + lane);
         const float *b = A.bary + ((tile * 3) << 6) + lane;
-        ru[p] = ld_stream(b); rv[p] = ld_stream(b + 64); rjm[p] = ld_stream(b + 128);
+        rwx[p] = rwy[p] = 0.f;
+        if (REC) {
+            const float *f = A.foot_in + ((tile * 4) << 6) + lane;
+            ru[p] = ld_stream(f); rv[p] = ld_stream(f + 64); rwx[p] = ld_stream(f + 128); rwy[p] = ld_stream(f + 192);
+        } else { ru[p] = ld_stream(b); rv[p] = ld_stream(b + 64); }
+        rjm[p] = ld_stream(b + 128);
         const int xc = xs[p] < A.W ? xs[p] : A.W - 1, yc = ys[p] < A.H ? ys[p] : A.H - 1;
         const long long gb = A.img_tiled ? ((tile * 4) << 6) + lane : (long long)n * 4 * plane + (long long)yc * A.W + xc;
         const long long cs = A.img_tiled ? 64 : plane;
@@ -166,12 +185,16 @@
         jm[p] = valid[p] ? __float_as_int(rjm[p]) : 0;
         ru[p] = valid[p] ? ru[p] : 0.f;
         rv[p] = valid[p] ? rv[p] : 0.f;
+        rwx[p] = valid[p] ? rwx[p] : 0.f;
+        rwy[p] = valid[p] ? rwy[p] : 0.f;
 #pragma unroll
         for (int c = 0; c < 3; ++c) gc[p][c] = valid[p] ? rg[p][c] * gs : 0.f;
     }
 #pragma unroll 1
-    for (int p = 0; p < P; ++p)
-        env_bwd_pixel(A, fv, gmaps, gfv, want_bary, persp, mdc, s_md, tex_agg, face_agg, valid[p], fc[p], ru[p], rv[p], jm[p], gc[p], xs[p], ys[p]);
+    for (int p = 0; p < P; ++p) {
+        const int xi = REC ? (tx0 + p % R::PX) * 8 + (lane & 7) : xs[p], yi = REC ? (ty0 + p / R::PX) * 8 + (lane >> 3) : ys[p];
+        env_bwd_pixel<REC>(A, fv, gmaps, gfv, want_bary, persp, mdc, s_md, tex_agg, face_agg, valid[p], fc[p], ru[p], rv[p], rwx[p], rwy[p], jm[p], gc[p], xi, yi);
+    }
     __syncthreads();
     tex_agg.flush(gmaps, threadIdx.x, NTH);
     face_agg.flush(gfv, threadIdx.x, NTH);
diff --git a/differentiable-blocksworld_amd/csrc/render_fused.hip b/differentiable-blocksworld_amd/csrc/render_fused.hip
--- a/differentiable-blocksworld_amd/csrc/render_fused.hip
+++ b/differentiable-blocksworld_amd/csrc/render_fused.hip
@@ -4,6 +4,7 @@
 #include "raster_bin.h"
 #include "step_kernels.h"
 #include "../../include/dbw_hip.h"
+#include "../../include/dbw_records.h"
 
 #include <math.h>
 #include <stdlib.h>
@@ -185,6 +186,15 @@
     return u.r;
 }
 
+__device__ __forceinline__ void store_foot_rec(float *__restrict__ rp, const FootRec &fr) {
+#if DBW_NT_STORES
+    __builtin_nontemporal_store(__int_as_float(fr.a00), rp); __builtin_nontemporal_store(__uint_as_float(fr.steps), rp + 64);
+    __builtin_nontemporal_store(fr.wx1, rp + 128); __builtin_nontemporal_store(fr.wy1, rp + 192);
+#else
+    rp[0] = __int_as_float(fr.a00); rp[64] = __uint_as_float(fr.steps); rp[128] = fr.wx1; rp[192] = fr.wy1;
+#endif
+}
+
 struct EnvFold {
     const FaceRec *recs;
     const int *first_idx;
@@ -196,6 +206,7 @@
     const float *maps;
     float bg[3];
     int *p2f; float *uvj;
+    float *foot;
     int persp, dbg;
     float ndc[4];
 };
@@ -226,7 +237,9 @@
             convert_bary(sr.cd, sr.w2, sr.w3, bc, bo);
             interp_uv(bo, sr.uv, u, vv);
             SampleFwd s;
-            footprint_fwd(u, vv, sr.off, sr.hw >> 16, sr.hw & 0xffff, sr.pads >> 16, sr.pads & 0xffff, sr.sh, s);
+            FootRec fr;
+            footprint_fwd_rec<true>(u, vv, sr.off, sr.hw >> 16, sr.hw & 0xffff, sr.pads >> 16, sr.pads & 0xffff, sr.sh, s, fr);
+            if (in_img && E.foot) store_foot_rec(E.foot + ((long long)L * 4 << 6) + lane, fr);
             fetch_fwd(E.maps, s, rgb);
             if (in_img) {
                 const long long o = ((long long)L << 6) + lane;
@@ -277,7 +290,9 @@
     convert_bary(sr.cd, sr.w2, sr.w3, bc, bo);
     interp_uv(bo, sr.uv, u, vv);
     SampleFwd s;
-    footprint_fwd(u, vv, sr.off, sr.hw >> 16, sr.hw & 0xffff, sr.pads >> 16, sr.pads & 0xffff, sr.sh, s);
+    FootRec fr;
+    footprint_fwd_rec<true>(u, vv, sr.off, sr.hw >> 16, sr.hw & 0xffff, sr.pads >> 16, sr.pads & 0xffff, sr.sh, s, fr);
+    if (valid && E.foot) store_foot_rec(E.foot + ((long long)L * 4 << 6) + lane, fr);
     float col[3];
     fetch_fwd(E.maps, s, col);
 #pragma unroll
@@ -367,7 +382,7 @@
     uv8_epilogue(A, n, xi, yi, in_img, tile, lane, px, image, env_rgb, fold, true);
 }
 
-template <int KMAX>
+template <int KMAX, bool KEX>
 __device__ __forceinline__ void shade_uv8(const ShadeArgs &A, int K, const ShadeRec *__restrict__ srec, const TopK<KMAX, true> &q, const pay4 *home, int n,
                                           int xi, int yi, int *__restrict__ p2f, float *__restrict__ bary, float *__restrict__ dists,
                                           float *__restrict__ image, int dbg, const float (&env_rgb)[3], bool fold) {
@@ -379,6 +394,8 @@
     int *__restrict__ p2f_t = p2f + tb;
     float *__restrict__ dists_t = dists + tb;
     float *__restrict__ bary_t = bary + tb * 8;
+    float *__restrict__ foot_t = A.foot_out + tb * 4;
+    const bool want_foot = A.foot_out != nullptr;
 #if DBW_TOPK_ORDERED
     const int cnt = in_img ? q.cnt : 0;
 #else
@@ -415,7 +432,13 @@
 #endif
         const float a = cur.valid ? e * sr.fa : 0.f;
         SampleFwd s;
-        footprint_fwd(u, v, sr.off, sr.hw >> 16, sr.hw & 0xffff, sr.pads >> 16, sr.pads & 0xffff, sr.sh, s);
+        FootRec fr;
+        footprint_fwd_rec<false>(u, v, sr.off, sr.hw >> 16, sr.hw & 0xffff, sr.pads >> 16, sr.pads & 0xffff, sr.sh, s, fr);
+        if (want_foot && cur.valid) {
+            float *rb = foot_t;
+            asm volatile("" : "+s"(rb));
+            store_foot_rec(rb + (k << 8) + lane, fr);
+        }
         float c[3];
         fetch_fwd(A.maps, s, c);
         if (!(a != 0.f)) c[0] = c[1] = c[2] = 0.f;
@@ -426,7 +449,9 @@
 #if DBW_NT_STORES
             __builtin_nontemporal_store(k == 0 ? (cur.fik | (cnt << FRAG_COUNT_SHIFT)) : cur.fik, p2f_t + o);
             __builtin_nontemporal_store(d, dists_t + o);
-            float *bp = bary_t + (k << 9) + lane;
+            float *bb = bary_t;
+            if (KEX) asm volatile("" : "+s"(bb));
+            float *bp = bb + (k << 9) + lane;
             __builtin_nontemporal_store(u, bp);
             __builtin_nontemporal_store(v, bp + 64);
             __builtin_nontemporal_store(__int_as_float(sr.j | (sr.map << 20)), bp + 128);
@@ -444,6 +469,7 @@
             bp[256] = c[0]; bp[320] = c[1]; bp[384] = c[2];
             bp[448] = T;
 #endif
+
         }
         cur = nxt;
     }
@@ -487,7 +513,7 @@
     FPROF_T(t_k1);
     if constexpr (UV) {
         if (empty) shade_uv8_empty<KMAX>(A, K, n, xi, yi, p2f, image, env_rgb, fold);
-        else shade_uv8<KMAX>(A, K, srec, q, home, n, xi, yi, p2f, bary, dists, image, dbg, env_rgb, fold);
+        else shade_uv8<KMAX, KEX>(A, K, srec, q, home, n, xi, yi, p2f, bary, dists, image, dbg, env_rgb, fold);
     }
     else {
         if (xi >= A.W || yi >= A.H) return;
@@ -553,7 +579,7 @@
                                     int perspective_correct, const float *background3, int32_t *pix_to_face, float *bary,
                                     float *dists, float *image, void *workspace, size_t workspace_bytes,
                                     int frag_layout, const MseArgs *mse, int stage, int image_layout, dbw_stream_t stream,
-                                    const dbw::EnvFoldHost *fold = nullptr) {
+                                    const dbw::EnvFoldHost *fold = nullptr, float *frag_records = nullptr) {
     DBW_REQUIRE(stage >= 0 && stage <= 2, "stage must be 0 (whole pass), 1 (workspace only) or 2 (workspace already prepared)");
     DBW_REQUIRE(face_verts_c && first_idx && num_faces && pix_to_face && bary && dists && (image || mse) && workspace, "null pointer");
     DBW_REQUIRE(workspace_bytes >= dbw_rasterize_workspace_bytes(F_total), "workspace too small");
@@ -570,6 +596,8 @@
     DBW_REQUIRE(image_layout == 0 || image_layout == 1, "image_layout must be 0 (N,C,H,W) or 1 (8x8-tile planar)");
     A.tiled = frag_layout;
     A.img_tiled = image_layout;
+    DBW_REQUIRE(!frag_records || (frag_layout == 2 && K > 1 && sigma >= 0.f), "footprint records belong to the uv-fragment soft pass (frag_layout 2, K > 1, sigma >= 0)");
+    A.foot_out = frag_records;
     if (mse) {
         DBW_REQUIRE(frag_layout == 2 && K > 1 && sigma >= 0.f, "the composite + MSE epilogue belongs to the uv-fragment soft pass (frag_layout 2, K > 1, sigma >= 0)");
         DBW_REQUIRE(stage == 1 || ((mse->env_img || fold) && mse->target && mse->loss_part && mse->g_fg && mse->g_env), "null pointer");
@@ -608,7 +636,7 @@
         E.recs = w.recs; E.first_idx = fold->first_idx; E.cell = w.cell; E.pool = w.pool; E.dom = w.dom; E.clist = w.list; E.ccount = w.count; E.nx = w.nx; E.ny = w.ny;
         E.num_faces = fold->num_faces; E.srec = (const ShadeRec *)w.shade_recs; E.maps = fold->maps;
         for (int i = 0; i < 3; ++i) E.bg[i] = fold->bg[i];
-        E.p2f = fold->p2f; E.uvj = fold->uvj; E.persp = perspective_correct; E.dbg = g_render_dbg;
+        E.p2f = fold->p2f; E.uvj = fold->uvj; E.foot = fold->foot; E.persp = perspective_correct; E.dbg = g_render_dbg;
         for (int i = 0; i < 4; ++i) E.ndc[i] = cb.ndc[i];
         A.lean_grads = 1;
     }
@@ -629,9 +657,22 @@
                                     int perspective_correct, const float *background3, int32_t *pix_to_face, float *bary,
                                     float *dists, float *image, void *workspace, size_t workspace_bytes,
                                     int frag_layout, int stage, int image_layout, dbw_stream_t stream) {
+    return dbw_render_fwd_fused_rec(face_verts_c, first_idx, num_faces, neighbor, c2o, clip_code, clip_w, Fc_stride, face_uvs, face_map, map_desc, maps,
+                                    faces_alpha, alpha_len, N, F_total, H, W, K, F, sigma, blur_radius, perspective_correct, background3, pix_to_face,
+                                    bary, dists, image, workspace, workspace_bytes, frag_layout, stage, image_layout, stream, nullptr);
+}
+
+extern "C" int dbw_render_fwd_fused_rec(const float *face_verts_c, const int32_t *first_idx, const int32_t *num_faces,
+                                        const int32_t *neighbor, const int32_t *c2o, const int32_t *clip_code,
+                                        const float *clip_w, int Fc_stride, const float *face_uvs, const int32_t *face_map,
+                                        const int32_t *map_desc, const float *maps, const float *faces_alpha, int alpha_len,
+                                        int N, int64_t F_total, int H, int W, int K, int F, float sigma, float blur_radius,
+                                        int perspective_correct, const float *background3, int32_t *pix_to_face, float *bary,
+                                        float *dists, float *image, void *workspace, size_t workspace_bytes,
+                                        int frag_layout, int stage, int image_layout, dbw_stream_t stream, float *frag_records) {
     return render_fwd_impl(face_verts_c, first_idx, num_faces, neighbor, c2o, clip_code, clip_w, Fc_stride, face_uvs, face_map, map_desc, maps,
                            faces_alpha, alpha_len, N, F_total, H, W, K, F, sigma, blur_radius, perspective_correct, background3, pix_to_face,
-                           bary, dists, image, workspace, workspace_bytes, frag_layout, nullptr, stage, image_layout, stream);
+                           bary, dists, image, workspace, workspace_bytes, frag_layout, nullptr, stage, image_layout, stream, nullptr, frag_records);
 }
 
 extern "C" int dbw_render_fwd_fused_mse(const float *face_verts_c, const int32_t *first_idx, const int32_t *num_faces,
@@ -655,9 +696,9 @@
                                    int64_t F_total, int H, int W, int K, int F, float sigma, float blur_radius, int perspective_correct,
                                    const float *background3, int32_t *pix_to_face, float *bary, float *dists, void *workspace, size_t workspace_bytes,
                                    const float *target, float mse_scale, float *loss_partial, float *grad_fg, float *grad_env, const EnvFoldHost &fold,
-                                   float *rec_out, const float *grad_rec, hipStream_t stream) {
+                                   float *rec_out, const float *grad_rec, float *frag_records, hipStream_t stream) {
     const MseArgs mse{nullptr, target, mse_scale, loss_partial, grad_fg, grad_env, rec_out, grad_rec};
     return render_fwd_impl(face_verts_c, first_idx, num_faces, neighbor, c2o, clip_code, clip_w, Fc_stride, face_uvs, face_map, map_desc, maps,
                            faces_alpha, alpha_len, N, F_total, H, W, K, F, sigma, blur_radius, perspective_correct, background3, pix_to_face,
-                           bary, dists, nullptr, workspace, workspace_bytes, 2, &mse, 2, 1, (dbw_stream_t)stream, &fold);
-}
+                           bary, dists, nullptr, workspace, workspace_bytes, 2, &mse, 2, 1, (dbw_stream_t)stream, &fold, frag_records);
+}
diff --git a/differentiable-blocksworld_amd/csrc/shade_blend.hip b/differentiable-blocksworld_amd/csrc/shade_blend.hip
--- a/differentiable-blocksworld_amd/csrc/shade_blend.hip
+++ b/differentiable-blocksworld_amd/csrc/shade_blend.hip
@@ -1,6 +1,7 @@
 #include "shade_common.h"
 #include "env_bwd.h"
 #include "../../include/dbw_hip.h"
+#include "../../include/dbw_records.h"
 #include "step_kernels.h"
 
 #include <stdlib.h>
@@ -554,10 +555,11 @@
 #else
 #define BWD_CLOCK_END(n_, layers_)
 #endif
-template <bool BINNED>
-__global__ __launch_bounds__(NT, (BINNED ? DBW_UVB_WAVES : 5)) void render_bwd_uv_kernel(ShadeArgs A, long long total_blocks, const float *__restrict__ gimg,
-                                                              float *__restrict__ gmaps, float *__restrict__ galpha,
-                                                              const float *__restrict__ fv, float *__restrict__ gfv) {
+template <bool BINNED, bool REC>
+__device__ __forceinline__ void render_bwd_uv_body(const ShadeArgs &A, long long total_blocks, const float *__restrict__ gimg,
+                                                   float *__restrict__ gmaps, float *__restrict__ galpha,
+                                                   const float *__restrict__ fv, float *__restrict__ gfv) {
+    static_assert(!(BINNED && REC), "footprint records: the unbinned instantiation");
     extern __shared__ __attribute__((aligned(16))) float s_uvbwd[];
     constexpr bool SINGLE = false;
     (void)SINGLE;
@@ -578,6 +580,7 @@
     const int *__restrict__ p2f_t = A.p2f + tb + lane;
     const float *__restrict__ dists_t = A.dists + tb + lane;
     const float *__restrict__ bary_t = A.bary + tb * 8 + lane;
+    const float *__restrict__ foot_t = REC ? A.foot_in + tb * 4 + lane : nullptr;
     int cnt = 0;
     if (in_img && (yi >> 3) < tiles_y && (xi >> 3) < tiles_x) {
         const int raw0 = ld_stream(p2f_t);
@@ -629,14 +632,20 @@
     PROF_ADD(0, t_begin, t_p0);
     BlendBack bk;
     blend_back_init(bk, A.bg);
-    struct Raw { int fc; float u, v, jm, a, c0, c1, c2, T, d; };
+    struct Raw { int fc; float u, v, jm, a, c0, c1, c2, T, d, wx1, wy1; };
     auto load = [&](int k, bool ok) {
         Raw r;
-        r.fc = 0; r.u = r.v = r.jm = r.a = r.c0 = r.c1 = r.c2 = r.d = 0.f; r.T = 1.f;
+        r.fc = 0; r.u = r.v = r.jm = r.a = r.c0 = r.c1 = r.c2 = r.d = r.wx1 = r.wy1 = 0.f; r.T = 1.f;
         if (ok) {
             r.fc = ld_stream(p2f_t + (k << 6)) & FRAG_FACE_MASK;
             const float *b = bary_t + (k << 9);
+            if (REC) {
+                const float *f = foot_t + (k << 8);
+                r.u = ld_stream(f); r.v = ld_stream(f + 64); r.wx1 = ld_stream(f + 128); r.wy1 = ld_stream(f + 192);
+                r.jm = ld_stream(b + 128); r.a = ld_stream(b + 192);
+            } else {
             r.u = ld_stream(b); r.v = ld_stream(b + 64); r.jm = ld_stream(b + 128); r.a = ld_stream(b + 192);
+            }
             r.c0 = ld_stream(b + 256); r.c1 = ld_stream(b + 320); r.c2 = ld_stream(b + 384); r.T = ld_stream(b + 448);
             r.d = ld_stream(dists_t + (k << 6));
         }
@@ -649,10 +658,12 @@
         r.u = ld_stream(b); r.v = ld_stream(b + 64); r.jm = ld_stream(b + 128); r.a = ld_stream(b + 192);
         r.c0 = ld_stream(b + 256); r.c1 = ld_stream(b + 320); r.c2 = ld_stream(b + 384); r.T = ld_stream(b + 448);
         r.d = ld_stream(dists_t + (k << 6));
+        r.wx1 = r.wy1 = 0.f;
         return r;
     };
     auto masked = [&](const Raw &x, bool ok) {
         Raw r;
+        r.wx1 = r.wy1 = 0.f;
         r.fc = ok ? (x.fc & FRAG_FACE_MASK) : 0;
         r.u = ok ? x.u : 0.f; r.v = ok ? x.v : 0.f; r.jm = ok ? x.jm : 0.f; r.a = ok ? x.a : 0.f;
         r.c0 = ok ? x.c0 : 0.f; r.c1 = ok ? x.c1 : 0.f; r.c2 = ok ? x.c2 : 0.f; r.T = ok ? x.T : 1.f; r.d = ok ? x.d : 0.f;
@@ -767,10 +778,16 @@
                 }
             }
         } else if (__ballot(tex) != 0ull) {
-            int md[6];
-            mdc.get(A, s_md, valid ? map : 0, md);
             Sample s;
-            footprint_desc(cur.u, cur.v, md[0], md[1], md[2], md[3], md[4], md[5], s);
+            if (REC) {
+                const FootRec fr{(int)((unsigned)__float_as_int(cur.u) / 3u), __float_as_uint(cur.v), cur.wx1, cur.wy1};
+                foot_rec_unpack<1>(fr, s);
+            } else {
+                int md[6];
+                mdc.get(A, s_md, valid ? map : 0, md);
+                footprint_desc(cur.u, cur.v, md[0], md[1], md[2], md[3], md[4], md[5], s);
+            }
+            auto key_of = [](int a) { return REC ? a : (int)((unsigned)a / 3u); };
             float w00 = s.w00, w01 = s.w01, w10 = s.w10, w11 = s.w11;
             if (s.a01 == s.a00) { w00 += w01; w01 = 0.f; }
             if (s.a10 == s.a00) { w00 += w10; w10 = 0.f; }
@@ -784,7 +801,7 @@
                 int dk, rp, taps = 0, tap_lanes = 0, tap_replays = 0;
                 for (int q = 0; q < 4; ++q) {
                     const bool onq = tex && wt[q] != 0.f;
-                    key_stats((int)((unsigned)ad[q] / 3u), onq, dk, rp);
+                    key_stats(key_of(ad[q]), onq, dk, rp);
                     taps += __ballot(onq) != 0ull ? 1 : 0;
                     tap_lanes += __popcll(__ballot(onq));
                     tap_replays += rp;
@@ -800,8 +817,8 @@
             for (int q = 0; q < 2; ++q) {
                 float v3[3] = {gc[0] * w2[q], gc[1] * w2[q], gc[2] * w2[q]};
                 bool on = tex && w2[q] != 0.f && !(A.dbg & 1);
-                if (TEX_MERGE > 0 && __ballot(on) != 0ull) lane_merge<3, TEX_MERGE>((int)((unsigned)a2[q] / 3u), on, v3);
-                if (on) tex_agg.add(gmaps, (int)((unsigned)a2[q] / 3u), v3);
+                if (TEX_MERGE > 0 && __ballot(on) != 0ull) lane_merge<3, TEX_MERGE>(key_of(a2[q]), on, v3);
+                if (on) tex_agg.add(gmaps, key_of(a2[q]), v3);
             }
             const bool rest = tex && !(A.dbg & 1) && ((f == 1 && (wt[2] != 0.f || wt[3] != 0.f)) || (f == 2 && wt[3] != 0.f));
             if (__ballot(rest) != 0ull) {
@@ -809,7 +826,7 @@
                 for (int q = 2; q < 4; ++q)
                     if (rest && q > f && wt[q] != 0.f) {
                         const float v3[3] = {gc[0] * wt[q], gc[1] * wt[q], gc[2] * wt[q]};
-                        tex_agg.add(gmaps, (int)((unsigned)ad[q] / 3u), v3);
+                        tex_agg.add(gmaps, key_of(ad[q]), v3);
                     }
             }
         }
@@ -876,6 +893,19 @@
     PROF_ADD(1, t_sync, t_fl);
     PROF_ADD(7, t_begin, t_fl);
     BWD_CLOCK_END(n, kmax);
+}
+
+template <bool BINNED>
+__global__ __launch_bounds__(NT, (BINNED ? DBW_UVB_WAVES : 5)) void render_bwd_uv_kernel(ShadeArgs A, long long total_blocks, const float *__restrict__ gimg,
+                                                              float *__restrict__ gmaps, float *__restrict__ galpha,
+                                                              const float *__restrict__ fv, float *__restrict__ gfv) {
+    if constexpr (!BINNED) {
+        if (A.foot_in) {
+            render_bwd_uv_body<false, true>(A, total_blocks, gimg, gmaps, galpha, fv, gfv);
+            return;
+        }
+    }
+    render_bwd_uv_body<BINNED, false>(A, total_blocks, gimg, gmaps, galpha, fv, gfv);
 }
 
 #ifndef DBW_BIN_STAGE
@@ -1066,6 +1096,7 @@
     A.lean_grads = 0;
     A.rec_out = nullptr; A.grad_rec = nullptr;
     A.sync_flag = nullptr; A.sync_val = 0;
+    A.foot_out = nullptr; A.foot_in = nullptr;
     return DBW_OK;
 }
 
@@ -1103,7 +1134,14 @@
                                                             float *__restrict__ gfv, int want_bary, int persp) {
     extern __shared__ __attribute__((aligned(16))) float s_hard[];
     __shared__ __attribute__((aligned(16))) int s_md[MD_CACHE_MAPS * 8];
-    env_bwd_region<HARD_P>(A, total_blocks, gimg, gmaps, fv, gfv, want_bary, persp, s_hard, s_md);
+    env_bwd_region<HARD_P, false>(A, total_blocks, gimg, gmaps, fv, gfv, want_bary, persp, s_hard, s_md);
+}
+__global__ __launch_bounds__(NT) void render_bwd_hard_kernel_rec(ShadeArgs A, long long total_blocks, const float *__restrict__ gimg,
+                                                                float *__restrict__ gmaps, const float *__restrict__ fv,
+                                                                float *__restrict__ gfv, int want_bary, int persp) {
+    extern __shared__ __attribute__((aligned(16))) float s_hard[];
+    __shared__ __attribute__((aligned(16))) int s_md[MD_CACHE_MAPS * 8];
+    env_bwd_region<HARD_P, true>(A, total_blocks, gimg, gmaps, fv, gfv, want_bary, persp, s_hard, s_md);
 }
 
 __global__ void flag_store_kernel(unsigned *flag, unsigned v) { __hip_atomic_store(flag, v, __ATOMIC_RELEASE, __HIP_MEMORY_SCOPE_AGENT); }
@@ -1140,6 +1178,8 @@
         hipLaunchKernelGGL(flag_store_kernel, dim3(1), dim3(1), 0, s, A.sync_flag, A.sync_val);
         A.sync_flag = nullptr;
     }
+    DBW_REQUIRE(!A.foot_in || (uv_kernel && !A.bin_records) || A.tiled == 3,
+                "footprint records are read by the unbinned uv backward (frag_layout 2, detach_bary, lds_aggregate) and by the hard pass's backward (frag_layout 3)");
     if (uv_kernel) {
         static bool raised_uv = false;
         if (!raised_uv) {
@@ -1160,6 +1200,10 @@
     }
     if (A.tiled == 3) {
         const long long regions = HardRegion<HARD_P>::blocks(N, H, W);
+        if (A.foot_in)
+            hipLaunchKernelGGL(render_bwd_hard_kernel_rec, dim3(dbw_xcd_grid(regions)), dim3(NT), HardTexAgg::BYTES + HardFaceAgg::BYTES, s, A, regions, grad_image,
+                               grad_maps, fv, gfv, want_bary, persp);
+        else
         hipLaunchKernelGGL(render_bwd_hard_kernel, dim3(dbw_xcd_grid(regions)), dim3(NT), HardTexAgg::BYTES + HardFaceAgg::BYTES, s, A, regions, grad_image,
                            grad_maps, fv, gfv, want_bary, persp);
         return dbw_check_launch("render_bwd_hard_kernel");
@@ -1205,7 +1249,8 @@
                                     float *grad_maps, float *grad_faces_alpha, float *grad_face_verts_c,
                                     int lds_aggregate, int frag_layout, const int32_t *bin_base, int32_t *bin_cursor,
                                     void *bin_records, int bin_cap, const uint32_t *bin_layout, int const_geometry_faces,
-                                    const float *grad_scale, int image_layout, dbw_stream_t stream, unsigned *sync_flag, unsigned sync_val) {
+                                    const float *grad_scale, int image_layout, dbw_stream_t stream, unsigned *sync_flag, unsigned sync_val,
+                                    const float *frag_records) {
     ShadeArgs A;
     int rc = fill_args(A, pix_to_face, bary, dists, c2o, clip_code, clip_w, Fc_stride, face_uvs, face_map, map_desc,
                        maps, faces_alpha, alpha_len, N, H, W, K, F, sigma, background3);
@@ -1223,6 +1268,7 @@
     A.gscale = grad_scale;
     A.geom_begin = const_geometry_faces;
     A.sync_flag = sync_flag; A.sync_val = sync_val;
+    A.foot_in = frag_records;
     DBW_REQUIRE((bin_base && bin_cursor && bin_records && bin_cap >= DBW_BIN_SUBCURSORS) || (!bin_base && !bin_cursor && !bin_records), "texture bins: all or none (bin_cap >= DBW_BIN_SUBCURSORS)");
     if (bin_records && !lds_aggregate) {
         A.bin_base = bin_base; A.bin_cursor = bin_cursor; A.bin_records = (int4 *)bin_records; A.bin_cap = bin_cap; A.bin_layout = bin_layout;
@@ -1245,7 +1291,23 @@
     return dbw::render_bwd_fused_signal(pix_to_face, bary, dists, c2o, clip_code, clip_w, Fc_stride, face_uvs, face_map, map_desc, maps, faces_alpha, alpha_len,
                                         N, H, W, K, F, sigma, background3, grad_image, face_verts_c, perspective_correct, detach_bary, grad_maps, grad_faces_alpha,
                                         grad_face_verts_c, lds_aggregate, frag_layout, bin_base, bin_cursor, bin_records, bin_cap, bin_layout, const_geometry_faces,
-                                        grad_scale, image_layout, stream, nullptr, 0);
+                                        grad_scale, image_layout, stream, nullptr, 0, nullptr);
+}
+
+extern "C" int dbw_render_bwd_fused_rec(const int32_t *pix_to_face, const float *bary, const float *dists,
+                                        const int32_t *c2o, const int32_t *clip_code, const float *clip_w, int Fc_stride,
+                                        const float *face_uvs, const int32_t *face_map, const int32_t *map_desc,
+                                        const float *maps, const float *faces_alpha, int alpha_len, int N, int H, int W,
+                                        int K, int F, float sigma, const float *background3, const float *grad_image,
+                                        const float *face_verts_c, int perspective_correct, int detach_bary,
+                                        float *grad_maps, float *grad_faces_alpha, float *grad_face_verts_c,
+                                        int lds_aggregate, int frag_layout, const int32_t *bin_base, int32_t *bin_cursor,
+                                        void *bin_records, int bin_cap, const uint32_t *bin_layout, int const_geometry_faces,
+                                        const float *grad_scale, int image_layout, dbw_stream_t stream, const float *frag_records) {
+    return dbw::render_bwd_fused_signal(pix_to_face, bary, dists, c2o, clip_code, clip_w, Fc_stride, face_uvs, face_map, map_desc, maps, faces_alpha, alpha_len,
+                                        N, H, W, K, F, sigma, background3, grad_image, face_verts_c, perspective_correct, detach_bary, grad_maps, grad_faces_alpha,
+                                        grad_face_verts_c, lds_aggregate, frag_layout, bin_base, bin_cursor, bin_records, bin_cap, bin_layout, const_geometry_faces,
+                                        grad_scale, image_layout, stream, nullptr, 0, frag_records);
 }
 
 #ifdef DBW_TILE_CLOCK
diff --git a/differentiable-blocksworld_amd/csrc/shade_common.h b/differentiable-blocksworld_amd/csrc/shade_common.h
--- a/differentiable-blocksworld_amd/csrc/shade_common.h
+++ b/differentiable-blocksworld_amd/csrc/shade_common.h
@@ -48,6 +48,7 @@
     float *rec_out;
     const float *grad_rec;
     unsigned *sync_flag; unsigned sync_val;
+    float *foot_out; const float *foot_in;
 };
 
 #ifndef DBW_MD_LDS
diff --git a/differentiable-blocksworld_amd/csrc/shade_math.h b/differentiable-blocksworld_amd/csrc/shade_math.h
--- a/differentiable-blocksworld_amd/csrc/shade_math.h
+++ b/differentiable-blocksworld_amd/csrc/shade_math.h
@@ -84,7 +84,30 @@
 }
 
 struct SampleFwd { unsigned b00, b01, b10, b11; float w00, w01, w10, w11; };
-DBW_HD void footprint_fwd(float u, float v, int off, int h, int w, int pl, int pr, int sh, SampleFwd &s) {
+
+struct FootRec { int a00; unsigned steps; float wx1, wy1; };
+constexpr int FOOT_REC_MAX_WS = (1 << 14) - 1;
+DBW_HD bool foot_rec_fits(int ws) { return ws >= 1 && ws <= FOOT_REC_MAX_WS; }
+
+template <int STRIDE = 3>
+DBW_HD void foot_rec_unpack(const FootRec &r, Sample &s) {
+    const int cs = ((int)(r.steps << 16)) >> 16, rs = (int)((r.steps >> 16) & 0x3fffu);
+    s.a00 = r.a00; s.a01 = r.a00 + cs * STRIDE;
+    s.a10 = r.a00 - rs * STRIDE; s.a11 = s.a10 + cs * STRIDE;
+    s.wx1 = r.wx1; s.wx0 = 1.f - s.wx1;
+    s.wy1 = r.wy1; s.wy0 = 1.f - s.wy1;
+    s.w00 = s.wx0 * s.wy0; s.w01 = s.wx1 * s.wy0; s.w10 = s.wx0 * s.wy1; s.w11 = s.wx1 * s.wy1;
+    s.dudx = s.dvdy = 0.f;
+    s.r0 = s.c0 = s.r1 = s.c1 = s.ws = 0;
+}
+DBW_HD void foot_rec_unpack_grad(const FootRec &r, int h, int w, int pl, int pr, Sample &s) {
+    foot_rec_unpack(r, s);
+    s.dudx = (r.steps & (1u << 30)) ? 0.f : (float)(w + pl + pr - 1);
+    s.dvdy = (r.steps & (1u << 31)) ? 0.f : (float)(h - 1);
+}
+
+template <bool REC, bool CLAMP_BITS>
+DBW_HD void footprint_fwd_t(float u, float v, int off, int h, int w, int pl, int pr, int sh, SampleFwd &s, FootRec &r) {
     const int wp = w + pl + pr;
     float ix = ((u * 2.f - 1.f) + 1.f) / 2.f * (float)(wp - 1);
     float iy = ((v * 2.f - 1.f) + 1.f) / 2.f * (float)(h - 1);
@@ -100,6 +123,20 @@
     s.b00 = ((unsigned)off + (unsigned)(r0 * ws + c0) * 3u) * 4u; s.b01 = ((unsigned)off + (unsigned)(r0 * ws + c1) * 3u) * 4u;
     s.b10 = ((unsigned)off + (unsigned)(r1 * ws + c0) * 3u) * 4u; s.b11 = ((unsigned)off + (unsigned)(r1 * ws + c1) * 3u) * 4u;
     s.w00 = wx0 * wy0; s.w01 = wx1 * wy0; s.w10 = wx0 * wy1; s.w11 = wx1 * wy1;
+    if (REC) {
+        r.a00 = (int)(s.b00 >> 2);
+        r.steps = ((unsigned)(c1 - c0) & 0xffffu) | ((unsigned)((r0 - r1) * ws) << 16);
+        if (CLAMP_BITS) r.steps |= ((ix == 0.f || ix == (float)(wp - 1)) ? (1u << 30) : 0u) | ((iy == 0.f || iy == (float)(h - 1)) ? (1u << 31) : 0u);
+        r.wx1 = wx1; r.wy1 = wy1;
+    }
+}
+template <bool CLAMP_BITS>
+DBW_HD void footprint_fwd_rec(float u, float v, int off, int h, int w, int pl, int pr, int sh, SampleFwd &s, FootRec &r) {
+    footprint_fwd_t<true, CLAMP_BITS>(u, v, off, h, w, pl, pr, sh, s, r);
+}
+DBW_HD void footprint_fwd(float u, float v, int off, int h, int w, int pl, int pr, int sh, SampleFwd &s) {
+    FootRec r;
+    footprint_fwd_t<false, false>(u, v, off, h, w, pl, pr, sh, s, r);
 }
 DBW_HD void fetch_fwd(const float *maps, const SampleFwd &s, float c[3]) {
     DBW_FMA_SCOPE
diff --git a/differentiable-blocksworld_amd/csrc/step_kernels.h b/differentiable-blocksworld_amd/csrc/step_kernels.h
--- a/differentiable-blocksworld_amd/csrc/step_kernels.h
+++ b/differentiable-blocksworld_amd/csrc/step_kernels.h
@@ -100,6 +100,7 @@
 struct EnvFoldHost {
     const RasterWorkspace *ws; const int *first_idx, *num_faces; const float *maps; float bg[3];
     int *p2f; float *uvj;
+    float *foot;
 };
 int render_fwd_fused_mse_fold(const float *face_verts_c, const int32_t *first_idx, const int32_t *num_faces, const int32_t *neighbor,
                               const int32_t *c2o, const int32_t *clip_code, const float *clip_w, int Fc_stride, const float *face_uvs,
@@ -107,7 +108,7 @@
                               int64_t F_total, int H, int W, int K, int F, float sigma, float blur_radius, int perspective_correct,
                               const float *background3, int32_t *pix_to_face, float *bary, float *dists, void *workspace, size_t workspace_bytes,
                               const float *target, float mse_scale, float *loss_partial, float *grad_fg, float *grad_env, const EnvFoldHost &fold,
-                              float *rec_out, const float *grad_rec, hipStream_t stream);
+                              float *rec_out, const float *grad_rec, float *frag_records, hipStream_t stream);
 
 int render_bwd_fused_signal(const int32_t *pix_to_face, const float *bary, const float *dists, const int32_t *c2o, const int32_t *clip_code,
                             const float *clip_w, int Fc_stride, const float *face_uvs, const int32_t *face_map, const int32_t *map_desc, const float *maps,
@@ -115,6 +116,7 @@
                             const float *grad_image, const float *face_verts_c, int perspective_correct, int detach_bary, float *grad_maps,
                             float *grad_faces_alpha, float *grad_face_verts_c, int lds_aggregate, int frag_layout, const int32_t *bin_base,
                             int32_t *bin_cursor, void *bin_records, int bin_cap, const uint32_t *bin_layout, int const_geometry_faces,
-                            const float *grad_scale, int image_layout, dbw_stream_t stream, unsigned *sync_flag, unsigned sync_val);
+                            const float *grad_scale, int image_layout, dbw_stream_t stream, unsigned *sync_flag, unsigned sync_val,
+                            const float *frag_records);
 
 }
diff --git a/differentiable-blocksworld_amd/csrc/train_step.hip b/differentiable-blocksworld_amd/csrc/train_step.hip
--- a/differentiable-blocksworld_amd/csrc/train_step.hip
+++ b/differentiable-blocksworld_amd/csrc/train_step.hip
@@ -1,7 +1,9 @@
 #include "dbw_common.h"
 #include "raster_bin.h"
 #include "step_kernels.h"
+#include "shade_math.h"
 #include "../../include/dbw_hip.h"
+#include "../../include/dbw_records.h"
 
 #include <math.h>
 #include <mutex>
@@ -64,6 +66,7 @@
     size_t env_maps, blk_maps, sig[3], g_sig[3];
     size_t alpha, alpha_full, keep, blk_verts, sq_local, losses, target;
     size_t records, cursor[2], layout[2], layout_uniform;
+    size_t rec_fg, rec_env; bool has_rec_fg, has_rec_env;
     size_t arena_begin, g_alpha_full, ovl_ws, vals, tickets, g_blk_maps, g_env_maps, g_maps_end, g_fa, g_fvc_f, g_blk_verts, g_fvc_e, g_env_verts, arena_end;
     size_t total;
     int Fe, Ff, Ve, Vf, tiles, bin_cap;
@@ -72,6 +75,10 @@
 
 bool tv_on(const dbw_step_desc &d) { return d.w_tv_bkg != 0.f || d.w_tv_blocks != 0.f || d.w_tv_ground != 0.f; }
 bool bins_on(const dbw_step_desc &d) { return d.decim_blocks == 1 && d.n_bins > 0 && d.block_bin_base && d.block_bin_info; }
+
+thread_local int g_records_mask = 3;
+bool rec_fg_on(const dbw_step_desc &d) { return (g_records_mask & 1) != 0 && (d.fuse & 16) != 0 && d.decim_blocks > 1 && !bins_on(d) && foot_rec_fits(d.txt_size / d.decim_blocks); }
+bool rec_env_on(const dbw_step_desc &d) { return (g_records_mask & 2) != 0 && (d.fuse & 16) != 0 && foot_rec_fits(d.env_txt_size / d.decim_env); }
 
 int texbin_capacity(int B, int H, int W, int K, int nbins) {
     long long cap = (long long)B * H * W * (K > 4 ? K : 4) / (2LL * nbins);
@@ -141,6 +148,9 @@
         for (int i = 0; i < 2; ++i) { L.layout[i] = o; o += al(nsub * 8); }
         L.layout_uniform = o; o += al(nsub * 8);
     }
+    L.has_rec_fg = rec_fg_on(d); L.has_rec_env = rec_env_on(d);
+    if (L.has_rec_fg) { L.rec_fg = o; o += al(bt * K * 64 * 4 * 4); }
+    if (L.has_rec_env) { L.rec_env = o; o += al(bt * 64 * 4 * 4); }
     L.arena_begin = o;
     L.g_alpha_full = o; o += al((size_t)d.n_blocks * 4);
     L.ovl_ws = o; o += al((size_t)d.n_blocks * 18 * 4);
@@ -285,6 +295,13 @@
     bool last_tail;
 };
 
+extern "C" int dbw_records_abi_version(void) { return DBW_RECORDS_ABI_VERSION; }
+extern "C" int dbw_train_step_records_mask(int mask) {
+    const int was = g_records_mask;
+    if (mask >= 0) g_records_mask = mask & 3;
+    return was;
+}
+
 extern "C" size_t dbw_train_step_workspace_bytes(const dbw_step_desc *desc) {
     if (check_desc(desc)) return 0;
     Layout L;
@@ -369,6 +386,8 @@
         case 12: return (int64_t)L.bary_e;
         case 13: return (int64_t)L.g_blk_maps;
         case 14: return (int64_t)L.g_maps_end;
+        case 15: return L.has_rec_fg ? (int64_t)L.rec_fg : -1;
+        case 16: return L.has_rec_env ? (int64_t)L.rec_env : -1;
         default: return -1;
     }
 }
@@ -668,10 +687,12 @@
         fh.ws = &we; fh.first_idx = IP(L.e.first); fh.num_faces = IP(L.e.num); fh.maps = FP(L.env_maps);
         for (int i = 0; i < 3; ++i) fh.bg[i] = d.bg_env[i];
         fh.p2f = IP(L.p2f_e); fh.uvj = FP(L.bary_e);
+        fh.foot = L.has_rec_env ? FP(L.rec_env) : nullptr;
         RC(render_fwd_fused_mse_fold(FP(L.f.fvc), IP(L.f.first), IP(L.f.num), IP(L.f.nbr), IP(L.f.c2o), IP(L.f.code), FP(L.f.cw), 2 * Ff, d.block_face_uvs,
                                      d.block_face_map, d.block_map_desc, FP(L.blk_maps), fa, alpha_len, B, Ftf, H, W, K, Ff, d.sigma, d.blur_radius,
                                      d.perspective_correct, d.bg_fg, IP(L.p2f), FP(L.bary), FP(L.dists), ws + L.f.rws, L.f.rws_bytes, target, mse_scale,
-                                     FP(L.part), FP(L.g_fg), FP(L.g_env), fh, phase == 1 ? in->rec_out : nullptr, phase == 2 ? in->grad_rec : nullptr, M));
+                                     FP(L.part), FP(L.g_fg), FP(L.g_env), fh, phase == 1 ? in->rec_out : nullptr, phase == 2 ? in->grad_rec : nullptr,
+                                     L.has_rec_fg ? FP(L.rec_fg) : nullptr, M));
         if (phase == 1) { p->phase1_done = true; return DBW_OK; }
         p->phase1_done = false;
     } else
@@ -699,9 +720,10 @@
 
     auto env_backward = [&](hipStream_t st) -> int {
         PROF(6, st);
-        RC(dbw_render_bwd_fused(IP(L.p2f_e), FP(L.bary_e), FP(L.dists_e), IP(L.e.c2o), IP(L.e.code), FP(L.e.cw), 2 * Fe, d.env_face_uvs, d.env_face_map,
-                                d.env_map_desc, FP(L.env_maps), nullptr, 0, B, H, W, 1, Fe, 0.f, d.bg_env, FP(L.g_env), FP(L.e.fvc), d.perspective_correct, 0,
-                                FP(L.g_env_maps), nullptr, FP(L.g_fvc_e), 1, 3, nullptr, nullptr, nullptr, 0, nullptr, d.n_sky_faces, nullptr, 1, st));
+        RC(render_bwd_fused_signal(IP(L.p2f_e), FP(L.bary_e), FP(L.dists_e), IP(L.e.c2o), IP(L.e.code), FP(L.e.cw), 2 * Fe, d.env_face_uvs, d.env_face_map,
+                                   d.env_map_desc, FP(L.env_maps), nullptr, 0, B, H, W, 1, Fe, 0.f, d.bg_env, FP(L.g_env), FP(L.e.fvc), d.perspective_correct, 0,
+                                   FP(L.g_env_maps), nullptr, FP(L.g_fvc_e), 1, 3, nullptr, nullptr, nullptr, 0, nullptr, d.n_sky_faces, nullptr, 1, st, nullptr, 0,
+                                   (fold && L.has_rec_env) ? FP(L.rec_env) : nullptr));
         PROF(7, st);
         RC(dbw_project_clip_bwd(d.env_verts, d.env_faces, in->R, in->T, d.Kmat, B, Ve, Fe, d.cam_eps, d.z_clip, d.perspective_correct, IP(L.e.num),
                                 IP(L.e.c2o), IP(L.e.code), FP(L.e.cw), FP(L.g_fvc_e), FP(L.g_env_verts), st));
@@ -735,7 +757,8 @@
     RC(render_bwd_fused_signal(IP(L.p2f), FP(L.bary), FP(L.dists), IP(L.f.c2o), IP(L.f.code), FP(L.f.cw), 2 * Ff, d.block_face_uvs, d.block_face_map,
                                d.block_map_desc, FP(L.blk_maps), fa, alpha_len, B, H, W, K, Ff, d.sigma, d.bg_fg, FP(L.g_fg), FP(L.f.fvc), d.perspective_correct, 1,
                                FP(L.g_blk_maps), coarse ? FP(L.g_fa) : nullptr, FP(L.g_fvc_f), d.decim_blocks > 1 ? 1 : 0, 2, bins ? d.block_bin_base : nullptr, cursor,
-                               bins ? (void *)(ws + L.records) : nullptr, bins ? L.bin_cap : 0, blayout, 0, nullptr, 1, M, bwd_flag, bwd_val));
+                               bins ? (void *)(ws + L.records) : nullptr, bins ? L.bin_cap : 0, blayout, 0, nullptr, 1, M, bwd_flag, bwd_val,
+                               (fold && L.has_rec_fg) ? FP(L.rec_fg) : nullptr));
     PROF(5, M);
     if (fwd_signal_folded) RC(side_after_fwd());
     if (two && seq) {
diff --git a/differentiable-blocksworld_amd/dbw_amd/_lib.py b/differentiable-blocksworld_amd/dbw_amd/_lib.py
--- a/differentiable-blocksworld_amd/dbw_amd/_lib.py
+++ b/differentiable-blocksworld_amd/dbw_amd/_lib.py
@@ -221,6 +221,25 @@
 MONITOR_ABI_VERSION = _header_monitor_abi_version()
 
 
+RECORDS_SIGNATURES = {
+    'dbw_render_fwd_fused_rec': SIGNATURES['dbw_render_fwd_fused'] + [c_p],
+    'dbw_render_bwd_fused_rec': SIGNATURES['dbw_render_bwd_fused'] + [c_p],
+}
+RECORDS_OTHER_SIGNATURES = {
+    'dbw_train_step_records_mask': (c_i, [c_i]),
+}
+FOOT_REC_MAX_STORED_WIDTH = 16383
+
+
+def _header_records_abi_version():
+    import re
+    with open(os.path.join(_HERE, '..', '..', 'include', 'dbw_records.h')) as f:
+        return int(re.search(r'#define DBW_RECORDS_ABI_VERSION (\d+)', f.read()).group(1))
+
+
+RECORDS_ABI_VERSION = _header_records_abi_version()
+
+
 def load():
     global _lib
     if _lib is not None:
@@ -305,6 +324,15 @@
         for name, (restype, argtypes) in MONITOR_OTHER_SIGNATURES.items():
             fn = getattr(lib, name)
             fn.argtypes, fn.restype = argtypes, restype
+    if hasattr(lib, 'dbw_render_fwd_fused_rec'):
+        for name, argtypes in RECORDS_SIGNATURES.items():
+            fn = getattr(lib, name)
+            fn.argtypes = argtypes
+            fn.restype = c_i
+        for name, (restype, argtypes) in RECORDS_OTHER_SIGNATURES.items():
+            fn = getattr(lib, name)
+            fn.argtypes, fn.restype = argtypes, restype
+        lib.dbw_records_abi_version.restype = c_i
     _lib = lib
     return lib
 
diff --git a/differentiable-blocksworld_amd/dbw_amd/c_step.py b/differentiable-blocksworld_amd/dbw_amd/c_step.py
--- a/differentiable-blocksworld_amd/dbw_amd/c_step.py
+++ b/differentiable-blocksworld_amd/dbw_amd/c_step.py
@@ -12,7 +12,7 @@
 FUSE_ALL = 127
 _SIDE_STREAMS = {}
 _OFF = {'alpha': 0, 'alpha_full': 1, 'keep': 2, 'losses': 3, 'arena_begin': 4, 'arena_end': 5, 'g_fg': 6, 'g_env': 7, 'env_img': 8, 'blk_verts': 9,
-        'loss_part': 10, 'p2f_env': 11, 'uvj_env': 12}
+        'loss_part': 10, 'p2f_env': 11, 'uvj_env': 12, 'rec_fg': 15, 'rec_env': 16}
 
 
 def side_stream(dev, priority=True):
@@ -60,6 +60,7 @@
         self.own_side_stream = False
         self.serial_setup_max_views = 12
         self.sync_events = os.environ.get('DBW_STEP_EVENTS', '0') not in ('', '0')
+        self.frag_records = int(os.environ.get('DBW_FRAG_RECORDS', '3'))
         self.read_losses = False
         self._plans = {}
         self._pid = os.getpid()
@@ -115,7 +116,7 @@
         key = (coarse, decim, decim_blocks, m.world_size, self.fuse, int(seq), int(bool(both)), Kt.data_ptr(), m.R_world.data_ptr(),
                m.R_world._version, m.T_world._version, float(m.S_world),
                self.params.flat.data_ptr(), tuple(sorted(m.loss_weights.items())), float(m.opacity_noise or 0.0), bool(m.kill_blocks),
-               int(self.serial_setup_max_views), bool(self.sync_events), bool(defer))
+               int(self.serial_setup_max_views), bool(self.sync_events), bool(defer), int(self._records_mask()))
         have = self._plans.get(key)
         if have is not None and have[3] >= B:
             self._cur = have
@@ -187,6 +188,8 @@
         d.seed = int(getattr(m, '_rng_seed', 227391)) & 0xffffffffffffffff
         d.sync_events = int(bool(self.sync_events))
         lib = _lib.load()
+        if hasattr(lib, 'dbw_train_step_records_mask'):
+            lib.dbw_train_step_records_mask(self._records_mask())
         nbytes = lib.dbw_train_step_workspace_bytes(ctypes.byref(d))
         if nbytes == 0:
             raise RuntimeError(f'dbw_train_step_workspace_bytes: {lib.dbw_last_error().decode()}')
@@ -205,6 +208,12 @@
         off = _lib.load().dbw_train_step_offset(handle, _OFF[name])
         t = wsb[off:].view(dtype)
         return t if numel is None else t[:numel]
+
+    def _records_mask(self):
+        return 3 if self.frag_records is True else int(self.frag_records)
+
+    def has_records(self, which):
+        return _lib.load().dbw_train_step_offset(self._cur[0], _OFF['rec_' + which]) >= 0
 
     def arena(self):
         handle, wsb = self._cur[:2]
diff --git a/differentiable-blocksworld_amd/dbw_amd/ops.py b/differentiable-blocksworld_amd/dbw_amd/ops.py
--- a/differentiable-blocksworld_amd/dbw_amd/ops.py
+++ b/differentiable-blocksworld_amd/dbw_amd/ops.py
@@ -272,7 +272,11 @@
     return t.view(B, ty, tx, C, 8, 8).permute(0, 3, 1, 4, 2, 5).reshape(B, C, ty * 8, tx * 8)[:, :, :H, :W].contiguous()
 
 
-def _render_fwd_fused(fvc, cl, B, cfg, face_uvs, face_map, map_desc, maps, fa, bg, tiled=None, stage=0, state=None, img_tiled=False):
+def footprint_records_empty(B, H, W, K, device):
+    return torch.empty(B, (H + 7) // 8, (W + 7) // 8, K, 4, 64, dtype=torch.int32, device=device)
+
+
+def _render_fwd_fused(fvc, cl, B, cfg, face_uvs, face_map, map_desc, maps, fa, bg, tiled=None, stage=0, state=None, img_tiled=False, foot_records=None):
     TILED_FRAGMENTS = globals()['TILED_FRAGMENTS'] if tiled is None else tiled
     dev = fvc.device
     Ft = fvc.shape[0]
@@ -295,11 +299,13 @@
     p2f, bary, dists, img = out
     if int(TILED_FRAGMENTS) == 2 and maps.numel() >= (1 << 30):
         raise RuntimeError(f'uv-fragment passes address their texels with 32-bit byte offsets: the maps buffer ({maps.numel()} floats) must hold fewer than 2^30')
-    _lib.call('dbw_render_fwd_fused', _ptr(fvc), _ptr(cl['first_idx']), _ptr(cl['num_faces']), _ptr(cl['neighbor']), _ptr(cl['c2o']),
+    rec = () if foot_records is None else (_ptr(foot_records),)
+    _lib.call('dbw_render_fwd_fused' if foot_records is None else 'dbw_render_fwd_fused_rec',
+              _ptr(fvc), _ptr(cl['first_idx']), _ptr(cl['num_faces']), _ptr(cl['neighbor']), _ptr(cl['c2o']),
               _ptr(cl['clip_code']), _ptr(cl['clip_w']), 2 * cfg.F, _ptr(face_uvs), _ptr(face_map), _ptr(map_desc), _ptr(maps), _ptr(fa),
               _alpha_len(fa, map_desc, cfg.F), B, Ft, cfg.H, cfg.W, cfg.K, cfg.F, float(cfg.sigma), float(cfg.blur), int(cfg.persp),
               _bg_ptr(bg), _ptr(p2f), _ptr(bary), _ptr(dists), _ptr(img), _ptr(ws), ws_bytes, int(TILED_FRAGMENTS), int(stage),
-              int(img_tiled), _stream(fvc))
+              int(img_tiled), _stream(fvc), *rec)
     return (ws, ws_bytes, out) if stage == 1 else out
 
 
@@ -416,7 +422,7 @@
 
 
 def _fused_bwd(p2f, bary, dists, cl, face_uvs, face_map, map_desc, maps, fa, cfg, bg, tiled, g_img, B, gscale, after_kernel=None, img_tiled=False,
-               bin_demand=None):
+               bin_demand=None, foot_records=None):
     fvc = cl['face_verts'].view(-1, 3, 3)
     per_map = fa is not None and _alpha_len(fa, map_desc, cfg.F) < 0
     g_maps = ARENA.zeros_like(maps)
@@ -437,11 +443,12 @@
         if layout is None:
             layout = uniform_bin_layout(nbins, cap, fvc.device)
         records = torch.empty(nbins * cap * 8, dtype=torch.int32, device=fvc.device)
-    _lib.call('dbw_render_bwd_fused', *_shade_args(p2f, bary, dists, cl, face_uvs, face_map, map_desc, maps, fa, cfg.F, cfg.sigma, bg,
-                                                   (B, cfg.H, cfg.W, cfg.K)),
+    rec = () if foot_records is None else (_ptr(foot_records),)
+    _lib.call('dbw_render_bwd_fused' if foot_records is None else 'dbw_render_bwd_fused_rec',
+              *_shade_args(p2f, bary, dists, cl, face_uvs, face_map, map_desc, maps, fa, cfg.F, cfg.sigma, bg, (B, cfg.H, cfg.W, cfg.K)),
               _ptr(g_img), _ptr(fvc), int(cfg.persp), int(cfg.detach_bary), _ptr(g_maps), _ptr(g_alpha), _ptr(g_fvc),
               int(cfg.lds_aggregate), int(tiled), _ptr(bin_base), _ptr(cursor), _ptr(records), cap, _ptr(layout), int(cfg.const_faces),
-              _ptr(gscale), int(img_tiled), _stream(fvc))
+              _ptr(gscale), int(img_tiled), _stream(fvc), *rec)
     if after_kernel is not None:
         after_kernel()
     if records is not None:
diff --git a/include/dbw_records.h b/include/dbw_records.h
--- /dev/null
+++ b/include/dbw_records.h
@@ -0,0 +1,40 @@
+#ifndef DBW_RECORDS_H
+#define DBW_RECORDS_H
+
+#include "dbw_hip.h"
+
+#define DBW_RECORDS_ABI_VERSION 1
+#define DBW_FOOT_REC_MAX_STORED_WIDTH 16383
+
+#ifdef __cplusplus
+extern "C" {
+#endif
+
+int dbw_records_abi_version(void);
+
+int dbw_train_step_records_mask(int mask);
+
+int dbw_render_fwd_fused_rec(const float *face_verts_c, const int32_t *first_idx, const int32_t *num_faces,
+                             const int32_t *neighbor, const int32_t *c2o, const int32_t *clip_code, const float *clip_w,
+                             int Fc_stride, const float *face_uvs, const int32_t *face_map, const int32_t *map_desc,
+                             const float *maps, const float *faces_alpha, int alpha_len, int N, int64_t F_total, int H, int W,
+                             int K, int F, float sigma, float blur_radius, int perspective_correct, const float *background3,
+                             int32_t *pix_to_face, float *bary, float *dists, float *image, void *workspace,
+                             size_t workspace_bytes, int frag_layout, int stage, int image_layout, dbw_stream_t stream,
+                             float *frag_records);
+
+int dbw_render_bwd_fused_rec(const int32_t *pix_to_face, const float *bary, const float *dists, const int32_t *c2o,
+                             const int32_t *clip_code, const float *clip_w, int Fc_stride, const float *face_uvs,
+                             const int32_t *face_map, const int32_t *map_desc, const float *maps, const float *faces_alpha,
+                             int alpha_len, int N, int H, int W, int K, int F, float sigma, const float *background3,
+                             const float *grad_image, const float *face_verts_c, int perspective_correct, int detach_bary,
+                             float *grad_maps, float *grad_faces_alpha, float *grad_face_verts_c, int lds_aggregate,
+                             int frag_layout, const int32_t *bin_base, int32_t *bin_cursor, void *bin_records, int bin_cap,
+                             const uint32_t *bin_layout, int const_geometry_faces, const float *grad_scale, int image_layout,
+                             dbw_stream_t stream, const float *frag_records);
+
+#ifdef __cplusplus
+}
+#endif
+
+#endif
```

After: 77470 views/s. About the same (-1.0%).
